# CompVis/stable-diffusion

Hardware: AMD Instinct MI355X
Metric: 512x512 images/sec, SD-v1-4 50-step PLMS CFG=7.5 (higher is better)
Workload: dtype f16

## Files before the change

### include/sdmi.h

```cpp
#ifndef SDMI_H_
#define SDMI_H_

#include <stdint.h>

#ifdef __cplusplus
extern "C" {
#endif

#define SDMI_ABI_VERSION 17

typedef struct sdmi_unet sdmi_unet;

typedef struct sdmi_unet_cfg {
  int32_t in_channels;
  int32_t out_channels;
  int32_t model_channels;
  int32_t num_res_blocks;
  int32_t n_levels;
  int32_t channel_mult[8];
  int32_t n_attention_resolutions;
  int32_t attention_resolutions[8];
  int32_t num_heads;
  int32_t transformer_depth;
  int32_t context_dim;
// ... 164 lines not shown
                       float* special_care_scores, int B, int Nc, int Ns, int E, void* stream);

typedef struct sdmi_knn sdmi_knn;
int sdmi_knn_create(int D, int64_t capacity_rows, sdmi_knn** out);
int sdmi_knn_destroy(sdmi_knn* h);
int sdmi_knn_set_rows(sdmi_knn* h, int64_t first_row, int64_t n, const float* rows, void* stream);
int sdmi_knn_finalize(sdmi_knn* h, void* stream);
int64_t sdmi_knn_rows(const sdmi_knn* h);
int sdmi_knn_dim(const sdmi_knn* h);
int64_t sdmi_knn_workspace_bytes(sdmi_knn* h, int B, int k);
int sdmi_knn_search(sdmi_knn* h, const float* queries, int B, int k, int32_t* idx_out, float* score_out, float* nn_out_or_null,
                    void* workspace, int64_t workspace_bytes, void* stream);
int sdmi_knn_condition(sdmi_knn* h, const float* c, int B, int k, float* c_out, int32_t* idx_out, float* score_out, void* workspace,
                       int64_t workspace_bytes, void* stream);
int sdmi_k_knn_inv_norm(const float* db, int64_t N, int D, float* inv_norm, void* stream);
int sdmi_k_knn_scan(const float* db, const float* inv_norm, int64_t N, int D, const float* queries, int B, int k, int64_t slab_rows,
                    float* cand_score, int32_t* cand_idx, void* stream);
int sdmi_k_knn_merge(const float* cand_score, const int32_t* cand_idx, int B, int n_lists, int k, int32_t* idx_out, float* score_out,
                     void* stream);
int sdmi_k_knn_stream_read(const float* p, int64_t n_floats, float* sink, void* stream);
int sdmi_k_knn_gather(const float* db, const float* inv_norm, int64_t N, int D, const int32_t* idx, int B, int k, const float* c0_or_null,
                      float* out, int64_t ldo, void* stream);

typedef struct sdmi_igemm_desc {
  const void* a0; const void* a1; const void* a2;
  int32_t c0, c1, c2, lda0, lda1, lda2;
  int32_t B, Hin, Win, Hout, Wout, ksize, stride, up;
  const void* w;
  int32_t N;
  int32_t mode;
  const float* bias; const float* rowvec; int32_t ld_rowvec;
  const float* residual; int32_t ldr;
  float* out_f32; void* out_f16; int32_t ldo;
  void* seg_dst[3]; int32_t seg_kind[3];
  int32_t heads, dh, ntok, ntok_pad, segC;
  int32_t splitk;
  float* splitk_ws; int64_t splitk_ws_floats;
  int32_t tile;
  int32_t dma;
  int32_t asym_pad;
  int32_t gn_n; void* gn_acc[2]; int32_t gn_cpg[2]; int32_t gn_cbase[2];
  int32_t* splitk_cnt; int32_t splitk_cnt_ints;
  int32_t split16;
  const float* f16_scale; float* lnp_out;
  const float* lnf_part; int32_t lnf_npart; float lnf_eps; const float* lnf_cs; const float* lnf_d;
  const float* pgn_gamma; const float* pgn_beta; float pgn_eps; int32_t pgn_silu;
  void* pgn_out; int32_t pgn_keep_f32; int32_t* pgn_applied;
  void* out_lo;
} sdmi_igemm_desc;
int sdmi_k_igemm(const sdmi_igemm_desc* d, void* stream);
int sdmi_k_igemm_tail(const sdmi_igemm_desc* d, const void* t0, const void* t1, const void* t2, int tail_c, int tail_ld, const void* tail_w,
                      int tail_kt, void* stream);
int sdmi_k_tail_split_range(int nkt, int nsplit, int split, int* begin, int* end);
int sdmi_k_ff_tail(const sdmi_igemm_desc* proj_out, const void* ln_f16, const float* lnp, float ln_eps, const float* csd,
                   const void* wgg_f16, const void* wff2_f16, const float* bff2, const float* t, void* stream);
int sdmi_k_st_tail(const sdmi_igemm_desc* proj_out, const void* a_f16, const void* wo_f16, const float* bo, float* t, const float* ln_gamma,
                   float ln_eps, const float* csd, const void* wgg_f16, const void* wff2_f16, const float* bff2, void* stream);
int sdmi_k_gn_conv3(const sdmi_igemm_desc* conv, const float* x0, const float* x1, int c0, int c1, float* gn_ws, int64_t gn_ws_floats,
                    const float* gn_gamma, const float* gn_beta, float gn_eps, void* stream);
int sdmi_k_st_head(const float* x, float* gn_ws, int64_t gn_ws_floats, const float* gn_gamma, const float* gn_beta, float gn_eps,
                   const void* w_in3, const float* b_in, float* t, const float* ln_gamma, float ln_eps, const void* wqkv_f16,
                   const float* lnf_cs, const float* lnf_d, void* q, void* k, void* vt, int B, int ntok, int ntok_pad, int heads, int dh,
                   int C, void* stream);
int sdmi_k_st_mid(const void* a_f16, const void* wo_f16, const float* bo, float* t, const float* ln_gamma, float ln_eps, const void* wq_f16,
                  const float* lnf_cs, const float* lnf_d, void* q, int B, int ntok, int heads, int dh, int C, void* stream);
int sdmi_k_st_mid_ctx(const void* a_f16, const void* wo_f16, const float* bo, float* t, const float* ln_gamma, float ln_eps, const void* wq_f16,
                      const float* lnf_cs, const float* lnf_d, const void* ctx_k, const void* ctx_vt, int nkv, int nkv_pad, float scale, void* ao_out,
                      int B, int ntok, int heads, int dh, int C, void* stream);
int sdmi_k_ln_fold_prep(const void* w_f16, int N, int K, int ldw, const float* gamma, const float* beta, const float* bias,
                        float* cs, float* d, void* stream);
int sdmi_k_attention(const void* q, const void* k, const void* vt, void* out, int BH, int heads, int nq, int nkv,
                     int nkv_pad, int d, float scale, void* stream);
int sdmi_k_attention_split16(const void* q, const void* q_lo, const void* k, const void* k_lo, const void* vt, const void* vt_lo, void* out,
                             void* out_lo, int BH, int heads, int nq, int nkv, int nkv_pad, int d, float scale, void* stream);
int sdmi_k_attention_split16_causal(const void* q, const void* q_lo, const void* k, const void* k_lo, const void* vt, const void* vt_lo,
                                    void* out, void* out_lo, int BH, int heads, int n, int n_pad, int d, float scale, void* stream);
int sdmi_k_attention_causal(const void* q, const void* k, const void* vt, void* out, int BH, int heads, int n, int n_pad,
                            int d, float scale, void* stream);
int sdmi_k_groupnorm(const float* x0, const float* x1, int c0, int c1, int B, int HW, const float* gamma,
                     const float* beta, float eps, int silu, void* out_f16, float* out_f32, void* raw_f16, void* out_lo,
                     void* raw_lo, float* partial_ws, int64_t partial_floats, void* stream);
int64_t sdmi_k_groupnorm_ws_floats(int B, int HW);
int sdmi_k_groupnorm_film(const float* x0, const float* x1, int c0, int c1, int B, int HW, const float* gamma, const float* beta, float eps,
                          int silu, const float* film, int film_ld, void* out_f16, float* out_f32, void* raw_f16, void* out_lo, void* raw_lo,
                          float* partial_ws, int64_t partial_floats, void* stream);
int sdmi_k_layernorm(const float* x, const float* gamma, const float* beta, void* out_f16, int M, int C, float eps,
                     void* stream);
int sdmi_k_cast_f16(const float* x, void* out_f16, void* out_lo, int64_t n, void* stream);
int sdmi_k_split_heads(const float* src, int ld, int col0, void* dst, void* dst_lo, int kind, int B, int ntok, int ntok_pad, int heads, int dh,
                       void* stream);
int sdmi_k_geglu_split(const float* src, int M, int F, void* out, void* out_lo, void* stream);
int sdmi_k_layernorm_split(const float* x, const float* gamma, const float* beta, void* out, void* out_lo, int M, int C, float eps, void* stream);
int sdmi_k_timestep_embedding(const int64_t* t_i64, const float* t_f32, float* out, int B, int dim, void* stream);
int sdmi_k_small_linear(const float* in, int ld_in, const float* w, const float* bias, float* out, int ld_out, int B,
                        int N, int K, int silu_in, void* stream);
int sdmi_k_conv_in(const float* x_nchw, const float* w_oihw, const float* bias, float* out_nhwc, int B, int Cin, int H,
                   int W, int Cout, void* stream);
int sdmi_k_conv_out(const float* h_nhwc, const float* w_ohwi, const float* bias, float* out_nchw, int B, int H, int W,
                    int Cin, int Cout, void* stream);
int sdmi_k_pack_conv_weight(const float* w_oihw, void* dst_f16, int O, int I, int KH, int KW, void* stream);
int sdmi_k_pack_conv_weight_src(const float* w_oihw, void* dst_f16, int O, int I, int KH, int KW, int c0, int c1, int c2, void* stream);
int sdmi_k_pack_conv_out(const float* w_oihw, float* dst_ohwi, int O, int I, void* stream);
int sdmi_k_pack_split3(const float* w, void* dst_f16, int N, int K, void* stream);
int sdmi_k_pack_conv_split3(const float* w_oihw, void* dst_f16, int O, int I, int KH, int KW, void* stream);
int sdmi_k_pointwise_nchw(const float* x, const float* w, const float* bias, float* out, int B, int Cin, int Cout, int HW,
                          float in_scale, void* stream);
// ... 31 lines not shown
```

### stable-diffusion_amd/_lib.py

```python
import ctypes as C
import os

_HERE = os.path.dirname(os.path.abspath(__file__))
LIB_PATH = os.environ.get('SDMI_LIB_PATH') or os.path.join(_HERE, 'libsdmi.so')

c_f32p = C.c_void_p
c_ptr = C.c_void_p


class UNetCfg(C.Structure):
    _fields_ = [('in_channels', C.c_int32), ('out_channels', C.c_int32), ('model_channels', C.c_int32),
                ('num_res_blocks', C.c_int32), ('n_levels', C.c_int32), ('channel_mult', C.c_int32 * 8),
                ('n_attention_resolutions', C.c_int32), ('attention_resolutions', C.c_int32 * 8),
                ('num_heads', C.c_int32), ('transformer_depth', C.c_int32), ('context_dim', C.c_int32)]


class VaeCfg(C.Structure):
    _fields_ = [('ch', C.c_int32), ('out_ch', C.c_int32), ('n_levels', C.c_int32), ('ch_mult', C.c_int32 * 8),
                ('num_res_blocks', C.c_int32), ('in_channels', C.c_int32), ('z_channels', C.c_int32),
                ('embed_dim', C.c_int32)]


class UNetExt(C.Structure):
    _fields_ = [('attention_block', C.c_int32), ('resblock_updown', C.c_int32)]
# ... 92 lines not shown
    'sdmi_clip_precision': (C.c_int, [c_ptr]),
    'sdmi_clip_destroy': (C.c_int, [c_ptr]),
    'sdmi_clip_num_weights': (C.c_int, [c_ptr]),
    'sdmi_clip_weight_info': (C.c_int, [c_ptr, C.c_int, C.c_char_p, C.c_int, C.POINTER(C.c_int64), C.POINTER(C.c_int)]),
    'sdmi_clip_set_weight': (C.c_int, [c_ptr, C.c_char_p, c_ptr, C.POINTER(C.c_int64), C.c_int, c_ptr]),
    'sdmi_clip_finalize': (C.c_int, [c_ptr]),
    'sdmi_clip_workspace_bytes': (C.c_int64, [c_ptr, C.c_int, C.c_int]),
    'sdmi_clip_forward': (C.c_int, [c_ptr, c_ptr, c_ptr, C.c_int, C.c_int, c_ptr, C.c_int64, c_ptr]),
    'sdmi_clip_create_projection': (C.c_int, [C.POINTER(ClipCfg), C.c_int, C.c_int, C.POINTER(c_ptr)]),
    'sdmi_clip_projection_dim': (C.c_int, [c_ptr]),
    'sdmi_clip_text_embeds_workspace_bytes': (C.c_int64, [c_ptr, C.c_int, C.c_int]),
    'sdmi_clip_text_embeds': (C.c_int, [c_ptr, c_ptr, c_ptr, C.c_int, C.c_int, C.c_int, c_ptr, C.c_int64, c_ptr]),
    'sdmi_bert_create': (C.c_int, [C.POINTER(BertCfg), C.POINTER(c_ptr)]),
    'sdmi_bert_create_precision': (C.c_int, [C.POINTER(BertCfg), C.c_int, C.POINTER(c_ptr)]),
    'sdmi_bert_precision': (C.c_int, [c_ptr]),
    'sdmi_bert_destroy': (C.c_int, [c_ptr]),
    'sdmi_bert_num_weights': (C.c_int, [c_ptr]),
    'sdmi_bert_weight_info': (C.c_int, [c_ptr, C.c_int, C.c_char_p, C.c_int, C.POINTER(C.c_int64), C.POINTER(C.c_int)]),
    'sdmi_bert_set_weight': (C.c_int, [c_ptr, C.c_char_p, c_ptr, C.POINTER(C.c_int64), C.c_int, c_ptr]),
    'sdmi_bert_finalize': (C.c_int, [c_ptr]),
    'sdmi_bert_workspace_bytes': (C.c_int64, [c_ptr, C.c_int, C.c_int]),
    'sdmi_bert_forward': (C.c_int, [c_ptr, c_ptr, c_ptr, C.c_int, C.c_int, c_ptr, C.c_int64, c_ptr]),
    'sdmi_vit_create': (C.c_int, [C.POINTER(VitCfg), C.POINTER(c_ptr)]),
    'sdmi_vit_destroy': (C.c_int, [c_ptr]),
    'sdmi_vit_num_weights': (C.c_int, [c_ptr]),
    'sdmi_vit_weight_info': (C.c_int, [c_ptr, C.c_int, C.c_char_p, C.c_int, C.POINTER(C.c_int64), C.POINTER(C.c_int)]),
    'sdmi_vit_set_weight': (C.c_int, [c_ptr, C.c_char_p, c_ptr, C.POINTER(C.c_int64), C.c_int, c_ptr]),
    'sdmi_vit_finalize': (C.c_int, [c_ptr]),
    'sdmi_vit_workspace_bytes': (C.c_int64, [c_ptr, C.c_int]),
    'sdmi_vit_forward': (C.c_int, [c_ptr, c_ptr, c_ptr, c_ptr, c_ptr, C.c_int, c_ptr, C.c_int64, c_ptr]),
    'sdmi_k_vit_kpad': (C.c_int, [C.c_int]),
    'sdmi_k_vit_patchify': (C.c_int, [c_ptr, c_ptr, C.c_int, C.c_int, C.c_int, c_ptr]),
    'sdmi_k_vit_embed': (C.c_int, [c_ptr, c_ptr, c_ptr, c_ptr, C.c_int, C.c_int, C.c_int, c_ptr]),
    'sdmi_k_vit_preprocess': (C.c_int, [c_ptr, c_ptr, C.c_int, C.c_int, C.c_int, C.c_int, c_ptr]),
    'sdmi_k_safety_head': (C.c_int, [c_ptr, c_ptr, c_ptr, c_ptr, c_ptr, c_ptr, c_ptr, c_ptr, C.c_int, C.c_int, C.c_int, C.c_int, c_ptr]),
    'sdmi_knn_create': (C.c_int, [C.c_int, C.c_int64, C.POINTER(c_ptr)]),
    'sdmi_knn_destroy': (C.c_int, [c_ptr]),
    'sdmi_knn_set_rows': (C.c_int, [c_ptr, C.c_int64, C.c_int64, c_ptr, c_ptr]),
    'sdmi_knn_finalize': (C.c_int, [c_ptr, c_ptr]),
    'sdmi_knn_rows': (C.c_int64, [c_ptr]),
    'sdmi_knn_dim': (C.c_int, [c_ptr]),
    'sdmi_knn_workspace_bytes': (C.c_int64, [c_ptr, C.c_int, C.c_int]),
    'sdmi_knn_search': (C.c_int, [c_ptr, c_ptr, C.c_int, C.c_int, c_ptr, c_ptr, c_ptr, c_ptr, C.c_int64, c_ptr]),
    'sdmi_knn_condition': (C.c_int, [c_ptr, c_ptr, C.c_int, C.c_int, c_ptr, c_ptr, c_ptr, c_ptr, C.c_int64, c_ptr]),
    'sdmi_k_knn_inv_norm': (C.c_int, [c_ptr, C.c_int64, C.c_int, c_ptr, c_ptr]),
    'sdmi_k_knn_scan': (C.c_int, [c_ptr, c_ptr, C.c_int64, C.c_int, c_ptr, C.c_int, C.c_int, C.c_int64, c_ptr, c_ptr, c_ptr]),
    'sdmi_k_knn_merge': (C.c_int, [c_ptr, c_ptr, C.c_int, C.c_int, C.c_int, c_ptr, c_ptr, c_ptr]),
    'sdmi_k_knn_stream_read': (C.c_int, [c_ptr, C.c_int64, c_ptr, c_ptr]),
    'sdmi_k_knn_gather': (C.c_int, [c_ptr, c_ptr, C.c_int64, C.c_int, c_ptr, C.c_int, C.c_int, c_ptr, c_ptr, C.c_int64, c_ptr]),
    'sdmi_has_experiments': (C.c_int, []),
    'sdmi_k_igemm': (C.c_int, [C.POINTER(IGemmDesc), c_ptr]),
    'sdmi_k_igemm_tail': (C.c_int, [C.POINTER(IGemmDesc), c_ptr, c_ptr, c_ptr, C.c_int, C.c_int, c_ptr, C.c_int, c_ptr]),
    'sdmi_k_tail_split_range': (C.c_int, [C.c_int, C.c_int, C.c_int, C.POINTER(C.c_int), C.POINTER(C.c_int)]),
    'sdmi_tune_lookup': (C.c_int, [C.c_int] * 9 + [C.POINTER(C.c_int), C.POINTER(C.c_int)]),
    'sdmi_unet_skip_fold_plan': (C.c_int, [c_ptr, C.c_int, C.c_int, C.c_int, C.c_int, C.POINTER(C.c_int32), C.c_int]),
    'sdmi_k_ff_tail': (C.c_int, [C.POINTER(IGemmDesc), c_ptr, c_ptr, C.c_float, c_ptr, c_ptr, c_ptr, c_ptr, c_ptr, c_ptr]),
    'sdmi_k_gn_conv3': (C.c_int, [C.POINTER(IGemmDesc), c_ptr, c_ptr, C.c_int, C.c_int, c_ptr, C.c_int64, c_ptr, c_ptr, C.c_float, c_ptr]),
    'sdmi_k_st_mid_ctx': (C.c_int, [c_ptr, c_ptr, c_ptr, c_ptr, c_ptr, C.c_float, c_ptr, c_ptr, c_ptr, c_ptr, c_ptr, C.c_int, C.c_int, C.c_float, c_ptr,
                                    C.c_int, C.c_int, C.c_int, C.c_int, C.c_int, c_ptr]),
    'sdmi_k_st_tail': (C.c_int, [C.POINTER(IGemmDesc), c_ptr, c_ptr, c_ptr, c_ptr, c_ptr, C.c_float, c_ptr, c_ptr, c_ptr, c_ptr, c_ptr]),
    'sdmi_k_st_mid': (C.c_int, [c_ptr, c_ptr, c_ptr, c_ptr, c_ptr, C.c_float, c_ptr, c_ptr, c_ptr, c_ptr, C.c_int, C.c_int, C.c_int, C.c_int,
                                C.c_int, c_ptr]),
    'sdmi_k_st_head': (C.c_int, [c_ptr, c_ptr, C.c_int64, c_ptr, c_ptr, C.c_float, c_ptr, c_ptr, c_ptr, c_ptr, C.c_float, c_ptr, c_ptr, c_ptr,
                                 c_ptr, c_ptr, c_ptr, C.c_int, C.c_int, C.c_int, C.c_int, C.c_int, C.c_int, c_ptr]),
    'sdmi_k_attention_split16': (C.c_int, [c_ptr, c_ptr, c_ptr, c_ptr, c_ptr, c_ptr, c_ptr, c_ptr, C.c_int, C.c_int, C.c_int, C.c_int,
                                           C.c_int, C.c_int, C.c_float, c_ptr]),
    'sdmi_k_attention_split16_causal': (C.c_int, [c_ptr, c_ptr, c_ptr, c_ptr, c_ptr, c_ptr, c_ptr, c_ptr, C.c_int, C.c_int, C.c_int, C.c_int,
                                                  C.c_int, C.c_float, c_ptr]),
    'sdmi_k_attention_causal': (C.c_int, [c_ptr, c_ptr, c_ptr, c_ptr, C.c_int, C.c_int, C.c_int, C.c_int, C.c_int, C.c_float,
                                          c_ptr]),
    'sdmi_k_pointwise_nchw': (C.c_int, [c_ptr, c_ptr, c_ptr, c_ptr, C.c_int, C.c_int, C.c_int, C.c_int, C.c_float, c_ptr]),
    'sdmi_k_softmax_rows': (C.c_int, [c_ptr, c_ptr, C.c_int, C.c_int, C.c_float, c_ptr]),
    'sdmi_k_gelu_erf': (C.c_int, [c_ptr, c_ptr, C.c_int64, c_ptr]),
    'sdmi_k_quick_gelu': (C.c_int, [c_ptr, c_ptr, C.c_int64, c_ptr]),
    'sdmi_k_quick_gelu_split': (C.c_int, [c_ptr, c_ptr, c_ptr, C.c_int64, c_ptr]),
    'sdmi_k_gelu_erf_split': (C.c_int, [c_ptr, c_ptr, c_ptr, C.c_int64, c_ptr]),
    'sdmi_k_attention': (C.c_int, [c_ptr, c_ptr, c_ptr, c_ptr, C.c_int, C.c_int, C.c_int, C.c_int, C.c_int, C.c_int,
                                   C.c_float, c_ptr]),
    'sdmi_k_groupnorm': (C.c_int, [c_ptr, c_ptr, C.c_int, C.c_int, C.c_int, C.c_int, c_ptr, c_ptr, C.c_float, C.c_int,
                                   c_ptr, c_ptr, c_ptr, c_ptr, c_ptr, c_ptr, C.c_int64, c_ptr]),
    'sdmi_k_groupnorm_ws_floats': (C.c_int64, [C.c_int, C.c_int]),
    'sdmi_k_groupnorm_film': (C.c_int, [c_ptr, c_ptr, C.c_int, C.c_int, C.c_int, C.c_int, c_ptr, c_ptr, C.c_float, C.c_int, c_ptr, C.c_int,
                                        c_ptr, c_ptr, c_ptr, c_ptr, c_ptr, c_ptr, C.c_int64, c_ptr]),
    'sdmi_k_layernorm': (C.c_int, [c_ptr, c_ptr, c_ptr, c_ptr, C.c_int, C.c_int, C.c_float, c_ptr]),
    'sdmi_k_cast_f16': (C.c_int, [c_ptr, c_ptr, c_ptr, C.c_int64, c_ptr]),
    'sdmi_k_split_heads': (C.c_int, [c_ptr, C.c_int, C.c_int, c_ptr, c_ptr, C.c_int, C.c_int, C.c_int, C.c_int, C.c_int, C.c_int,
                                     c_ptr]),
    'sdmi_k_geglu_split': (C.c_int, [c_ptr, C.c_int, C.c_int, c_ptr, c_ptr, c_ptr]),
    'sdmi_k_layernorm_split': (C.c_int, [c_ptr, c_ptr, c_ptr, c_ptr, c_ptr, C.c_int, C.c_int, C.c_float, c_ptr]),
    'sdmi_k_timestep_embedding': (C.c_int, [c_ptr, c_ptr, c_ptr, C.c_int, C.c_int, c_ptr]),
    'sdmi_k_small_linear': (C.c_int, [c_ptr, C.c_int, c_ptr, c_ptr, c_ptr, C.c_int, C.c_int, C.c_int, C.c_int,
                                      C.c_int, c_ptr]),
    'sdmi_k_conv_in': (C.c_int, [c_ptr, c_ptr, c_ptr, c_ptr, C.c_int, C.c_int, C.c_int, C.c_int, C.c_int, c_ptr]),
    'sdmi_k_conv_out': (C.c_int, [c_ptr, c_ptr, c_ptr, c_ptr, C.c_int, C.c_int, C.c_int, C.c_int, C.c_int, c_ptr]),
    'sdmi_k_pack_conv_weight': (C.c_int, [c_ptr, c_ptr, C.c_int, C.c_int, C.c_int, C.c_int, c_ptr]),
    'sdmi_k_pack_conv_weight_src': (C.c_int, [c_ptr, c_ptr, C.c_int, C.c_int, C.c_int, C.c_int, C.c_int, C.c_int, C.c_int, c_ptr]),
    'sdmi_k_pack_conv_out': (C.c_int, [c_ptr, c_ptr, C.c_int, C.c_int, c_ptr]),
    'sdmi_k_pack_split3': (C.c_int, [c_ptr, c_ptr, C.c_int, C.c_int, c_ptr]),
    'sdmi_k_pack_conv_split3': (C.c_int, [c_ptr, c_ptr, C.c_int, C.c_int, C.c_int, C.c_int, c_ptr]),
    'sdmi_k_pack_geglu': (C.c_int, [c_ptr, c_ptr, c_ptr, c_ptr, C.c_int, C.c_int, c_ptr]),
    'sdmi_k_ln_fold_prep': (C.c_int, [c_ptr, C.c_int, C.c_int, C.c_int, c_ptr, c_ptr, c_ptr, c_ptr, c_ptr, c_ptr]),
    'sdmi_image_to_uint8': (C.c_int, [c_ptr, c_ptr, C.c_int, C.c_int, C.c_int, C.c_int, c_ptr]),
    'sdmi_range_check': (C.c_int, [C.c_int]),
    'sdmi_range_report': (C.c_int, [C.c_char_p, C.c_int]),
    'sdmi_tune_begin': (C.c_int, []),
    'sdmi_tune_round': (C.c_int, [C.c_int]),
# ... 49 lines not shown
```

### stable-diffusion_amd/csrc/api.cpp

```cpp
#include <string.h>

#include <new>

#include "prof.h"
#include "split16.h"
#include "unet.h"
#include "vae.h"
#include "clip.h"
#include "knn.h"

namespace sdmi {
static thread_local std::string g_err;
void set_error(const std::string& msg) { g_err = msg; }
int fail(const std::string& msg) { g_err = msg; return -1; }
}

struct sdmi_unet { sdmi::UNet impl; };
struct sdmi_vae { sdmi::Vae impl; };
struct sdmi_clip { sdmi::ClipText impl; };
struct sdmi_bert { sdmi::BertText impl; };
struct sdmi_vit { sdmi::ClipVision impl; };
struct sdmi_knn { sdmi::Knn impl; };

using namespace sdmi;
// ... 451 lines not shown
  p.vt = (const f16*)vt; p.vt_lo = (const f16*)vt_lo; p.out = (f16*)out; p.out_lo = (f16*)out_lo;
  p.BH = BH; p.heads = heads; p.nq = n; p.nkv = n; p.nkv_pad = n_pad; p.d = d; p.scale = scale; p.causal = 1;
  return launch_attention_split16(p, (hipStream_t)stream);
}
int sdmi_k_attention_causal(const void* q, const void* k, const void* vt, void* out, int BH, int heads, int n, int n_pad,
                            int d, float scale, void* stream) {
  AttnParams a = AttnParams();
  a.q = (const f16*)q; a.k = (const f16*)k; a.vt = (const f16*)vt; a.out = (f16*)out;
  a.BH = BH; a.heads = heads; a.nq = n; a.nkv = n; a.nkv_pad = n_pad; a.d = d; a.scale = scale; a.causal = 1;
  return launch_attention(a, (hipStream_t)stream);
}

static int igemm_params_of(const sdmi_igemm_desc* d, IGemmParams& p) {
  p.a0 = (const f16*)d->a0; p.a1 = (const f16*)d->a1; p.a2 = (const f16*)d->a2;
  p.c0 = d->c0; p.c1 = d->c1; p.c2 = d->c2; p.lda0 = d->lda0; p.lda1 = d->lda1; p.lda2 = d->lda2;
  p.B = d->B; p.Hin = d->Hin; p.Win = d->Win; p.Hout = d->Hout; p.Wout = d->Wout;
  p.ksize = d->ksize; p.stride = d->stride; p.up = d->up; p.pad = d->asym_pad ? 0 : 1;
  p.w = (const f16*)d->w; p.M = d->B * d->Hout * d->Wout; p.N = d->N; p.K = d->ksize * d->ksize * (d->c0 + d->c1 + d->c2);
  p.mode = d->mode; p.bias = d->bias; p.rowvec = d->rowvec; p.ld_rowvec = d->ld_rowvec;
  p.residual = d->residual; p.ldr = d->ldr; p.out_f32 = d->out_f32; p.out_f16 = (f16*)d->out_f16; p.ldo = d->ldo;
  for (int i = 0; i < 3; ++i) { p.seg_dst[i] = (f16*)d->seg_dst[i]; p.seg_kind[i] = d->seg_kind[i]; }
  p.heads = d->heads; p.dh = d->dh; p.ntok = d->ntok; p.ntok_pad = d->ntok_pad; p.segC = d->segC;
  p.splitk = d->splitk; p.splitk_ws = d->splitk_ws; p.splitk_ws_floats = d->splitk_ws_floats;
  p.splitk_cnt = d->splitk_cnt; p.splitk_cnt_ints = d->splitk_cnt_ints;
  p.gn_n = d->gn_n;
  for (int i = 0; i < 2; ++i) { p.gn_acc[i] = (long long*)d->gn_acc[i]; p.gn_cpg[i] = d->gn_cpg[i]; p.gn_cbase[i] = d->gn_cbase[i]; }
  if (d->split16) {
    p.split16 = 1; p.c1 = 0; p.K = d->c0; p.ldw = 3 * d->c0;
  }
  p.f16_scale = d->f16_scale; p.lnp_out = d->lnp_out;
  p.lnf_part = d->lnf_part; p.lnf_npart = d->lnf_npart; p.lnf_eps = d->lnf_eps; p.lnf_cs = d->lnf_cs; p.lnf_d = d->lnf_d;
  p.pgn_gamma = d->pgn_gamma; p.pgn_beta = d->pgn_beta; p.pgn_eps = d->pgn_eps; p.pgn_silu = d->pgn_silu;
  p.pgn_out = (f16*)d->pgn_out; p.pgn_keep_f32 = d->pgn_keep_f32; p.pgn_applied = d->pgn_applied;
  p.out_lo = (f16*)d->out_lo;
  return zero_page(&p.zero_page);
}
int sdmi_k_igemm(const sdmi_igemm_desc* d, void* stream) {
  SDMI_CHECK(d, "null descriptor");
  IGemmParams p = IGemmParams();
  if (igemm_params_of(d, p)) return -1;
  IGemmTune t; t.tile = d->tile; t.dma = d->dma;
  return launch_igemm(p, t, (hipStream_t)stream);
}
int sdmi_k_igemm_tail(const sdmi_igemm_desc* d, const void* t0, const void* t1, const void* t2, int tail_c, int tail_ld, const void* tail_w,
                      int tail_kt, void* stream) {
  SDMI_CHECK(d, "null descriptor");
  IGemmParams p = IGemmParams();
  if (igemm_params_of(d, p)) return -1;
  p.tail_a0 = (const f16*)t0; p.tail_a1 = (const f16*)t1; p.tail_a2 = (const f16*)t2;
  p.tail_c = tail_c; p.tail_ld = tail_ld; p.tail_w = (const f16*)tail_w; p.tail_kt = tail_kt;
  IGemmTune t; t.tile = d->tile; t.dma = d->dma;
  return launch_igemm(p, t, (hipStream_t)stream);
}
int sdmi_k_tail_split_range(int nkt, int nsplit, int split, int* begin, int* end) {
  SDMI_CHECK(begin && end && nkt >= 0 && nsplit >= 1 && split >= 0 && split < nsplit, "bad arguments");
  tail_split_range(nkt, nsplit, split, begin, end);
  return 0;
}
int sdmi_tune_lookup(int M, int N, int K, int ksize, int stride, int up, int mode, int splitk_req, int kt, int* tile, int* splitk) {
  SDMI_CHECK(tile && splitk, "null argument");
  return tune_lookup(M, N, K, ksize, stride, up, mode, splitk_req, kt, tile, splitk);
}
int sdmi_unet_skip_fold_plan(sdmi_unet* h, int B, int H, int W, int Lctx, int32_t* folded, int cap) {
  SDMI_CHECK(h && (folded || cap == 0), "null argument");
  int64_t need = 0;
  if (h->impl.run(nullptr, nullptr, nullptr, nullptr, nullptr, B, H, W, Lctx, nullptr, 0, nullptr, true, false, &need)) return -1;
  const std::vector<int>& plan = h->impl.skip_fold_plan_;
  for (int i = 0; i < (int)plan.size() && i < cap; ++i) folded[i] = plan[i];
  return (int)plan.size();
}
int sdmi_k_ff_tail(const sdmi_igemm_desc* proj_out, const void* ln_f16, const float* lnp, float ln_eps, const float* csd,
                   const void* wgg_f16, const void* wff2_f16, const float* bff2, const float* t, void* stream) {
  SDMI_CHECK(proj_out, "null descriptor");
  FfTailParams q = FfTailParams();
  if (igemm_params_of(proj_out, q.epi)) return -1;
  SDMI_CHECK(proj_out->split16 && proj_out->ksize == 1, "ff_tail: the proj_out descriptor is a split-fp16 1x1 (w = sdmi_k_pack_split3)");
  q.ln = (const f16*)ln_f16; q.lnp = lnp; q.ln_eps = ln_eps; q.csd = csd; q.wgg = (const f16*)wgg_f16; q.wff2 = (const f16*)wff2_f16;
  q.bff2 = bff2; q.t = t; q.wpo = (const f16*)proj_out->w;
  return launch_ff_tail(q, (hipStream_t)stream);
}
int sdmi_k_st_tail(const sdmi_igemm_desc* proj_out, const void* a_f16, const void* wo_f16, const float* bo, float* t, const float* ln_gamma,
                   float ln_eps, const float* csd, const void* wgg_f16, const void* wff2_f16, const float* bff2, void* stream) {
  SDMI_CHECK(proj_out && a_f16, "null argument");
  FfTailParams q = FfTailParams();
  if (igemm_params_of(proj_out, q.epi)) return -1;
  SDMI_CHECK(proj_out->split16 && proj_out->ksize == 1, "st_tail: the proj_out descriptor is a split-fp16 1x1 (w = sdmi_k_pack_split3)");
  q.a16 = (const f16*)a_f16; q.wo = (const f16*)wo_f16; q.bo = bo; q.ln_gamma = ln_gamma; q.ln_eps = ln_eps; q.csd = csd;
  q.wgg = (const f16*)wgg_f16; q.wff2 = (const f16*)wff2_f16; q.bff2 = bff2; q.t = t; q.wpo = (const f16*)proj_out->w;
  return launch_ff_tail(q, (hipStream_t)stream);
}
int sdmi_k_gn_conv3(const sdmi_igemm_desc* conv, const float* x0, const float* x1, int c0, int c1, float* gn_ws, int64_t gn_ws_floats,
                    const float* gn_gamma, const float* gn_beta, float gn_eps, void* stream) {
  SDMI_CHECK(conv && x0 && gn_ws && gn_gamma && gn_beta, "gn_conv3: null argument");
  GnConvParams q = GnConvParams();
  if (igemm_params_of(conv, q.epi)) return -1;
  const int B = q.epi.B;
  SDMI_CHECK(gn_ws_floats >= gn_acc_words(B) * 2, "groupnorm workspace too small");
  SDMI_HIP_OK(hipMemsetAsync(gn_ws, 0, gn_acc_words(B) * sizeof(long long), (hipStream_t)stream));
  GroupNormParams g = GroupNormParams();
  g.x0 = x0; g.c0 = c0; g.x1 = x1; g.c1 = c1; g.B = B; g.HW = q.epi.Hout * q.epi.Wout; g.gamma = gn_gamma; g.beta = gn_beta; g.eps = gn_eps;
  g.stats_only = 1; g.acc = (long long*)gn_ws;
  if (launch_groupnorm(g, (hipStream_t)stream)) return -1;
  q.x0 = x0; q.x1 = x1; q.c0 = c0; q.c1 = c1; q.gn_acc = (const long long*)gn_ws; q.gn_gamma = gn_gamma; q.gn_beta = gn_beta; q.gn_eps = gn_eps;
  q.w = (const f16*)conv->w;
  return launch_gn_conv3(q, (hipStream_t)stream);
}
// ... 174 lines not shown
```

### stable-diffusion_amd/csrc/common.h

```cpp
#pragma once
#include <hip/hip_runtime.h>
#include <stdint.h>
#include <algorithm>
#include <string>

#include "tape.h"

typedef _Float16 f16;
typedef _Float16 f16x2 __attribute__((ext_vector_type(2)));
typedef _Float16 f16x4 __attribute__((ext_vector_type(4)));
typedef _Float16 f16x8 __attribute__((ext_vector_type(8)));
typedef float f32x4 __attribute__((ext_vector_type(4)));
typedef float f32x16 __attribute__((ext_vector_type(16)));

#ifdef __HIPCC__
__device__ __forceinline__ float gn_apply_elem(float v, float mean, float rstd, float gamma, float beta, int silu) {
  float t = __builtin_fmaf((v - mean) * rstd, gamma, beta);
  if (silu) t = t * __builtin_amdgcn_rcpf(1.0f + __expf(-t));
  return t;
}
__device__ __forceinline__ float gn_apply_film_elem(float v, float mean, float rstd, float gamma, float beta, float scale, float shift,
                                                    int silu) {
  float t = __builtin_fmaf((v - mean) * rstd, gamma, beta);
  t = __builtin_fmaf(t, 1.0f + scale, shift);
// ... 115 lines not shown
  f16* seg_dst[3] = {nullptr, nullptr, nullptr};
  int seg_kind[3] = {0, 0, 0};
  int heads = 0, dh = 0, ntok = 0, ntok_pad = 0, segC = 0;
  int splitk = 1;
  float* splitk_ws = nullptr; int64_t splitk_ws_floats = 0;
  int* splitk_cnt = nullptr; int splitk_cnt_ints = 0;
  int nkt = 0;
#ifdef SDMI_IGEMM_TIMING
  long long* dbg_times = nullptr;
  int dbg_abl = 0;
#endif
  int splitk_fused = 0;
  int slab_tiled = 0, slab_bm = 0, slab_bn = 0, slab_wm = 0, slab_wn = 0;
  int slab_sh_qpt = 0, slab_sh_nt = 0, slab_sh_tn = 0, slab_sh_wn = 0;
  int epi_vec = 0;
  int tile_n_fastest = 0;
  const f16* zero_page = nullptr;
  int gn_n = 0;
  long long* gn_acc[2] = {nullptr, nullptr};
  int gn_cpg[2] = {0, 0}, gn_cbase[2] = {0, 0};
  unsigned long long gn_magic[2] = {0, 0};
  const float* pgn_gamma = nullptr; const float* pgn_beta = nullptr; float pgn_eps = 1e-5f; int pgn_silu = 1;
  f16* pgn_out = nullptr;
  int pgn_keep_f32 = 0;
  int* pgn_applied = nullptr;
  unsigned long long magic_hw = 0, magic_w = 0, magic_w2 = 0;
  int log2w = 0;
  const float* xf0 = nullptr; const float* xf1 = nullptr;
  const long long* gn_in_acc = nullptr;
  const float* gn_in_gamma = nullptr; const float* gn_in_beta = nullptr; float gn_in_eps = 1e-5f; int gn_in_silu = 1;
  f16* raw_hi = nullptr; f16* raw_lo = nullptr;
  f16* gn_scratch = nullptr;
  unsigned long long magic_cpg_in = 0;
  int halo_thi = 0, halo_ipt = 1, log2_tpi = 30;
  unsigned long long magic_hpi = 0;
  const f16* tail_a0 = nullptr; const f16* tail_a1 = nullptr; const f16* tail_a2 = nullptr;
  int tail_c = 0, tail_ld = 0;
  const f16* tail_w = nullptr;
  int tail_kt = 0;
};
__host__ __device__ static inline void tail_split_range(int nkt, int nsplit, int split, int* begin, int* end) {
  *begin = (int)(((long long)split * nkt) / nsplit);
  *end = (int)(((long long)(split + 1) * nkt) / nsplit);
}

constexpr int SDMI_NUM_TILES = 22;
struct IGemmTune {
  int tile = -1;
  int dma = -1;
};

int launch_igemm(const IGemmParams& p, const IGemmTune& tune, hipStream_t stream);
bool igemm_plans_halo(const IGemmParams& p);
int tune_lookup(int M, int N, int K, int ksize, int stride, int up, int mode, int splitk_req, int kt, int* tile, int* splitk);
bool range_check_enabled();
uint64_t tune_generation();
bool tune_collecting();
int range_check_set(int enable);
int range_scan(const char* what, const f16* p, int64_t n, hipStream_t stream);
int range_report(std::string* json);

int tune_begin();
int tune_round(int r);
int tune_end(const char* path, int* n_keys);
int tune_dump(std::string* out);
int launch_splitk_reduce(const IGemmParams& p, int nsplit, hipStream_t stream);

struct FfTailParams {
  const f16* ln = nullptr;
  const float* lnp = nullptr;
  float ln_eps = 1e-5f;
  const float* csd = nullptr;
  const f16* wgg = nullptr;
  const f16* wff2 = nullptr;
  const float* bff2 = nullptr;
  const float* t = nullptr;
  const f16* wpo = nullptr;
  const f16* a16 = nullptr;
  const f16* wo = nullptr;
  const float* bo = nullptr;
  const float* ln_gamma = nullptr;
#ifdef SDMI_RC_TIMING
  long long* dbg = nullptr;
#endif
  IGemmParams epi;
};
bool ff_tail_supported(int C, int M, int rows_per_sample);
int launch_ff_tail(const FfTailParams& p, hipStream_t stream);

struct StHeadParams {
  const f16* a16 = nullptr;
  const float* x = nullptr;
  const long long* gn_acc = nullptr;
  const float* gn_gamma = nullptr; const float* gn_beta = nullptr; float gn_eps = 1e-6f;
  const f16* w_in = nullptr;
  const float* b_in = nullptr;
  float* t = nullptr;
  const float* ln_gamma = nullptr;
  float ln_eps = 1e-5f;
  const f16* wqkv = nullptr;
  const float* lnf_cs = nullptr; const float* lnf_d = nullptr;
  f16* q = nullptr; f16* k = nullptr;
  f16* vt = nullptr;
  int M = 0, B = 0, ntok = 0, ntok_pad = 0, heads = 0, dh = 0, C = 0;
  const f16* ctx_k = nullptr; const f16* ctx_vt = nullptr; int ctx_nkv = 0, ctx_nkv_pad = 0; float ctx_scale = 0.f; f16* ao_out = nullptr;
#ifdef SDMI_RC_TIMING
// ... 70 lines not shown

struct DpmStepParams {
  const float* eps_model = nullptr;
  int cfg = 0; float scale = 1.f;
  const float* x = nullptr;
  const float* m_prev = nullptr;
  float alpha_s = 1.f, sigma_s = 0.f;
  float cx = 1.f, a = 0.f, inv_r0 = 0.f;
  int order = 1;
  float* m_out = nullptr;
  float* x_next = nullptr;
  int64_t n = 0;
};
int launch_dpm_step(const DpmStepParams& p, hipStream_t s);

int launch_embed_tokens(const int64_t* ids, const float* tok_emb, const float* pos_emb, float* out, int M, int L, int C,
                        int vocab, hipStream_t s);
int launch_quick_gelu(const float* x, f16* out, int64_t n, hipStream_t s);
int launch_gelu_erf(const float* x, f16* out, int64_t n, hipStream_t s);
int launch_quick_gelu_split(const float* x, f16* out, f16* out_lo, int64_t n, hipStream_t s);
int launch_gelu_erf_split(const float* x, f16* out, f16* out_lo, int64_t n, hipStream_t s);

int vit_kpad(int patch_size);
int launch_vit_patchify(const float* px, f16* out, int B, int S, int p, hipStream_t s);
int launch_vit_embed(const float* patch, const float* cls, const float* pos, float* out, int B, int T, int C, hipStream_t s);
int launch_vit_preprocess(const float* x, float* out, int B, int H, int W, int S, hipStream_t s);
int launch_safety_head(const float* image_embeds, const float* concept_embeds, const float* special_care_embeds, const float* concept_thr,
                       const float* special_thr, int* has_nsfw, float* concept_scores, float* special_scores, int B, int Nc, int Ns, int E,
                       hipStream_t s);

int launch_pointwise_nchw(const float* x_nchw, const float* w, const float* bias, float* out_nchw, int B, int Cin, int Cout,
                          int HW, float in_scale, hipStream_t s);
int launch_softmax_rows(const float* S, f16* P, int rows, int cols, int lds, int ldp, float scale, hipStream_t s);

int launch_resample2(const float* x, float* o32, f16* hi, f16* lo, int B, int H, int W, int C, int dir, hipStream_t s);
int launch_vq_norms(const float* e, float* se, int n_embed, int D, hipStream_t s);
int launch_vq_quantize(const float* z, float z_scale, const float* e, const float* se, int n_embed, int D, float* zq, int* idx, int B,
                       int HW, hipStream_t s);

int launch_patch_unfold(const float* x, const float* c, float* out, int B, int Cx, int Cc, int H, int W, int kh, int kw, int sy, int sx,
                        int l0, int nl, hipStream_t s);
int launch_patch_fold(const float* o, const float* w, float* out, int B, int C, int H, int W, int kh, int kw, int sy, int sx, int uf, int df,
                      int norm_only, hipStream_t s);

int launch_prefetch_lines(const void* ptr, int64_t bytes, hipStream_t s);

int launch_pack_conv_weight(const float* w_oihw, f16* dst, int O, int I, int KH, int KW, hipStream_t s);
int launch_pack_rows(const float* w, f16* dst, int rows, int cols, int dst_row0, int dst_ld, hipStream_t s);
int launch_ln_fold_prep(const f16* w, int N, int K, int ldw, const float* gamma, const float* beta, const float* bias, float* cs,
                        float* d, hipStream_t s);
int launch_pack_split3(const float* w, f16* dst, int N, int K, hipStream_t s);
int launch_pack_conv_weight_src(const float* w_oihw, f16* dst, int O, int I, int KH, int KW, int c0, int c1, int c2, hipStream_t s);
int launch_pack_conv_split3(const float* w, f16* dst, int O, int I, int KH, int KW, hipStream_t s);
int launch_pack_geglu(const float* w, const float* bias, f16* wdst, float* bdst, int N, int K, hipStream_t s);
int launch_pack_conv_out(const float* w_oihw, float* dst, int O, int I, hipStream_t s);

struct SamplerStepParams {
  const float* eps_model = nullptr;
  int cfg = 0; float scale = 1.f;
  const float* x = nullptr;
  int mode = 0;
  const float* old0 = nullptr; const float* old1 = nullptr; const float* old2 = nullptr;
  float a_t = 1.f, a_prev = 1.f, sigma = 0.f, sqrt_1m_at = 0.f;
  const float* noise = nullptr;
  float* e_t_out = nullptr;
  float* x_prev = nullptr; float* pred_x0 = nullptr;
  int64_t n = 0;
};
int launch_sampler_step(const SamplerStepParams& p, hipStream_t s);
int launch_image_u8(const float* img_nchw, unsigned char* out_nhwc, int B, int C, int H, int W, hipStream_t s);

}
```

### stable-diffusion_amd/csrc/igemm.hip

```cpp
#include <dlfcn.h>

#include <map>
#include <mutex>
#include <tuple>
#include <vector>

#include "igemm_dev.h"

namespace sdmi {
namespace {

__global__ void __launch_bounds__(256) splitk_reduce_kernel(IGemmParams p, int nsplit, int rows_per_block) {
  __shared__ unsigned long long s_gn[2][32][GN_WORDS];
  const int tx = threadIdx.x & 7, ty = threadIdx.x >> 3;
  const int n = (blockIdx.x * 8 + tx) * 4;
  const int row0 = blockIdx.y * rows_per_block;
  const int HW = p.Hout * p.Wout;
  const bool gn = p.gn_n > 0;
  const bool ncol = n < p.N;
  if (gn) {
    for (int i = threadIdx.x; i < 2 * 32 * GN_WORDS; i += 256) (&s_gn[0][0][0])[i] = 0ull;
    __syncthreads();
  }
  const size_t slab_sz = (size_t)p.M * p.N;
// ... 375 lines not shown
static inline bool tile_tn_even(int t) { return (kTiles[t].bn / kTiles[t].wn / 32) % 2 == 0; }

static int launch_tile(int tile, const IGemmParams& p, bool dma, int splitk, hipStream_t stream) {
  if (p.tail_kt && !tile_is_halo(tile)) return fail("a GEMM with a 1x1 tail phase was routed to tile " + std::to_string(tile) + ": only the halo-staged conv tiles 14..17 run a tail");
  if (p.split16) return launch_split16_tile(tile, p, splitk, stream);
  if (igemm_has_half(p)) {
    switch (tile) {
      case 0: case 1: case 2: case 3: case 4: case 5: return launch_generic_tile_h0(tile, p, dma, splitk, stream);
      case 6: case 7: case 8: case 9: case 10: return launch_generic_tile_h1(tile, p, dma, splitk, stream);
      case 11: case 12: case 13: case 18: case 19: case 20: case 21: return launch_generic_tile_h2(tile, p, dma, splitk, stream);
      default: break;
    }
  }
  switch (tile) {
    case 0: case 1: case 2: case 3: case 4: case 5: return launch_generic_tile_g0(tile, p, dma, splitk, stream);
    case 6: case 7: case 8: case 9: case 10: return launch_generic_tile_g1(tile, p, dma, splitk, stream);
    case 11: case 12: case 13: case 18: case 19: case 20: case 21: return launch_generic_tile_g2(tile, p, dma, splitk, stream);
    case 14: case 15: case 16: case 17: return launch_halo_tile(tile, p, splitk, stream);
    default: return fail("unknown igemm tile id");
  }
}

struct TuneKey {
  int M, N, K, ksize, stride, up, mode, splitk_req;
  int kt = 0;
  bool operator<(const TuneKey& o) const {
    return std::tie(M, N, K, ksize, stride, up, mode, splitk_req, kt) <
           std::tie(o.M, o.N, o.K, o.ksize, o.stride, o.up, o.mode, o.splitk_req, o.kt);
  }
};
struct TuneChoice { int tile, splitk; double us; };
struct TuneRec { TuneKey key; int cand; hipEvent_t e0, e1; };

class Tuner {
 public:
  std::mutex mu;
  std::map<TuneKey, TuneChoice> table;
  bool loaded = false, collecting = false;
  int round = 0;
  std::vector<TuneRec> recs;
  std::map<TuneKey, std::vector<std::pair<TuneChoice, std::vector<float>>>> stats;
  std::vector<hipEvent_t> pool;

  static std::string default_path() {
    if (const char* e = getenv("SDMI_TUNE_FILE")) return e;
    Dl_info info;
    if (dladdr((const void*)&Tuner::default_path, &info) && info.dli_fname) {
      std::string so = info.dli_fname;
      const size_t k = so.find_last_of('/');
      return (k == std::string::npos ? std::string(".") : so.substr(0, k)) + "/tune_gfx950.txt";
    }
    return "tune_gfx950.txt";
  }
  void load_file(const std::string& path) {
    FILE* f = fopen(path.c_str(), "r");
    if (!f) return;
    char line[256];
    while (fgets(line, sizeof line, f)) {
      if (line[0] == '#') continue;
      TuneKey k; TuneChoice c; c.us = 0;
      k.kt = 0;
      if (sscanf(line, "%d %d %d %d %d %d %d %d %d %d %lf %d", &k.M, &k.N, &k.K, &k.ksize, &k.stride, &k.up, &k.mode,
                 &k.splitk_req, &c.tile, &c.splitk, &c.us, &k.kt) >= 10 && c.tile >= 0 && c.tile < SDMI_NUM_TILES && c.splitk >= 1 &&
          c.splitk <= 16 && k.kt >= 0)
        table[k] = c;
    }
    fclose(f);
  }
  void ensure_loaded() {
    if (loaded) return;
    loaded = true;
    if (env_int("SDMI_TUNE_DISABLE", 0)) return;
    load_file(default_path());
  }
  std::map<TuneKey, TuneChoice>::const_iterator find_entry(TuneKey k) const {
    auto it = table.find(k);
    if (it == table.end() && k.kt) { k.kt = 0; it = table.find(k); }
    return it;
  }
  hipEvent_t ev() {
    if (!pool.empty()) { hipEvent_t e = pool.back(); pool.pop_back(); return e; }
    hipEvent_t e = nullptr;
    (void)hipEventCreate(&e);
    return e;
  }
};
static Tuner g_tuner;

static std::vector<TuneChoice> tune_candidates(const IGemmParams& p, bool can_split) {
  std::vector<TuneChoice> out;
  const int nkt = igemm_nkt(p);
  static const int splits[] = {1, 2, 3, 4, 5, 6, 8, 10, 12, 16};
  for (int t = 0; t < SDMI_NUM_TILES; ++t) {
    const TileCfg& c = kTiles[t];
    if (tile_is_halo(t) && !halo_supported(p, c.bm)) continue;
    if (p.tail_kt && !tile_is_halo(t)) continue;
    if (p.split16 && !split16_tile_supported(t)) continue;
    if (!p.split16 && ((c.ns == 2 && t != 11 && !tile_is_halo(t)) || t == 12 || t == 13)) continue;
    if (p.mode == EPI_GEGLU && !tile_tn_even(t)) continue;
    if (p.lnp_out && (p.M % c.bm || p.N % c.bn || (p.Hout * p.Wout) % c.bm)) continue;
    const long blocks = (long)cdiv(p.M, c.bm) * cdiv(p.N, c.bn);
    if ((long)c.bm > 2L * p.M && c.bm > 64) continue;
    if ((long)c.bn > 2L * p.N && c.bn > 64) continue;
    for (int sk : splits) {
      if ((sk == 5 || sk == 10) && !tile_is_halo(t)) continue;
      if (sk > 1) {
        if (p.splitk != 0 || !can_split) break;
        if (nkt / sk < 4) break;
        if (tile_is_halo(t) && (nkt / 9) % sk != 0) continue;
        if (blocks * (sk / 2 + 1) > 1536) break;
        if (splitk_ws_need(p, c.bm, c.bn, sk) > p.splitk_ws_floats) break;
      }
      if (blocks * sk < 48 && sk < 16 && nkt / (sk * 2) >= 4 && can_split && p.splitk == 0) continue;
      out.push_back({t, p.splitk > 1 ? p.splitk : sk, 0.0});
      if (p.splitk != 0) break;
    }
  }
  if (out.empty()) out.push_back({5, p.splitk > 0 ? p.splitk : 1, 0.0});
  return out;
}

int tune_begin() {
  std::lock_guard<std::mutex> lk(g_tuner.mu);
  g_tuner.ensure_loaded();
  g_tuner.collecting = true; g_tuner.round = 0;
  g_tuner.recs.clear(); g_tuner.stats.clear();
  return 0;
}
int tune_round(int r) {
  std::lock_guard<std::mutex> lk(g_tuner.mu);
  g_tuner.round = r;
  return 0;
}
static int tune_drain() {
  for (auto& r : g_tuner.recs) {
    float ms = 0.f;
    SDMI_HIP_OK(hipEventSynchronize(r.e1));
    SDMI_HIP_OK(hipEventElapsedTime(&ms, r.e0, r.e1));
    auto& v = g_tuner.stats[r.key];
    if ((int)v.size() > r.cand) v[r.cand].second.push_back(ms * 1e3f);
    g_tuner.pool.push_back(r.e0); g_tuner.pool.push_back(r.e1);
  }
  g_tuner.recs.clear();
  return 0;
}
bool tune_collecting() { return g_tuner.collecting; }
static uint64_t g_tune_generation = 0;
uint64_t tune_generation() { return g_tune_generation; }
int tune_end(const char* path, int* n_keys) {
  std::lock_guard<std::mutex> lk(g_tuner.mu);
  if (!g_tuner.collecting) return fail("sdmi_tune_end without sdmi_tune_begin");
  if (tune_drain()) return -1;
  g_tuner.collecting = false;
  auto score = [](std::vector<float> v) -> double {
    if (v.empty()) return 1e30;
    std::sort(v.begin(), v.end());
    return v.size() % 2 ? v[v.size() / 2] : 0.5 * (v[v.size() / 2 - 1] + v[v.size() / 2]);
  };
  for (auto& kv : g_tuner.stats) {
    double best = 1e30; const TuneChoice* bc = nullptr;
    for (auto& c : kv.second) {
      const double sc = score(c.second);
      if (sc < best) { best = sc; bc = &c.first; }
    }
    if (bc) g_tuner.table[kv.first] = {bc->tile, bc->splitk, best};
  }
  if (n_keys) *n_keys = (int)g_tuner.stats.size();
  ++g_tune_generation;
  const std::string out = (path && *path) ? std::string(path) : Tuner::default_path();
  FILE* f = fopen(out.c_str(), "w");
  if (!f) return fail("cannot write the tuning table to " + out);
  fprintf(f, "# libsdmi igemm tuning table (gfx950), measured in situ by tools/tune.py -- M N K ksize stride up mode splitk_req tile splitk us\n");
  for (auto& kv : g_tuner.table) {
    const TuneKey& k = kv.first;
    fprintf(f, "%d %d %d %d %d %d %d %d %d %d %.2f", k.M, k.N, k.K, k.ksize, k.stride, k.up, k.mode, k.splitk_req, kv.second.tile,
            kv.second.splitk, kv.second.us);
    if (k.kt) fprintf(f, " %d", k.kt);
    fprintf(f, "\n");
  }
  fclose(f);
  return 0;
}
int tune_dump(std::string* out) {
  std::lock_guard<std::mutex> lk(g_tuner.mu);
  char buf[256];
  for (auto& kv : g_tuner.stats) {
    const TuneKey& k = kv.first;
    for (auto& c : kv.second) {
      if (c.second.empty()) continue;
      std::vector<float> v = c.second;
      std::sort(v.begin(), v.end());
      snprintf(buf, sizeof buf, "%d %d %d %d %d %d %d %d%s | %d %d %.2f %.2f %d\n", k.M, k.N, k.K, k.ksize, k.stride, k.up, k.mode,
               k.splitk_req, k.kt ? (" t" + std::to_string(k.kt)).c_str() : "", c.first.tile, c.first.splitk, (double)v[v.size() / 2], (double)v[0], (int)v.size());
      *out += buf;
    }
  }
  return 0;
}

int tune_lookup(int M, int N, int K, int ksize, int stride, int up, int mode, int splitk_req, int kt, int* tile, int* splitk) {
  std::lock_guard<std::mutex> lk(g_tuner.mu);
  g_tuner.ensure_loaded();
  auto it = g_tuner.find_entry(TuneKey{M, N, K, ksize, stride, up, mode, splitk_req, kt});
  if (it == g_tuner.table.end()) return 1;
  *tile = it->second.tile; *splitk = it->second.splitk;
  return 0;
}

bool igemm_plans_halo(const IGemmParams& p) {
  static const int env_tile = env_int("SDMI_IGEMM_TILE", -1);
  if (p.ksize != 3 || p.split16 || igemm_has_half(p) || p.mode != EPI_PLAIN || p.splitk != 0 || env_tile >= 0 || env_int("SDMI_SPLITK", -1) >= 0) return false;
  std::lock_guard<std::mutex> lk(g_tuner.mu);
  g_tuner.ensure_loaded();
  if (g_tuner.collecting) {
    for (int t = 14; t <= 17; ++t) if (halo_supported(p, kTiles[t].bm)) return true;
    return false;
  }
  auto it = g_tuner.find_entry(TuneKey{p.M, p.N, igemm_nkt(p) * BK, p.ksize, p.stride, p.up, p.mode, 0, p.tail_kt});
  if (it == g_tuner.table.end()) return false;
  const int tt = it->second.tile, sk = it->second.splitk, nkt = igemm_nkt(p);
  const bool can_split = p.splitk_ws && p.N % 4 == 0 && p.ldo % 4 == 0 && (p.residual == nullptr || p.ldr % 4 == 0);
  return tile_is_halo(tt) && halo_supported(p, kTiles[tt].bm) &&
         (sk == 1 || (can_split && splitk_ws_need(p, kTiles[tt].bm, kTiles[tt].bn, sk) <= p.splitk_ws_floats && nkt / sk >= 4 && (nkt / 9) % sk == 0));
}

int launch_igemm(const IGemmParams& p, const IGemmTune& tune, hipStream_t stream) {
  SDMI_CHECK(p.M > 0 && p.N > 0 && p.K > 0, "empty GEMM");
  SDMI_CHECK(p.ksize == 1 || p.ksize == 3, "ksize must be 1 or 3");
  const int Cin = p.c0 + p.c1 + p.c2;
  SDMI_CHECK(p.K == p.ksize * p.ksize * Cin, "K != ksize^2 * (c0 + c1 + c2)");
  SDMI_CHECK(p.c0 % BKH == 0 && p.c1 % BKH == 0 && p.c2 % BKH == 0 && p.c0 > 0, "channel counts of every A source must be multiples of 32");
  SDMI_CHECK((p.c2 == 0 || p.c1 > 0), "third A source without a second");
  SDMI_CHECK(p.lda0 % 8 == 0 && (p.a1 == nullptr || p.lda1 % 8 == 0), "A row pitch must be a multiple of 8 halves");
  SDMI_CHECK(p.zero_page != nullptr, "zero page missing");
  SDMI_CHECK(p.M == p.B * p.Hout * p.Wout, "M != B * Hout * Wout");
  SDMI_CHECK(p.c1 == 0 || p.a1 != nullptr, "second A source missing");
  SDMI_CHECK(p.c2 == 0 || (p.a2 != nullptr && p.lda2 % 8 == 0), "third A source missing");
  SDMI_CHECK((p.c1 == 0 || p.lda1 == p.lda0) && (p.c2 == 0 || p.lda2 == p.lda0), "all A sources must share one row pitch");
  SDMI_CHECK(!p.up || (p.ksize == 3 && p.stride == 1), "upsample folding needs a 3x3 stride-1 conv");
  if (p.mode == EPI_GEGLU) SDMI_CHECK(p.N % 64 == 0 && p.out_f16 != nullptr, "GEGLU needs N % 64 == 0 and an fp16 output");
  if (p.ln_out)
    SDMI_CHECK(p.mode == EPI_PLAIN && p.out_f32 && p.ldo == p.N && p.N % 4 == 0 && p.N <= 2560 && p.ln_gamma && p.ln_beta,
               "LayerNorm post-op needs plain mode, an fp32 output with ldo == N <= 2560, gamma and beta");
  if (p.out_lo) SDMI_CHECK(p.mode == EPI_PLAIN && p.ldo % 4 == 0, "out_lo needs plain mode");
  if (p.lnp_out || p.f16_scale)
    SDMI_CHECK(p.mode == EPI_PLAIN && p.out_f32 && p.out_f16 && !p.out_lo && !p.ln_out && p.N % 64 == 0 && p.M % 64 == 0 &&
                   (p.Hout * p.Wout) % 64 == 0 && p.splitk == 1 && epi_vec_ok(p),
               "LayerNorm row statistics: plain mode, fp32 + fp16 outputs, no split-K, M / N / rows per sample multiples of 64, 16-byte aligned rows");
  if (p.lnf_part)
    SDMI_CHECK(p.ksize == 1 && p.c1 == 0 && p.c2 == 0 && !p.split16 && p.lnf_npart * 32 == p.K && p.lnf_cs && p.lnf_d && !p.bias &&
                   p.splitk == 1 && p.lnf_npart <= 40,
               "LayerNorm-folding GEMM: dense, one source, K = 32 * lnf_npart <= 1280, column sums + offsets, no bias, no split-K");
  if (p.gn_n) {
    SDMI_CHECK(p.mode == EPI_PLAIN && p.gn_n <= 2 && (p.Hout * p.Wout) % 32 == 0, "GroupNorm statistics need plain mode and Hout*Wout % 32 == 0");
    SDMI_CHECK(p.N % 4 == 0, "GroupNorm statistics: N % 4 == 0");
    for (int t = 0; t < p.gn_n; ++t)
      SDMI_CHECK(p.gn_acc[t] && p.gn_cpg[t] >= 2 && (p.gn_cbase[t] + p.N + p.gn_cpg[t] - 1) / p.gn_cpg[t] <= 32, "bad GroupNorm statistics target");
  }
  if (p.mode == EPI_HEADS) SDMI_CHECK(p.segC > 0 && p.dh > 0 && p.N % p.segC == 0 && p.N / p.segC <= 3, "bad head scatter");

  SDMI_CHECK((int64_t)p.B * p.Hin * p.Win * p.lda0 * 2 + (int64_t)(p.Win + 1) * p.lda0 * 2 < ((int64_t)1 << 31) - 65536 &&
                 (int64_t)p.N * p.K * 2 < ((int64_t)1 << 31) - 65536,
             "tensor too large for 31-bit byte offsets (buffer addressing)");
  static const int env_dma = env_int("SDMI_IGEMM_DMA", 1);
  static const int env_tile = env_int("SDMI_IGEMM_TILE", -1);
  const bool dma = (tune.dma >= 0 ? tune.dma : env_dma) != 0;
  int tile = tune.tile >= 0 ? tune.tile : env_tile;
  SDMI_CHECK(tile < SDMI_NUM_TILES, "unknown igemm tile id");
  int splitk = p.splitk;
  const int nkt = igemm_nkt(p);
  static const int env_split = env_int("SDMI_SPLITK", -1);
  const bool can_split_plain = p.mode == EPI_PLAIN && p.splitk_ws && p.N % 4 == 0 && p.ldo % 4 == 0 &&
                               (p.residual == nullptr || p.ldr % 4 == 0);
  const bool can_split_heads = p.mode == EPI_HEADS && p.splitk_ws && p.dh % 4 == 0 && p.segC % 4 == 0;
  const bool can_split = can_split_plain || can_split_heads;
  if (env_split >= 0 && splitk == 0) splitk = env_split;

  hipEvent_t ev0 = nullptr, ev1 = nullptr;
  TuneKey tkey{p.M, p.N, nkt * BK, p.split16 ? 11 : p.ksize, p.stride, p.up, p.mode, splitk, p.tail_kt};
  int tcand = -1;
  if (tile < 0) {
    std::lock_guard<std::mutex> lk(g_tuner.mu);
    g_tuner.ensure_loaded();
    static const int only_ksize = env_int("SDMI_TUNE_ONLY_KSIZE", -1);
    if (g_tuner.collecting && (only_ksize < 0 || tkey.ksize == only_ksize)) {
      IGemmParams q = p; q.splitk = splitk;
      const std::vector<TuneChoice> cands = tune_candidates(q, can_split);
      auto& st = g_tuner.stats[tkey];
      if (st.empty()) for (auto& c : cands) st.push_back({c, {}});
      tcand = g_tuner.round % (int)cands.size();
      tile = cands[tcand].tile; splitk = cands[tcand].splitk;
      ev0 = g_tuner.ev(); ev1 = g_tuner.ev();
    } else {
      auto it = g_tuner.find_entry(tkey);
      if (it != g_tuner.table.end()) {
        const int tt = it->second.tile, sk = it->second.splitk;
        const bool halo = tile_is_halo(tt);
        const bool ws_ok = sk == 1 || (can_split && splitk_ws_need(p, kTiles[tt].bm, kTiles[tt].bn, sk) <= p.splitk_ws_floats);
        const bool split_ok = splitk != 0 ? (sk == splitk && ws_ok)
                                          : (sk == 1 || (ws_ok && nkt / sk >= 4 && (halo || (sk != 5 && sk != 10)) &&
                                                         (!halo || (nkt / 9) % sk == 0)));
        if (split_ok && (p.mode != EPI_GEGLU || tile_tn_even(tt)) && (!halo || halo_supported(p, kTiles[tt].bm)) &&
            (!p.split16 || split16_tile_supported(tt))) {
          tile = tt; splitk = sk;
        }
      }
    }
  }
  if (p.mode == EPI_GEGLU && tile >= 0 && !tile_tn_even(tile)) tile = 0;
  if (p.split16) {
    if (tile >= 0) SDMI_CHECK(split16_tile_supported(tile), "split-fp16 GEMM: tile id without an instantiation");
    else tile = 5;
  }
  if (tile < 0) {
    const double gflop = 2.0 * p.M * (double)p.N * p.K * 1e-9;
    if (p.mode == EPI_GEGLU) tile = 0;
    else if (p.mode == EPI_HEADS) tile = 2;
    else tile = gflop >= 25.0 ? 3 : 5;
  }
  if (p.lnp_out) {
    const int hw = p.Hout * p.Wout;
    if (p.M % kTiles[tile].bm || p.N % kTiles[tile].bn || hw % kTiles[tile].bm || (p.split16 && !split16_tile_supported(tile))) tile = 5;
  }
  if (splitk <= 0) {
    splitk = 1;
    if (can_split) {
      const long blocks = (long)cdiv(p.M, kTiles[tile].bm) * cdiv(p.N, kTiles[tile].bn);
      const long want = (kTiles[tile].wm * kTiles[tile].wn == 8) ? 160 : 512;
      while (blocks * splitk < want && nkt / (splitk * 2) >= 8 && splitk < 16 &&
             splitk_ws_need(p, kTiles[tile].bm, kTiles[tile].bn, splitk * 2) <= p.splitk_ws_floats)
        splitk *= 2;
    }
  }
  if (splitk > 1) {
    SDMI_CHECK(can_split, "split-K needs plain or head-scatter mode, a slab workspace and N / ldo / ldr multiples of 4");
    SDMI_CHECK(splitk_ws_need(p, kTiles[tile].bm, kTiles[tile].bn, splitk) <= p.splitk_ws_floats, "split-K workspace too small");
  }
  if (ev0) SDMI_HIP_OK(hipEventRecord(ev0, stream));
#ifdef SDMI_IGEMM_TIMING
  static const char* dbg_path = getenv("SDMI_IGEMM_TIMING");
  static const int dbg_abl = env_int("SDMI_EPI_ABL", 0);
  static long long* dbg_buf = nullptr;
  constexpr int DBG_WG = 16384;
  IGemmParams pd = p;
  pd.dbg_abl = dbg_abl;
  if (dbg_path) {
    if (!dbg_buf) SDMI_HIP_OK(hipMalloc((void**)&dbg_buf, 6 * DBG_WG * sizeof(long long)));
    SDMI_HIP_OK(hipMemsetAsync(dbg_buf, 0, 6 * DBG_WG * sizeof(long long), stream));
    pd.dbg_times = dbg_buf;
  }
  const int rc = launch_tile(tile, pd, dma, splitk, stream);
  if (dbg_path && pd.dbg_times && rc == 0) {
    SDMI_HIP_OK(hipStreamSynchronize(stream));
    std::vector<long long> h(6 * DBG_WG);
    SDMI_HIP_OK(hipMemcpy(h.data(), dbg_buf, h.size() * sizeof(long long), hipMemcpyDeviceToHost));
    std::vector<long long> pro, loop, epi, sto, start;
    long long tmin = 0, tmax = 0;
    for (int b = 0; b < DBG_WG; ++b) {
      const long long* d = &h[6 * b];
      if (d[4] == 0) continue;
      pro.push_back(d[1] - d[0]); loop.push_back(d[2] - d[1]); epi.push_back(d[4] - d[2]);
      sto.push_back(d[3] ? d[3] - d[2] : d[4] - d[2]);
      if (start.empty() || d[0] < tmin) tmin = d[0];
      if (d[4] > tmax) tmax = d[4];
      start.push_back(d[0]);
    }
    if (!pro.empty()) {
      auto med = [](std::vector<long long>& v) { std::sort(v.begin(), v.end()); return v[v.size() / 2]; };
      auto mx = [](std::vector<long long>& v) { return *std::max_element(v.begin(), v.end()); };
      long long late = 0;
      for (long long t : start) late = std::max(late, t - tmin);
      if (FILE* f = fopen(dbg_path, "a")) {
        const int nkt_split = (p.K / BK + std::max(splitk, 1) - 1) / std::max(splitk, 1);
        fprintf(f, "M%d N%d K%d k%d mode%d tile%d split%d res%d gn%d blocks%zu k-tiles/block %d | shader cycles: span %lld last-start %lld | median prologue %lld loop %lld epilogue %lld (stores %lld) | max loop %lld max epi %lld | loop cycles per k-tile %.1f\n",
                p.M, p.N, p.K, p.ksize, p.mode, tile, splitk, p.residual ? 1 : 0, p.gn_n, pro.size(), nkt_split, tmax - tmin, late, med(pro), med(loop),
                med(epi), med(sto), mx(loop), mx(epi), (double)med(loop) / nkt_split);
        fclose(f);
      }
    }
  }
#else
  const int rc = launch_tile(tile, p, dma, splitk, stream);
#endif
  if (rc == 0 && range_check_enabled()) {
    const char* what = p.mode == EPI_GEGLU ? "igemm GEGLU output" : (p.mode == EPI_HEADS ? "igemm q/k/v^T" : "igemm fp16 output");
    if (p.mode == EPI_HEADS) {
      for (int sg = 0; sg < p.N / p.segC; ++sg)
        if (range_scan(what, p.seg_dst[sg], p.seg_kind[sg] == 0 ? (int64_t)p.M * p.segC : (int64_t)p.B * p.segC * p.ntok_pad, stream)) return -1;
    } else if (p.out_f16) {
      if (range_scan(what, p.out_f16, (int64_t)(p.M - 1) * p.ldo + (p.mode == EPI_GEGLU ? p.N / 2 : p.N), stream)) return -1;
    }
    if (p.ln_out && range_scan("LayerNorm output", p.ln_out, (int64_t)p.M * p.N, stream)) return -1;
  }
  if (ev0) {
    SDMI_HIP_OK(hipEventRecord(ev1, stream));
    std::lock_guard<std::mutex> lk(g_tuner.mu);
    g_tuner.recs.push_back({tkey, tcand, ev0, ev1});
  }
  return rc;
}

}
```

### stable-diffusion_amd/csrc/igemm_dev.h

```cpp
#pragma once
#include "common.h"
#include "prof.h"

namespace sdmi {
typedef unsigned u32x4 __attribute__((ext_vector_type(4)));

int launch_splitk_reduce(const IGemmParams& p, int nsplit, hipStream_t stream);
int launch_generic_tile_g0(int tile, const IGemmParams& p, bool dma, int splitk, hipStream_t stream);
int launch_generic_tile_g1(int tile, const IGemmParams& p, bool dma, int splitk, hipStream_t stream);
int launch_generic_tile_g2(int tile, const IGemmParams& p, bool dma, int splitk, hipStream_t stream);
int launch_generic_tile_h0(int tile, const IGemmParams& p, bool dma, int splitk, hipStream_t stream);
int launch_generic_tile_h1(int tile, const IGemmParams& p, bool dma, int splitk, hipStream_t stream);
int launch_generic_tile_h2(int tile, const IGemmParams& p, bool dma, int splitk, hipStream_t stream);

static int env_int(const char* name, int dflt) {
  const char* v = getenv(name);
  return v ? atoi(v) : dflt;
}

namespace {

constexpr int BK = 64;
constexpr int BKH = 32;
static inline int src_chunks(int c) { return (c + BK - 1) / BK; }
static inline bool igemm_has_half(const IGemmParams& p) { return p.split16 ? (p.K % BK != 0) : (p.c0 % BK || p.c1 % BK || p.c2 % BK); }
static inline int igemm_nkt(const IGemmParams& p) {
  if (p.split16) return src_chunks(p.K);
  return p.ksize * p.ksize * (src_chunks(p.c0) + src_chunks(p.c1) + src_chunks(p.c2));
}

#ifdef SDMI_IGEMM_TIMING
#define SDMI_STAMP(name) const long long name = p.dbg_times ? (long long)__builtin_readcyclecounter() : 0
#else
#define SDMI_STAMP(name)
#endif

__device__ __forceinline__ float gelu_erf(float x) {
  const float z = fabsf(x) * 0.70710678118654752440f;
  const float t = __builtin_amdgcn_rcpf(1.0f + 0.3275911f * z);
  const float poly = t * (0.254829592f + t * (-0.284496736f + t * (1.421413741f + t * (-1.453152027f + t * 1.061405429f))));
  const float erf_abs = 1.0f - poly * __expf(-z * z);
  const float erf_v = __builtin_copysignf(erf_abs, x);
  return 0.5f * x * (1.0f + erf_v);
}

__device__ __forceinline__ void wait_vmcnt_n(int n) {
  switch (n) {
#define SDMI_VMCNT_CASE(k) case k: asm volatile("s_waitcnt vmcnt(" #k ")" ::: "memory"); break
    SDMI_VMCNT_CASE(0); SDMI_VMCNT_CASE(1); SDMI_VMCNT_CASE(2); SDMI_VMCNT_CASE(3); SDMI_VMCNT_CASE(4);
    SDMI_VMCNT_CASE(5); SDMI_VMCNT_CASE(6); SDMI_VMCNT_CASE(7); SDMI_VMCNT_CASE(8); SDMI_VMCNT_CASE(9);
    SDMI_VMCNT_CASE(10); SDMI_VMCNT_CASE(11); SDMI_VMCNT_CASE(12); SDMI_VMCNT_CASE(13); SDMI_VMCNT_CASE(14);
    SDMI_VMCNT_CASE(15); SDMI_VMCNT_CASE(16); SDMI_VMCNT_CASE(17); SDMI_VMCNT_CASE(18); SDMI_VMCNT_CASE(19);
    SDMI_VMCNT_CASE(20); SDMI_VMCNT_CASE(21); SDMI_VMCNT_CASE(22); SDMI_VMCNT_CASE(23); SDMI_VMCNT_CASE(24);
    SDMI_VMCNT_CASE(25); SDMI_VMCNT_CASE(26); SDMI_VMCNT_CASE(27); SDMI_VMCNT_CASE(28); SDMI_VMCNT_CASE(29);
    SDMI_VMCNT_CASE(30); SDMI_VMCNT_CASE(31); SDMI_VMCNT_CASE(32); SDMI_VMCNT_CASE(33); SDMI_VMCNT_CASE(34);
    SDMI_VMCNT_CASE(35); SDMI_VMCNT_CASE(36); SDMI_VMCNT_CASE(37); SDMI_VMCNT_CASE(38); SDMI_VMCNT_CASE(39);
    SDMI_VMCNT_CASE(40); SDMI_VMCNT_CASE(41); SDMI_VMCNT_CASE(42); SDMI_VMCNT_CASE(43); SDMI_VMCNT_CASE(44);
    SDMI_VMCNT_CASE(45); SDMI_VMCNT_CASE(46); SDMI_VMCNT_CASE(47); SDMI_VMCNT_CASE(48);
#undef SDMI_VMCNT_CASE
    default: __builtin_trap();
  }
}
template <int N>
__device__ __forceinline__ void wait_vmcnt() {
  static_assert(N >= 0 && N <= 48, "add the literal");
  wait_vmcnt_n(N);
}

enum : int { KIND_1X1 = 0, KIND_3X3 = 1, KIND_3X3_UP = 2 };

__device__ __forceinline__ int fast_div(int m, unsigned long long magic) {
  return (int)(((unsigned long long)(unsigned)m * magic) >> 40);
}
__device__ __forceinline__ int fast_div_hw(int m, unsigned long long magic) {
  return (int)(((unsigned long long)(unsigned)m * magic) >> 48);
}

#if defined(__HIP_DEVICE_COMPILE__)
template <int WTN> constexpr int SLAB_LPR = WTN / 4;
template <int WTN> constexpr int SLAB_RPI = 64 / (WTN / 4);
template <int WTN> constexpr int SLAB_NPASS = 32 / (64 / (WTN / 4));
template <int NWAVES, int WTN, int LDS_BYTES>
constexpr int SLAB_LSTR = (NWAVES * 32 * (WTN + 4) * 4 <= LDS_BYTES) ? WTN + 4 : WTN;
template <int NWAVES, int WTN, int LDS_BYTES>
__device__ __forceinline__ float* slab_base(unsigned char* smem, int wave) {
  static_assert(WTN == 32 || WTN == 64, "lane mapping of the 16-byte epilogue");
  static_assert(NWAVES * 32 * SLAB_LSTR<NWAVES, WTN, LDS_BYTES> * 4 <= LDS_BYTES, "LDS too small for the epilogue slabs");
  return (float*)smem + wave * (32 * SLAB_LSTR<NWAVES, WTN, LDS_BYTES>);
}
template <int TN, int LSTR>
__device__ __forceinline__ void slab_put(float* wl, const f32x16 (&a)[TN], int l31, int lg) {
#pragma unroll
  for (int j = 0; j < TN; ++j)
#pragma unroll
    for (int r = 0; r < 16; ++r) wl[((r & 3) + 8 * (r >> 2) + 4 * lg) * LSTR + j * 32 + l31] = a[j][r];
  asm volatile("s_waitcnt lgkmcnt(0)" ::: "memory");
}
template <int TN, int LSTR>
__device__ __forceinline__ void slab_get(const float* wl, f32x16 (&a)[TN], int l31, int lg) {
  asm volatile("s_waitcnt lgkmcnt(0)" ::: "memory");
#pragma unroll
  for (int j = 0; j < TN; ++j)
#pragma unroll
    for (int r = 0; r < 16; ++r) a[j][r] = wl[((r & 3) + 8 * (r >> 2) + 4 * lg) * LSTR + j * 32 + l31];
  asm volatile("s_waitcnt lgkmcnt(0)" ::: "memory");
}

constexpr int LNF_MAXP = 40;
__device__ __forceinline__ void lnf_request(const IGemmParams& p, int m, float2 (&pv)[LNF_MAXP]) {
  const float2* src = (const float2*)p.lnf_part + m;
#pragma unroll
  for (int j = 0; j < 20; ++j) pv[j] = src[(size_t)min(j, p.lnf_npart - 1) * p.M];
  if (p.lnf_npart > 20) {
#pragma unroll
    for (int j = 20; j < LNF_MAXP; ++j) pv[j] = src[(size_t)min(j, p.lnf_npart - 1) * p.M];
  } else {
#pragma unroll
    for (int j = 20; j < LNF_MAXP; ++j) pv[j] = float2{0.f, 0.f};
  }
}
__device__ __forceinline__ void lnf_finish(const IGemmParams& p, const float2 (&pv)[LNF_MAXP], float* mean, float* rstd) {
  float s = 0.f, q = 0.f;
#pragma unroll
  for (int j = 0; j < LNF_MAXP; ++j)
    if (j < p.lnf_npart) { s += pv[j].x; q += pv[j].y; }
  const float inv_c = 1.0f / (32.0f * (float)p.lnf_npart);
  const float mu = s * inv_c;
  const float var = fmaxf(q * inv_c - mu * mu, 0.f);
  *mean = mu;
  *rstd = 1.0f / sqrtf(var + p.lnf_eps);
}
__device__ __forceinline__ float sum8_dpp(float v) {
  v += __builtin_bit_cast(float, __builtin_amdgcn_update_dpp(0, __builtin_bit_cast(int, v), 0xB1, 0xF, 0xF, true));
  v += __builtin_bit_cast(float, __builtin_amdgcn_update_dpp(0, __builtin_bit_cast(int, v), 0x4E, 0xF, 0xF, true));
  v += __builtin_bit_cast(float, __builtin_amdgcn_update_dpp(0, __builtin_bit_cast(int, v), 0x141, 0xF, 0xF, true));
  return v;
}

template <int BM, int BN, int WARPS_M, int WARPS_N, int LDS_BYTES>
__device__ __forceinline__ void igemm_epilogue(const IGemmParams& p_arg, f32x16 (&acc)[BM / WARPS_M / 32][BN / WARPS_N / 32],
                                               const int m0, const int n0, const int split, const int tile_m,
                                               const int tile_n, unsigned char* smem, const float lnf_mean = 0.f,
                                               const float lnf_rstd = 1.f) {
#ifdef SDMI_IGEMM_TIMING
  IGemmParams p = p_arg;
  if (p.dbg_abl & 1) p.residual = nullptr;
  if (p.dbg_abl & 4) { p.out_f32 = nullptr; p.out_f16 = nullptr; p.out_lo = nullptr; }
#else
  const IGemmParams& p = p_arg;
#endif
  constexpr int NT = WARPS_M * WARPS_N * 64;
  constexpr int WTM = BM / WARPS_M, WTN = BN / WARPS_N;
  constexpr int TM = WTM / 32, TN = WTN / 32;
  constexpr int LSTR = SLAB_LSTR<WARPS_M * WARPS_N, WTN, LDS_BYTES>;
  const int tid = threadIdx.x;
  const int lane = tid & 63;
  const int wave = tid >> 6;
  const int wm = wave / WARPS_N, wn = wave - wm * WARPS_N;
  const int l31 = lane & 31, lg = lane >> 5;
  const int HWout = p.Hout * p.Wout;
  const int mw = m0 + wm * WTM, nw = n0 + wn * WTN;
  const bool full = (m0 + BM <= p.M) && (n0 + BN <= p.N);
  if (p.splitk > 1 && p.splitk_fused) {
    constexpr int SC1 = 16;
    const int tile_lin = tile_m * ((p.N + BN - 1) / BN) + tile_n;
    const __amdgpu_buffer_rsrc_t ws = __builtin_amdgcn_make_buffer_rsrc(
        (void*)(p.splitk_ws + (size_t)tile_lin * p.splitk * (BM * BN)), 0, p.splitk * (BM * BN) * 4, 0x00020000);
    const int my_off = (split * (BM * BN) + tid * 4) * 4;
#pragma unroll
    for (int i = 0; i < TM; ++i)
#pragma unroll
      for (int j = 0; j < TN; ++j)
#pragma unroll
        for (int r4 = 0; r4 < 4; ++r4) {
          const f32x4 v = {acc[i][j][4 * r4], acc[i][j][4 * r4 + 1], acc[i][j][4 * r4 + 2], acc[i][j][4 * r4 + 3]};
          __builtin_amdgcn_raw_buffer_store_b128(__builtin_bit_cast(u32x4, v), ws, my_off + ((i * TN + j) * 4 + r4) * (NT * 16), 0, SC1);
        }
    asm volatile("s_waitcnt vmcnt(0)" ::: "memory");
    __syncthreads();
    if (tid == 0) *(volatile int*)smem = __hip_atomic_fetch_add(p.splitk_cnt + tile_lin, 1, __ATOMIC_RELAXED, __HIP_MEMORY_SCOPE_AGENT);
    __syncthreads();
    const int ticket = *(volatile int*)smem;
    if (ticket != p.splitk - 1) return;
    if (tid == 0) __hip_atomic_store(p.splitk_cnt + tile_lin, 0, __ATOMIC_RELAXED, __HIP_MEMORY_SCOPE_AGENT);
#pragma unroll
    for (int i = 0; i < TM; ++i)
#pragma unroll
      for (int j = 0; j < TN; ++j)
#pragma unroll
        for (int r = 0; r < 16; ++r) acc[i][j][r] = 0.f;
    constexpr int QPS = TM * TN * 4;
    constexpr int SB = QPS >= 16 ? 1 : 16 / QPS;
    for (int s0 = 0; s0 < p.splitk; s0 += SB) {
      f32x4 v[SB][QPS];
#pragma unroll
      for (int ss = 0; ss < SB; ++ss) {
        const int off = (min(s0 + ss, p.splitk - 1) * (BM * BN) + tid * 4) * 4;
#pragma unroll
        for (int e = 0; e < QPS; ++e)
          v[ss][e] = __builtin_bit_cast(f32x4, __builtin_amdgcn_raw_buffer_load_b128(ws, off + e * (NT * 16), 0, SC1));
      }
#pragma unroll
      for (int ss = 0; ss < SB; ++ss) {
        if (s0 + ss < p.splitk) {
#pragma unroll
          for (int i = 0; i < TM; ++i)
#pragma unroll
            for (int j = 0; j < TN; ++j)
#pragma unroll
              for (int r4 = 0; r4 < 4; ++r4)
#pragma unroll
                for (int e = 0; e < 4; ++e) acc[i][j][4 * r4 + e] += v[ss][(i * TN + j) * 4 + r4][e];
        }
// ... 20 lines not shown
  }
  if (p.lnf_part) {
    __syncthreads();
    float2* const tab = (float2*)smem;
    if (tid < BM) tab[tid] = float2{lnf_mean, lnf_rstd};
    __syncthreads();
#pragma unroll
    for (int j = 0; j < TN; ++j) {
      const int n = min(nw + j * 32 + l31, p.N - 1);
      const float cs = p.lnf_cs[n], dn = p.lnf_d[n];
#pragma unroll
      for (int i = 0; i < TM; ++i)
#pragma unroll
        for (int r = 0; r < 16; ++r) {
          const float2 mr = tab[wm * WTM + i * 32 + (r & 3) + 8 * (r >> 2) + 4 * lg];
          acc[i][j][r] = fmaf(mr.y, acc[i][j][r] - mr.x * cs, dn);
        }
    }
    __syncthreads();
  }
  const bool unfused_split = p.splitk > 1 && !p.splitk_fused;
  if (p.mode == EPI_PLAIN) {
    const bool atomic = unfused_split;
    float* slab = atomic ? (p.splitk_ws + (size_t)split * p.M * p.N) : nullptr;
    const int b_first = m0 / HWout;
    const bool one_batch = ((m0 + BM - 1) / HWout == b_first);
    if (full && one_batch && p.epi_vec && !atomic) {
      __syncthreads();
      float* const wl = slab_base<WARPS_M * WARPS_N, WTN, LDS_BYTES>(smem, wave);
      const int rl = lane / SLAB_LPR<WTN>, c4 = (lane % SLAB_LPR<WTN>) * 4;
      f32x4 colv = {0.f, 0.f, 0.f, 0.f};
      if (p.bias) colv = *(const f32x4*)(p.bias + nw + c4);
      if (p.rowvec) colv += *(const f32x4*)(p.rowvec + (size_t)b_first * p.ld_rowvec + nw + c4);
      f32x4 g4 = {1.f, 1.f, 1.f, 1.f};
      if (p.f16_scale) g4 = *(const f32x4*)(p.f16_scale + nw + c4);
#pragma unroll
      for (int i = 0; i < TM; ++i) {
        slab_put<TN, LSTR>(wl, acc[i], l31, lg);
        constexpr int NP = SLAB_NPASS<WTN>, RPI = SLAB_RPI<WTN>;
        f32x4 resv[NP];
        if (p.residual) {
#pragma unroll
          for (int q = 0; q < NP; ++q)
            resv[q] = *(const f32x4*)(p.residual + (size_t)(mw + i * 32 + q * RPI + rl) * p.ldr + nw + c4);
        } else {
#pragma unroll
          for (int q = 0; q < NP; ++q) resv[q] = f32x4{0.f, 0.f, 0.f, 0.f};
        }
#pragma unroll
        for (int q = 0; q < NP; ++q) {
          const int row = q * RPI + rl;
          float* const lp = wl + row * LSTR + c4;
          const f32x4 v = *(const f32x4*)lp + colv + resv[q];
          const size_t ro = (size_t)(mw + i * 32 + row) * p.ldo + nw + c4;
          if (p.out_f32) SDMI_ST_F32X4(p.out_f32, ro, v);
          const f32x4 vs = v * g4;
          const f16x4 h = {(f16)vs[0], (f16)vs[1], (f16)vs[2], (f16)vs[3]};
          if (p.out_f16) SDMI_ST_F16X4(p.out_f16, ro, h);
          if (p.out_lo)
            *(f16x4*)(p.out_lo + ro) = f16x4{(f16)(v[0] - (float)h[0]), (f16)(v[1] - (float)h[1]), (f16)(v[2] - (float)h[2]),
                                            (f16)(v[3] - (float)h[3])};
          if (p.lnp_out) {
            float s1 = (v[0] + v[1]) + (v[2] + v[3]);
            float s2 = (v[0] * v[0] + v[1] * v[1]) + (v[2] * v[2] + v[3] * v[3]);
            s1 = sum8_dpp(s1); s2 = sum8_dpp(s2);
            if ((lane & 7) == 0)
              *(float2*)(p.lnp_out + 2 * ((size_t)((nw + c4) >> 5) * p.M + (size_t)(mw + i * 32 + row))) = float2{s1, s2};
          }
          if (p.gn_n > 0) *(f32x4*)lp = v;
        }
        if (p.gn_n > 0) slab_get<TN, LSTR>(wl, acc[i], l31, lg);
        else asm volatile("s_waitcnt lgkmcnt(0)" ::: "memory");
      }
    } else if (full && one_batch) {
      if (atomic) {
#pragma unroll
        for (int i = 0; i < TM; ++i)
#pragma unroll
          for (int r = 0; r < 16; ++r) {
            float* row = slab + (size_t)(mw + i * 32 + (r & 3) + 8 * (r >> 2) + 4 * lg) * p.N + nw + l31;
#pragma unroll
            for (int j = 0; j < TN; ++j) row[j * 32] = acc[i][j][r];
          }
      } else {
        float colv[TN];
#pragma unroll
        for (int j = 0; j < TN; ++j) {
          const int n = nw + j * 32 + l31;
          colv[j] = p.bias ? p.bias[n] : 0.f;
          if (p.rowvec) colv[j] += p.rowvec[(size_t)b_first * p.ld_rowvec + n];
        }
#pragma unroll
        for (int i = 0; i < TM; ++i) {
          float resv[16][TN];
          if (p.residual) {
#pragma unroll
            for (int r = 0; r < 16; ++r) {
              const float* row = p.residual + (size_t)(mw + i * 32 + (r & 3) + 8 * (r >> 2) + 4 * lg) * p.ldr + nw + l31;
#pragma unroll
              for (int j = 0; j < TN; ++j) resv[r][j] = row[j * 32];
            }
          } else {
#pragma unroll
            for (int r = 0; r < 16; ++r)
#pragma unroll
              for (int j = 0; j < TN; ++j) resv[r][j] = 0.f;
          }
#pragma unroll
          for (int r = 0; r < 16; ++r) {
            const size_t ro = (size_t)(mw + i * 32 + (r & 3) + 8 * (r >> 2) + 4 * lg) * p.ldo + nw + l31;
#pragma unroll
            for (int j = 0; j < TN; ++j) {
              const float v = acc[i][j][r] + colv[j] + resv[r][j];
              acc[i][j][r] = v;
              if (p.out_f32) p.out_f32[ro + j * 32] = v;
              if (p.out_f16) p.out_f16[ro + j * 32] = (f16)v;
              if (p.out_lo) p.out_lo[ro + j * 32] = (f16)(v - (float)(f16)v);
            }
          }
        }
      }
    } else {
      float bias_v[TN];
#pragma unroll
      for (int j = 0; j < TN; ++j) {
        const int n = nw + j * 32 + l31;
        bias_v[j] = (!atomic && p.bias && n < p.N) ? p.bias[n] : 0.f;
      }
#pragma unroll
      for (int i = 0; i < TM; ++i) {
#pragma unroll
        for (int r = 0; r < 16; ++r) {
          const int m = mw + i * 32 + (r & 3) + 8 * (r >> 2) + 4 * lg;
          if (m >= p.M) continue;
          const float* rv = (!atomic && p.rowvec) ? (p.rowvec + (size_t)(m / HWout) * p.ld_rowvec) : nullptr;
#pragma unroll
          for (int j = 0; j < TN; ++j) {
            const int n = nw + j * 32 + l31;
            if (n >= p.N) continue;
            float v = acc[i][j][r];
            if (atomic) {
              slab[(size_t)m * p.N + n] = v;
            } else {
              v += bias_v[j];
              if (rv) v += rv[n];
              if (p.residual) v += p.residual[(size_t)m * p.ldr + n];
              acc[i][j][r] = v;
              if (p.out_f32) p.out_f32[(size_t)m * p.ldo + n] = v;
              if (p.out_f16) p.out_f16[(size_t)m * p.ldo + n] = (f16)v;
              if (p.out_lo) p.out_lo[(size_t)m * p.ldo + n] = (f16)(v - (float)(f16)v);
            }
          }
        }
      }
    }
#ifdef SDMI_IGEMM_TIMING
    if (p.dbg_times && threadIdx.x == 0) p.dbg_times[6 * (size_t)blockIdx.x + 3] = (long long)__builtin_readcyclecounter();
    if (p.dbg_abl & 2) return;
#endif
    if (p.gn_n > 0 && !atomic) {
      constexpr int GNB = BM / 32;
      unsigned long long* lacc = (unsigned long long*)smem;
      static_assert(2 * GNB * 32 * GN_WORDS * 8 <= LDS_BYTES, "LDS too small for the statistics accumulators");
      __syncthreads();
      for (int e = tid; e < 2 * GNB * 32 * GN_WORDS; e += NT) lacc[e] = 0ull;
      __syncthreads();
      const int b_tile = m0 / HWout;
#pragma unroll
      for (int j = 0; j < TN; ++j) {
        const int n = nw + j * 32 + l31;
        const bool nvalid = n < p.N;
        auto flush = [&](int b, float s1, float s2) {
          if (!nvalid) { s1 = 0.f; s2 = 0.f; }
          s1 += __shfl_xor(s1, 32); s2 += __shfl_xor(s2, 32);
          for (int t = 0; t < p.gn_n; ++t) {
            const int gid = nvalid ? fast_div(p.gn_cbase[t] + n, p.gn_magic[t]) : -1;
            float a1 = s1, a2 = s2;
#pragma unroll
            for (int off = 1; off < 32; off <<= 1) {
              const float t1 = __shfl_down(a1, off, 32), t2 = __shfl_down(a2, off, 32);
              const int tg = __shfl_down(gid, off, 32);
              if (l31 + off < 32 && tg == gid) { a1 += t1; a2 += t2; }
            }
            const int gprev = __shfl_up(gid, 1, 32);
            if (lg == 0 && gid >= 0 && (l31 == 0 || gprev != gid)) {
              unsigned long long* dst = lacc + ((size_t)(t * GNB + (b - b_tile)) * 32 + gid) * GN_WORDS;
              gn_acc_add(dst, a1);
              gn_acc_add(dst + 2, a2);
            }
          }
        };
        float s1 = 0.f, s2 = 0.f;
        int bcur = -1;
#pragma unroll
        for (int i = 0; i < TM; ++i) {
          const int mt = mw + i * 32;
          if (mt < p.M) {
            const int bi = mt / HWout;
            if (bcur >= 0 && bi != bcur) { flush(bcur, s1, s2); s1 = 0.f; s2 = 0.f; }
            bcur = bi;
#pragma unroll
            for (int r = 0; r < 16; ++r) {
              const int m = mt + (r & 3) + 8 * (r >> 2) + 4 * lg;
// ... 218 lines not shown
```

### stable-diffusion_amd/csrc/igemm_kernel.h

```cpp
#pragma once
#include <string>

#include "igemm_dev.h"

namespace sdmi {
namespace {


template <int BM, int BN, int WARPS_M, int WARPS_N, bool DMA, int NS, int KIND, bool HALF = false>
__global__ void __launch_bounds__(WARPS_M* WARPS_N * 64) igemm_kernel(const IGemmParams p, const int tiles_m,
                                                                       const int tiles_n, const int kt_per_split) {
  static_assert(DMA || NS == 2, "the register-staged path is double buffered");
#if defined(__HIP_DEVICE_COMPILE__)
  constexpr bool UP = KIND == KIND_3X3_UP;
  constexpr bool K3 = KIND != KIND_1X1;
  constexpr int NT = WARPS_M * WARPS_N * 64;
  constexpr int RPP = NT / 8;
  constexpr int A_PASSES = BM / RPP;
  constexpr int B_PASSES = BN / RPP;
  constexpr int WTM = BM / WARPS_M, WTN = BN / WARPS_N;
  constexpr int TM = WTM / 32, TN = WTN / 32;
  constexpr int STAGE_BYTES = (BM + BN) * 128;
  static_assert(A_PASSES >= 1 && B_PASSES >= 1 && TM >= 1 && TN >= 1, "tile/wave shape");
  static_assert(RPP % 16 == 0, "swizzle assumes pass offset keeps row bits 1..3");

  __shared__ __attribute__((aligned(16))) unsigned char smem[NS * STAGE_BYTES];

  const int nblk = gridDim.x;
  const int bid = blockIdx.x;
  const int q8 = nblk >> 3, r8 = nblk & 7, xcd = bid & 7;
  const int wgid = (xcd < r8 ? xcd * (q8 + 1) : r8 * (q8 + 1) + (xcd - r8) * q8) + (bid >> 3);
  const int tiles_mn = tiles_m * tiles_n;
  const int split = wgid / tiles_mn;
  const int tmn = wgid - split * tiles_mn;
  int tile_m, tile_n;
  if (p.tile_n_fastest) { tile_m = tmn / tiles_n; tile_n = tmn - tile_m * tiles_n; }
  else { tile_n = tmn / tiles_m; tile_m = tmn - tile_n * tiles_m; }
  const int m0 = tile_m * BM, n0 = tile_n * BN;
  const int nkt = HALF ? p.nkt : p.K / BK;
  const int kt_begin = split * kt_per_split;
  const int kt_end = min(nkt, kt_begin + kt_per_split);
  if (kt_begin >= kt_end) return;

  const int tid = threadIdx.x;
  SDMI_STAMP(dbg_t0);
  float2 lnf_pv[LNF_MAXP];
  float lnf_mean = 0.f, lnf_rstd = 1.f;
  const bool lnf_mine = p.lnf_part != nullptr && tid < BM;
  if (lnf_mine) lnf_request(p, min(m0 + tid, p.M - 1), lnf_pv);
  const int lane = tid & 63;
  const int wave = tid >> 6;
  const int cpos = tid & 7;
  const int lrow = tid >> 3;
  const int gch = cpos ^ ((lrow >> 1) & 7);
  const int hi_oob = (HALF && gch >= 4) ? (int)0x80000000 : 0;

  const int HWout = p.Hout * p.Wout;
  const int pad = K3 ? p.pad : 0;
  constexpr int ntap = K3 ? 9 : 1;
  const int ld = p.lda0;
  int a_off[A_PASSES];
  unsigned a_mask[K3 ? A_PASSES : 1];
  int a_ro[UP ? A_PASSES : 1][3], a_co[UP ? A_PASSES : 1][3];
#pragma unroll
  for (int i = 0; i < A_PASSES; ++i) {
    const int m = min(m0 + i * RPP + lrow, p.M - 1);
    const int b = fast_div_hw(m, p.magic_hw);
    const int rem = m - b * HWout;
    const int oy = fast_div(rem, p.magic_w), ox = rem - oy * p.Wout;
    const int pb = b * p.Hin * p.Win;
    if constexpr (UP) {
      const int Hv = 2 * p.Hin, Wv = 2 * p.Win;
      unsigned mk = 0;
#pragma unroll
      for (int d = 0; d < 3; ++d) {
        const int iy = oy + d - 1, ix = ox + d - 1;
        a_ro[i][d] = (pb + (max(iy, 0) >> 1) * p.Win) * ld * 2;
        a_co[i][d] = ((max(ix, 0) >> 1) * ld + gch * 8) * 2;
      }
#pragma unroll
      for (int t = 0; t < 9; ++t) {
        const int iy = oy + t / 3 - 1, ix = ox + t % 3 - 1;
        if (iy >= 0 && iy < Hv && ix >= 0 && ix < Wv) mk |= 1u << t;
      }
      a_mask[i] = mk | ((HALF && gch < 4) ? mk << 9 : 0u);
      a_off[i] = 0;
    } else {
      const int cy = oy * p.stride, cx = ox * p.stride;
      a_off[i] = ((pb + cy * p.Win + cx) * ld + gch * 8) * 2;
      if constexpr (K3) {
        unsigned mk = 0;
#pragma unroll
        for (int t = 0; t < 9; ++t) {
          const int iy = cy + t / 3 - pad, ix = cx + t % 3 - pad;
          if (iy >= 0 && iy < p.Hin && ix >= 0 && ix < p.Win) mk |= 1u << t;
        }
        a_mask[i] = mk | ((HALF && gch < 4) ? mk << 9 : 0u);
      }
    }
  }
  int b_off[B_PASSES];
#pragma unroll
  for (int i = 0; i < B_PASSES; ++i) {
    const int n = min(n0 + i * RPP + lrow, p.N - 1);
    b_off[i] = (n * p.K + gch * 8) * 2;
  }

  f16x8 regA[DMA ? 1 : A_PASSES], regB[DMA ? 1 : B_PASSES];
  const int wave_u = __builtin_amdgcn_readfirstlane(wave);

  int ld_kt = kt_begin;
  int ld_tap = K3 ? kt_begin % ntap : 0;
  int ld_cin0 = (kt_begin / ntap) * BK;
  int ld_ky = K3 ? ld_tap / 3 : 0, ld_kx = K3 ? ld_tap - 3 * (ld_tap / 3) : 0;
  const int pc0 = p.c0, pc1 = p.c1, pc2 = p.c2;
  const int pp0 = (pc0 + BK - 1) & ~(BK - 1), pp01 = pp0 + ((pc1 + BK - 1) & ~(BK - 1));
  int ld_boff = 0;
  if constexpr (HALF) {
    const int dense0 = ld_cin0 - (ld_cin0 >= pp0 ? pp0 - pc0 : 0) - (ld_cin0 >= pp01 ? pp01 - pp0 - pc1 : 0);
    const int left = ld_cin0 < pp0 ? pc0 - ld_cin0 : (ld_cin0 < pp01 ? pc1 - (ld_cin0 - pp0) : pc2 - (ld_cin0 - pp01));
    ld_boff = (ntap * dense0 + ld_tap * min(left, BK)) * 2;
  }

  constexpr int OOB = (int)0x80000000;
  const long long a_shift = (K3 && !UP) ? (long long)(pad * p.Win + pad) * ld * 2 : 0;
  const char* const srcA0 = (const char*)p.a0 - a_shift; const char* const srcA1 = (const char*)p.a1 - a_shift;
  const char* const srcA2 = (const char*)p.a2 - a_shift;
  const __amdgpu_buffer_rsrc_t rsrc_w = __builtin_amdgcn_make_buffer_rsrc((void*)p.w, 0, OOB, 0x00020000);
  const int pWin = p.Win;

  struct TileCursor { __amdgpu_buffer_rsrc_t rsrc_a; int a_soff, b_soff; unsigned tapbit; int ky, kx; unsigned lds; int half; };
  auto next_tile = [&](int stage) {
    TileCursor c;
    const char* src; int coff, left;
    if (ld_cin0 < pp0) { src = srcA0; coff = ld_cin0; left = pc0 - coff; }
    else if (ld_cin0 < pp01) { src = srcA1; coff = ld_cin0 - pp0; left = pc1 - coff; }
    else { src = srcA2; coff = ld_cin0 - pp01; left = pc2 - coff; }
    const bool half = HALF && left < BK;
    c.rsrc_a = __builtin_amdgcn_make_buffer_rsrc((void*)src, 0, OOB, 0x00020000);
    c.a_soff = ((K3 && !UP) ? (ld_ky * pWin + ld_kx) * ld + coff : coff) * 2;
    c.b_soff = HALF ? ld_boff : ld_kt * (BK * 2);
    c.tapbit = 1u << (half ? ld_tap + 9 : ld_tap); c.ky = ld_ky; c.kx = ld_kx;
    c.half = half ? OOB : 0;
    c.lds = stage * STAGE_BYTES;
    if (ld_kt + 1 < kt_end) {
      ++ld_kt;
      if constexpr (HALF) ld_boff += half ? BKH * 2 : BK * 2;
      if constexpr (K3) {
        ++ld_tap;
        if (++ld_kx == 3) { ld_kx = 0; ++ld_ky; }
        if (ld_tap == ntap) { ld_tap = 0; ld_ky = 0; ld_kx = 0; ld_cin0 += BK; }
      } else {
        ld_cin0 += BK;
      }
    }
    return c;
  };
  auto a_voff = [&](const TileCursor& c, int i) -> int {
    int v;
    if constexpr (UP) v = a_ro[i][c.ky] + a_co[i][c.kx];
    else v = a_off[i];
    if constexpr (K3) v = (a_mask[i] & c.tapbit) ? v : OOB;
    else if constexpr (HALF) v |= hi_oob & c.half;
    return v;
  };
  auto b_voff = [&](const TileCursor& c, int i) -> int { return HALF ? (b_off[i] | (hi_oob & c.half)) : b_off[i]; };
  auto issue_piece = [&](const TileCursor& c, int q) {
    const unsigned row0 = (q < A_PASSES ? q * RPP : BM + (q - A_PASSES) * RPP) + wave_u * 8;
    auto dst = (__attribute__((address_space(3))) void*)(smem + c.lds + row0 * 128);
    if (q < A_PASSES) __builtin_amdgcn_raw_ptr_buffer_load_lds(c.rsrc_a, dst, 16, a_voff(c, q), c.a_soff, 0, 0);
    else __builtin_amdgcn_raw_ptr_buffer_load_lds(rsrc_w, dst, 16, b_voff(c, q - A_PASSES), c.b_soff, 0, SDMI_W_AUX);
  };
  auto issue_loads = [&](int stage) {
    const TileCursor c = next_tile(stage);
#pragma unroll
    for (int q = 0; q < A_PASSES + B_PASSES; ++q) {
      if constexpr (DMA) {
        issue_piece(c, q);
      } else {
        typedef int i32x4 __attribute__((ext_vector_type(4)));
        i32x4 v;
        if (q < A_PASSES) v = __builtin_amdgcn_raw_buffer_load_b128(c.rsrc_a, a_voff(c, q), c.a_soff, 0);
        else v = __builtin_amdgcn_raw_buffer_load_b128(rsrc_w, b_voff(c, q - A_PASSES), c.b_soff, 0);
        if (q < A_PASSES) regA[q] = __builtin_bit_cast(f16x8, v);
        else regB[q - A_PASSES] = __builtin_bit_cast(f16x8, v);
      }
    }
  };
  auto commit_regs = [&](int stage) {
    if constexpr (!DMA) {
      unsigned char* As = smem + stage * STAGE_BYTES;
      unsigned char* Bs = As + BM * 128;
#pragma unroll
      for (int i = 0; i < A_PASSES; ++i) *(f16x8*)(As + (i * RPP + lrow) * 128 + cpos * 16) = regA[i];
#pragma unroll
      for (int i = 0; i < B_PASSES; ++i) *(f16x8*)(Bs + (i * RPP + lrow) * 128 + cpos * 16) = regB[i];
    }
  };

  const int wm = wave / WARPS_N, wn = wave - wm * WARPS_N;
  const int l31 = lane & 31, lg = lane >> 5;
  const int rsw = (l31 >> 1) & 7;
  f32x16 acc[TM][TN];
// ... 35 lines not shown
    asm volatile("s_waitcnt lgkmcnt(0)\n\ts_barrier" ::: "memory");
    f16x8 fa[2][G][TM], fb[2][G][TN];
#pragma unroll
    for (int g = 0; g < G; ++g) read_frags(0, g, fa[0][g], fb[0][g]);
    int cur = 0, nxt = NS - 1;
    for (int kt = kt_begin; kt < kt_end; ++kt) {
      const TileCursor c = next_tile(nxt);
      const int cur1 = (cur + 1 == NS) ? 0 : cur + 1;
#pragma unroll
      for (int u = 0; u < U; ++u) {
        if (u + 1 < U) {
#pragma unroll
          for (int g = 0; g < G; ++g) read_frags(cur, (u + 1) * G + g, fa[(u + 1) & 1][g], fb[(u + 1) & 1][g]);
#pragma unroll
          for (int q = u * PPU; q < (u + 1) * PPU && q < LPT; ++q) issue_piece(c, q);
        } else {
          wait_vmcnt<LPT*(NS - 2)>();
          asm volatile("s_waitcnt lgkmcnt(0)\n\ts_barrier" ::: "memory");
#pragma unroll
          for (int g = 0; g < G; ++g) read_frags(cur1, g, fa[0][g], fb[0][g]);
        }
#pragma unroll
        for (int g = 0; g < G; ++g) mfma_step(fa[u & 1][g], fb[u & 1][g]);
        __builtin_amdgcn_sched_group_barrier(0x100, G * (TM + TN), 0);
#pragma unroll
        for (int e = 0; e < MPU; ++e) {
          __builtin_amdgcn_sched_group_barrier(0x008, 1, 0);
          if (u + 1 < U && e < PPU && u * PPU + e < LPT) __builtin_amdgcn_sched_group_barrier(0x010, 1, 0);
        }
      }
      cur = cur1;
      nxt = (nxt + 1 == NS) ? 0 : nxt + 1;
    }
    wait_vmcnt<0>();
  } else {
    issue_loads(0);
    commit_regs(0);
    for (int kt = kt_begin; kt < kt_end; ++kt) {
      const int cur = (kt - kt_begin) & 1;
      __syncthreads();
      const bool more = (kt + 1 < kt_end);
      if (more) issue_loads(cur ^ 1);
#pragma unroll
      for (int ks = 0; ks < BK / 16; ++ks) {
        f16x8 a[TM], b[TN];
        read_frags(cur, ks, a, b);
        mfma_step(a, b);
      }
      if (more) commit_regs(cur ^ 1);
    }
  }

  SDMI_STAMP(dbg_t2);
  igemm_epilogue<BM, BN, WARPS_M, WARPS_N, NS * STAGE_BYTES>(p, acc, m0, n0, split, tile_m, tile_n, smem, lnf_mean, lnf_rstd);
#ifdef SDMI_IGEMM_TIMING
  if (p.dbg_times && tid == 0) {
    long long* d = p.dbg_times + 6 * (size_t)blockIdx.x;
    d[0] = dbg_t0; d[1] = dbg_t1; d[2] = dbg_t2; d[4] = (long long)__builtin_readcyclecounter();
  }
#endif
#endif
}

template <int BM, int BN, int WARPS_M, int WARPS_N, int NS, bool HALF = false>
int launch_cfg(const IGemmParams& p, bool dma, int splitk, hipStream_t stream) {
  SDMI_CHECK(HALF || (p.c0 % BK == 0 && p.c1 % BK == 0 && p.c2 % BK == 0), "internal: a half k-tile launch on the whole-chunk kernel");
  const int tiles_m = cdiv(p.M, BM), tiles_n = cdiv(p.N, BN);
  const int nkt = igemm_nkt(p);
  const int kt_per_split = cdiv(nkt, splitk);
  const int nsplit = cdiv(nkt, kt_per_split);
  IGemmParams q = p;
  q.nkt = nkt;
  q.splitk = nsplit;
  q.tile_n_fastest = tile_order_n_fastest(p);
  q.splitk_fused = 0;
  slab_layout(q, BM, BN, WARPS_M, WARPS_N, nsplit);
  q.epi_vec = epi_vec_ok(p);
  SDMI_CHECK(splitk_ws_need(p, BM, BN, nsplit) <= p.splitk_ws_floats, "split-K workspace too small");
  SDMI_CHECK((int64_t)p.M < (int64_t)65536 * p.Hout * p.Wout, "fast_div_hw: at most 65535 samples per launch");
  q.magic_hw = div_magic_hw(p.Hout * p.Wout);
  q.magic_w = div_magic(p.Wout);
  for (int t = 0; t < p.gn_n; ++t) q.gn_magic[t] = div_magic(p.gn_cpg[t]);
  dim3 grid(tiles_m * tiles_n * nsplit), block(WARPS_M * WARPS_N * 64);
  static const int by_shape = env_int("SDMI_PROF_SHAPES", 0);
  std::string pname = std::string("igemm_") + std::to_string(BM) + "x" + std::to_string(BN) + "w" +
                      std::to_string(WARPS_M * WARPS_N) + "s" + std::to_string(NS) + (HALF ? "h" : "");
  if (by_shape && prof_enabled())
    pname += "_M" + std::to_string(p.M) + "_N" + std::to_string(p.N) + "_K" + std::to_string(p.K) + "_k" +
             std::to_string(p.ksize) + "_m" + std::to_string(p.mode) + "_s" + std::to_string(nsplit);
  const double src_pix = (double)p.B * p.Hin * p.Win;
  const double out_b = (p.out_f32 ? 4.0 : 0.0) + ((p.out_f16 || p.mode != EPI_PLAIN) ? 2.0 : 0.0);
  const double n_out = p.mode == EPI_GEGLU ? p.N / 2.0 : (double)p.N;
  const int k_alg = p.k_alg > 0 ? p.k_alg : p.K;
  const double cin_alg = p.k_alg > 0 ? (double)p.k_alg : (double)(p.c0 + p.c1 + p.c2);
  ProfScope ps(pname.c_str(), 2.0 * p.M * (double)p.N * k_alg,
               src_pix * cin_alg * 2.0 + (double)p.N * k_alg * 2.0 + (double)p.M * n_out * out_b +
                   (p.residual ? (double)p.M * p.N * 4.0 : 0.0),
               stream, 2.0 * p.M * (double)p.N * p.K);
  const int kind = p.ksize == 1 ? KIND_1X1 : (p.up ? KIND_3X3_UP : KIND_3X3);
#define SDMI_LAUNCH_KIND(K_)                                                                                        \
  do {                                                                                                              \
    if (dma) SDMI_LAUNCH((igemm_kernel<BM, BN, WARPS_M, WARPS_N, true, NS, K_, HALF>), grid, block, 0, stream, q,   \
                                tiles_m, tiles_n, kt_per_split);                                                    \
    else SDMI_LAUNCH((igemm_kernel<BM, BN, WARPS_M, WARPS_N, false, 2, K_, HALF>), grid, block, 0, stream, q,       \
                            tiles_m, tiles_n, kt_per_split);                                                        \
  } while (0)
  if (kind == KIND_1X1) SDMI_LAUNCH_KIND(KIND_1X1);
  else if (kind == KIND_3X3) SDMI_LAUNCH_KIND(KIND_3X3);
  else SDMI_LAUNCH_KIND(KIND_3X3_UP);
#undef SDMI_LAUNCH_KIND
  SDMI_HIP_OK(hipGetLastError());
  ps.end();
  if (nsplit > 1) return launch_splitk_reduce(q, nsplit, stream);
  if (q.ln_out) return launch_layernorm(q.out_f32, q.ln_gamma, q.ln_beta, q.ln_out, q.M, q.N, q.ln_eps, stream);
  return 0;
}

}
}
```

### stable-diffusion_amd/csrc/small.hip

```cpp
#include "common.h"
#include "igemm_dev.h"
#include "prof.h"
#include <math.h>
#include <vector>

namespace sdmi {
namespace {

__global__ void temb_kernel(const int64_t* t_i64, const float* t_f32, const float* freqs, float* out, int B, int dim) {
  const int half = dim / 2;
  const int idx = blockIdx.x * blockDim.x + threadIdx.x;
  if (idx >= B * half) return;
  const int b = idx / half, i = idx - b * half;
  const float t = t_i64 ? (float)t_i64[b] : t_f32[b];
  const float arg = t * freqs[i];
  out[(size_t)b * dim + i] = cosf(arg);
  out[(size_t)b * dim + half + i] = sinf(arg);
  if ((dim & 1) && i == 0) out[(size_t)b * dim + dim - 1] = 0.f;
}

constexpr int SL_MAXB = 8;
__global__ void __launch_bounds__(256) small_linear_kernel(const float* in, int ld_in, const float* w, const float* bias,
                                                           float* out, int ld_out, int B, int N, int K, int silu_in) {
  const int lane = threadIdx.x & 63;
// ... 576 lines not shown
  SDMI_HIP_OK(hipGetLastError());
  return 0;
}

int launch_quick_gelu_split(const float* x, f16* out, f16* out_lo, int64_t n, hipStream_t s) {
  SDMI_CHECK(x && out && out_lo, "quick_gelu_split: null operand");
  SDMI_CHECK(n >= 4 && n % 4 == 0, "quick_gelu_split: n % 4");
  SDMI_LAUNCH(gelu_split_kernel<false>, dim3((unsigned)((n / 4 + 255) / 256)), dim3(256), 0, s, x, out, out_lo, n / 4);
  SDMI_HIP_OK(hipGetLastError());
  return 0;
}

int launch_gelu_erf_split(const float* x, f16* out, f16* out_lo, int64_t n, hipStream_t s) {
  SDMI_CHECK(x && out && out_lo, "gelu_erf_split: null operand");
  SDMI_CHECK(n >= 4 && n % 4 == 0, "gelu_erf_split: n % 4");
  SDMI_LAUNCH(gelu_split_kernel<true>, dim3((unsigned)((n / 4 + 255) / 256)), dim3(256), 0, s, x, out, out_lo, n / 4);
  SDMI_HIP_OK(hipGetLastError());
  return 0;
}

int launch_pointwise_nchw(const float* x, const float* w, const float* bias, float* out, int B, int Cin, int Cout, int HW,
                          float in_scale, hipStream_t s) {
  SDMI_CHECK(Cin >= 1 && Cin <= PW_MAXC && Cout >= 1, "pointwise conv: 1 <= Cin <= 16");
  const int64_t total = (int64_t)B * HW;
  SDMI_LAUNCH(pointwise_nchw_kernel, dim3((unsigned)((total + 255) / 256)), dim3(256), 0, s, x, w, bias, out, B, Cin,
                     Cout, HW, in_scale);
  SDMI_HIP_OK(hipGetLastError());
  return 0;
}

int launch_softmax_rows(const float* S, f16* P, int rows, int cols, int lds, int ldp, float scale, hipStream_t s) {
  SDMI_CHECK(cols % 4 == 0 && lds % 4 == 0 && ldp % 4 == 0 && rows >= 1, "softmax rows: cols % 4");
  ProfScope ps("softmax_rows", 0.0, (double)rows * cols * 6.0, s);
  SDMI_LAUNCH(softmax_rows_kernel, dim3(rows), dim3(256), 0, s, S, P, cols, lds, ldp, scale);
  SDMI_HIP_OK(hipGetLastError());
  return 0;
}

int launch_pack_conv_weight_src(const float* w, f16* dst, int O, int I, int KH, int KW, int c0, int c1, int c2, hipStream_t s) {
  SDMI_CHECK(c0 > 0 && c1 >= 0 && c2 >= 0 && c0 + c1 + c2 == I && (c2 == 0 || c1 > 0), "conv pack: the source split must add up to the input channels");
  SDMI_CHECK(c0 % 32 == 0 && c1 % 32 == 0 && c2 % 32 == 0, "conv pack: every A source must be a multiple of 32 channels");
  const int64_t total = (int64_t)O * I * KH * KW;
  SDMI_LAUNCH(pack_conv_src_kernel, dim3((unsigned)((total + 255) / 256)), dim3(256), 0, s, w, dst, O, I, KH, KW, c0, c1, c2, 0);
  SDMI_HIP_OK(hipGetLastError());
  return 0;
}
int launch_pack_conv_weight(const float* w, f16* dst, int O, int I, int KH, int KW, hipStream_t s) {
  if (KH * KW > 1 && I % 64 != 0) return launch_pack_conv_weight_src(w, dst, O, I, KH, KW, I, 0, 0, s);
  const int64_t total = (int64_t)O * I * KH * KW;
  SDMI_LAUNCH(pack_conv_kernel, dim3((unsigned)((total + 255) / 256)), dim3(256), 0, s, w, dst, O, I, KH, KW);
  SDMI_HIP_OK(hipGetLastError());
  return 0;
}
__global__ void __launch_bounds__(256) prefetch_lines_kernel(const unsigned* p, long long nlines) {
  const long long i = (long long)blockIdx.x * 256 + threadIdx.x;
  if (i >= nlines) return;
  const unsigned v = __builtin_nontemporal_load(p + i * 32);
  asm volatile("" ::"v"(v));
}
int launch_prefetch_lines(const void* ptr, int64_t bytes, hipStream_t s) {
  const long long nlines = bytes / 128;
  if (nlines <= 0) return 0;
  SDMI_LAUNCH(prefetch_lines_kernel, dim3((unsigned)((nlines + 255) / 256)), dim3(256), 0, s, (const unsigned*)ptr, nlines);
  SDMI_HIP_OK(hipGetLastError());
  return 0;
}

int launch_pack_conv_split3(const float* w, f16* dst, int O, int I, int KH, int KW, hipStream_t s) {
  SDMI_CHECK(I % 32 == 0, "split-fp16 conv pack: input channels % 64 must be 0, or 32 (a half k-tile)");
  const int64_t total = (int64_t)O * 3 * I * KH * KW;
  if (I % 64 != 0) {
    SDMI_LAUNCH(pack_conv_src_kernel, dim3((unsigned)((total + 255) / 256)), dim3(256), 0, s, w, dst, O, I, KH, KW, I, I, I, 1);
    SDMI_HIP_OK(hipGetLastError());
    return 0;
  }
  SDMI_LAUNCH(pack_conv_split3_kernel, dim3((unsigned)((total + 255) / 256)), dim3(256), 0, s, w, dst, O, I, KH, KW);
  SDMI_HIP_OK(hipGetLastError());
  return 0;
}
int launch_pack_conv_out(const float* w, float* dst, int O, int I, hipStream_t s) {
  const int64_t total = (int64_t)O * I * 9;
  SDMI_LAUNCH(pack_conv_f32_kernel, dim3((unsigned)((total + 255) / 256)), dim3(256), 0, s, w, dst, O, I, 3, 3);
  SDMI_HIP_OK(hipGetLastError());
  return 0;
}
int launch_pack_rows(const float* w, f16* dst, int rows, int cols, int dst_row0, int dst_ld, hipStream_t s) {
  const int64_t total = (int64_t)rows * cols;
  SDMI_LAUNCH(pack_rows_kernel, dim3((unsigned)((total + 255) / 256)), dim3(256), 0, s, w, dst, rows, cols,
                     dst_row0, dst_ld);
  SDMI_HIP_OK(hipGetLastError());
  return 0;
}

__global__ void __launch_bounds__(256) ln_fold_prep_kernel(const f16* w, int N, int K, int ldw, const float* gamma, const float* beta,
                                                           const float* bias, float* cs, float* d) {
  const int lane = threadIdx.x & 63;
  const int n = blockIdx.x * 4 + (threadIdx.x >> 6);
  if (n >= N) return;
  const f16* row = w + (size_t)n * ldw;
  float a = 0.f, b = 0.f;
  for (int k = lane; k < K; k += 64) { const float wv = (float)row[k]; a = fmaf(gamma[k], wv, a); b = fmaf(beta[k], wv, b); }
#pragma unroll
  for (int o = 32; o >= 1; o >>= 1) { a += __shfl_xor(a, o); b += __shfl_xor(b, o); }
  if (lane == 0) { cs[n] = a; d[n] = b + (bias ? bias[n] : 0.f); }
}
int launch_ln_fold_prep(const f16* w, int N, int K, int ldw, const float* gamma, const float* beta, const float* bias, float* cs,
// ... 22 lines not shown
```

### stable-diffusion_amd/csrc/unet.cpp

```cpp
#include "unet.h"

extern "C" char** environ;
#include "prof.h"
#include "split16.h"

#include <math.h>
#include <stdio.h>
#include <string.h>

#include <algorithm>

namespace sdmi {

static bool in_list(const int* v, int n, int x) {
  for (int i = 0; i < n; ++i)
    if (v[i] == x) return true;
  return false;
}

thread_local Tape* g_tape_rec = nullptr;

namespace {
uint64_t sdmi_env_hash() {
  uint64_t h = 1469598103934665603ull;
// ... 229 lines not shown
}

UNet::~UNet() {
  if (emb_tab_) (void)hipFree(emb_tab_);
  if (emb_tab_tdev_) (void)hipFree(emb_tab_tdev_);
  for_each_layer([](Layer& L) -> int {
    for (auto& T : L.tb) {
      if (T.ck) (void)hipFree(T.ck);
      if (T.cvt) (void)hipFree(T.cvt);
      if (T.ck_lo) (void)hipFree(T.ck_lo);
      if (T.cvt_lo) (void)hipFree(T.cvt_lo);
    }
    return 0;
  });
}

int UNet::set_weight(const char* key, const float* ptr, const int64_t* shape, int ndim, hipStream_t stream) {
  if (int rc = store_.set(key, ptr, shape, ndim, stream)) return rc;
  ++weights_gen_;
  finalized_ = false;
  ctx_valid_ = false;
  drop_timestep_table();
  return 0;
}

int UNet::finalize() {
  if (const WeightSlot* m = store_.missing()) return fail("weight not set: " + m->key);
  if (store_.zero_page()) return -1;
  if (reserve_ctx_cache(8, 77)) return -1;
  {
    SDMI_HIP_OK(hipDeviceSynchronize());
    if (for_each_layer([&](Layer& L) -> int {
      if (L.kind != L_ATTN || full()) return 0;
      const int C = L.cin;
      for (auto& T : L.tb) {
        const int n_[3] = {3 * C, C, 8 * C};
        const f16* w_[3] = {T.wqkv, T.wq2, T.wgg};
        const float* b_[3] = {nullptr, nullptr, T.bgg};
        for (int i = 0; i < 3; ++i) {
          if (store_.alloc((void**)&T.lnf[2 * i], (size_t)n_[i] * sizeof(float)) || store_.alloc((void**)&T.lnf[2 * i + 1], (size_t)n_[i] * sizeof(float)))
            return -1;
          if (launch_ln_fold_prep(w_[i], n_[i], C, C, T.ln[2 * i], T.ln[2 * i + 1], b_[i], T.lnf[2 * i], T.lnf[2 * i + 1], nullptr)) return -1;
        }
        if (ff_tail_supported(C, 32, 32)) {
          if (store_.alloc((void**)&T.lnf_csd, (size_t)16 * C * sizeof(float))) return -1;
          for (int h = 0; h < 4; ++h) {
            SDMI_HIP_OK(hipMemcpyAsync(T.lnf_csd + (size_t)h * 4 * C, T.lnf[4] + (size_t)h * 2 * C, (size_t)2 * C * sizeof(float), hipMemcpyDeviceToDevice, nullptr));
            SDMI_HIP_OK(hipMemcpyAsync(T.lnf_csd + (size_t)h * 4 * C + 2 * C, T.lnf[5] + (size_t)h * 2 * C, (size_t)2 * C * sizeof(float), hipMemcpyDeviceToDevice, nullptr));
          }
        }
      }
      return 0;
    })) return -1;
    SDMI_HIP_OK(hipDeviceSynchronize());
    if (for_each_layer([&](Layer& L) -> int {
      if (L.kind != L_RES || L.updown || L.cin == L.cout || !L.f32[5] || !L.f32[6]) return 0;
      std::vector<float> b2((size_t)L.cout), bs((size_t)L.cout);
      SDMI_HIP_OK(hipMemcpy(b2.data(), L.f32[5], b2.size() * sizeof(float), hipMemcpyDeviceToHost));
      SDMI_HIP_OK(hipMemcpy(bs.data(), L.f32[6], bs.size() * sizeof(float), hipMemcpyDeviceToHost));
      for (size_t i = 0; i < b2.size(); ++i) b2[i] += bs[i];
      if (store_.alloc((void**)&L.bias_fold, b2.size() * sizeof(float))) return -1;
      SDMI_HIP_OK(hipMemcpy(L.bias_fold, b2.data(), b2.size() * sizeof(float), hipMemcpyHostToDevice));
      return 0;
    })) return -1;
  }
  ++weights_gen_;
  finalized_ = true;
  return 0;
}

namespace {
struct PackedHeader {
  char magic[8];
  int32_t abi, precise_1x1, n_buffers, reserved;
  sdmi_unet_cfg cfg;
  int64_t total_bytes;
};
constexpr int64_t PK_ALIGN = 256;
constexpr int PK_NHC_SHIFT = 16;
constexpr int32_t PK_NHC_MASK = 0xfff << PK_NHC_SHIFT;
constexpr int32_t PK_FULL = 4;
}

int UNet::packed_layout(std::vector<std::pair<void**, size_t>>* bufs, int64_t* total) const {
  int64_t off = (int64_t)round_up((int64_t)sizeof(PackedHeader), PK_ALIGN);
  for (const auto& b : store_.buffers()) {
    if (bufs) bufs->push_back(b);
    off += (int64_t)round_up((int64_t)b.second, PK_ALIGN);
  }
  *total = off;
  return 0;
}

int UNet::export_packed(void* host_buf, int64_t bytes, hipStream_t stream) {
  SDMI_CHECK(finalized_, "export needs a finalized handle");
  std::vector<std::pair<void**, size_t>> bufs;
  int64_t total = 0;
  packed_layout(&bufs, &total);
  SDMI_CHECK(host_buf && bytes >= total, "packed buffer too small: need " + std::to_string(total) + " bytes");
  PackedHeader h{};
  memcpy(h.magic, "SDMIPK01", 8);
  h.abi = SDMI_ABI_VERSION; h.precise_1x1 = precise_1x1_ ? 1 : 0; h.n_buffers = (int32_t)bufs.size(); h.cfg = cfg_;
  h.reserved = (precise_kv_ ? 1 : 0) | (precise_last_res_ ? 2 : 0) | (precise_1x1_max_ds_ << 8);
  h.reserved |= (ext_.attention_block << 4) | (ext_.resblock_updown << 5) | ((scale_shift_ ? 1 : 0) << 6);
  h.reserved |= num_head_channels_ << PK_NHC_SHIFT;
  if (full()) h.reserved |= PK_FULL;
// ... 382 lines not shown
      if (chain_ff) {
        TBlock& T = L.tb[0];
        FfTailParams q = FfTailParams();
        q.ln = ln; q.lnp = lnp; q.ln_eps = 1e-5f; q.csd = T.lnf_csd; q.wgg = T.wgg; q.wff2 = T.wff2; q.bff2 = T.bff2; q.t = t; q.wpo = L.w16[1];
        if (chain_tail) { q.a16 = ao; q.wo = T.wo2; q.bo = T.bo2; q.ln_gamma = T.ln[4]; }
        q.epi = p;
        if (!dry && !rc) ok(launch_ff_tail(q, s));
      } else {
        gemm(p);
      }
    }
    scratch.off = mark;
    return out;
  }

  void attention(const f16* q, const f16* k, const f16* vt, f16* out, Layer& L, int nq, int nkv, int nkv_pad, float scale) {
    AttnParams a = AttnParams();
    a.q = q; a.k = k; a.vt = vt; a.out = out; a.BH = B * L.heads; a.heads = L.heads; a.nq = nq; a.nkv = nkv;
    a.nkv_pad = nkv_pad; a.d = L.dh; a.scale = scale;
    if (!dry && !rc) ok(launch_attention(a, s));
  }

  Act resample(Layer& L, const Act& x, bool up) {
    const int Hin = x.H, Win = x.W, C = x.C;
    const int Hout = up ? 2 * Hin : (Hin - 1) / 2 + 1, Wout = up ? 2 * Win : (Win - 1) / 2 + 1;
    const size_t mark = scratch.off;
    if (u->full()) {
      const int64_t n = (int64_t)B * Hin * Win * C;
      f16* hi = S<f16>((size_t)n); f16* lo = S<f16>((size_t)n);
      if (!dry && !rc) ok(launch_cast_f16(x.p, hi, lo, n, s));
      Act out = make_act(P<float>((size_t)B * Hout * Wout * C), L.cout, Hout, Wout, true);
      IGemmParams p = conv3(hi, C, Hin, Win, Hout, Wout, up ? 1 : 2, up ? 1 : 0, L.w16[0], L.cout);
      split3(p, hi, lo, C);
      p.bias = L.f32[0]; p.out_f32 = out.p; p.ldo = L.cout;
      attach_gn_targets(p, out);
      gemm(p);
      scratch.off = mark;
      return out;
    }
    const f16* x16 = nullptr;
    if (dry) { if (!want_f16_copy(x)) (void)S<f16>((size_t)B * Hin * Win * C); }
    else {
      x16 = f16_copy(x);
      if (!x16) {
        f16* c = S<f16>((size_t)B * Hin * Win * C);
        if (!rc) ok(launch_cast_f16(x.p, c, nullptr, (int64_t)B * Hin * Win * C, s));
        x16 = c;
      }
    }
    Act out = make_act(P<float>((size_t)B * Hout * Wout * C), L.cout, Hout, Wout, true);
    IGemmParams p = conv3(x16, C, Hin, Win, Hout, Wout, up ? 1 : 2, up ? 1 : 0, L.w16[0], L.cout);
    p.bias = L.f32[0]; p.out_f32 = out.p; p.ldo = L.cout;
    attach_gn_targets(p, out);
    gemm(p);
    scratch.off = mark;
    return out;
  }

  Act res_block_updown(Layer& L, const Act& x) {
    const int dir = L.updown, H = x.H, W = x.W, C = L.cin;
    if (x.C != C || L.cout != C) ok(fail("resampling res block channel mismatch at " + L.prefix));
    if (dir > 0 && ((H | W) & 1)) ok(fail("resampling res block at " + L.prefix + ": the 2x2 average pool needs even H and W"));
    const int Ho = dir > 0 ? H / 2 : 2 * H, Wo = dir > 0 ? W / 2 : 2 * W, M = B * Ho * Wo;
    const bool p3 = L.precise3;
    const bool ss = u->scale_shift_;
    const float* const film = ss ? emb_all + L.emb_off : nullptr;
    const size_t mark = scratch.off;
    float* g = S<float>((size_t)B * H * W * C);
    groupnorm(x, nullptr, L.f32[0], L.f32[1], 1e-5f, 1, nullptr, g, nullptr);
    f16* a = S<f16>((size_t)M * C);
    f16* a_lo = p3 ? S<f16>((size_t)M * C) : nullptr;
    float* xs = S<float>((size_t)M * C);
    if (!dry && !rc) ok(launch_resample2(g, nullptr, a, a_lo, B, H, W, C, dir, s));
    if (!dry && !rc) ok(launch_resample2(x.p, xs, nullptr, nullptr, B, H, W, C, dir, s));
    float* h = S<float>((size_t)M * C);
    Act out = make_act(P<float>((size_t)M * C), C, Ho, Wo, true);
    Act hact = make_act(h, C, Ho, Wo, true);
    {
      IGemmParams p = conv3(a, C, Ho, Wo, Ho, Wo, 1, 0, L.w16[0], C);
      if (p3) split3(p, a, a_lo, C);
      p.bias = L.f32[2];
      if (!ss) { p.rowvec = emb_all + L.emb_off; p.ld_rowvec = emb_ld; }
      p.out_f32 = h; p.ldo = C;
      attach_gn_targets(p, hact);
      TapeCaller tc(Tape::R_EMB, emb_caller ? p.rowvec : nullptr);
      gemm(p);
    }
    {
      f16* a2 = S<f16>((size_t)M * C);
      f16* a2_lo = p3 ? S<f16>((size_t)M * C) : nullptr;
      {
        TapeCaller tc(Tape::R_EMB, emb_caller ? film : nullptr);
        groupnorm(hact, nullptr, L.f32[3], L.f32[4], 1e-5f, 1, a2, nullptr, nullptr, a2_lo, nullptr, false, false, film, emb_ld);
      }
      IGemmParams p = conv3(a2, C, Ho, Wo, Ho, Wo, 1, 0, L.w16[1], C);
      if (p3) split3(p, a2, a2_lo, C);
      p.bias = L.f32[5]; p.residual = xs; p.ldr = C; p.out_f32 = out.p; p.ldo = C;
      attach_gn_targets(p, out);
      gemm(p);
    }
    scratch.off = mark;
    return out;
  }

  Act attn_block_legacy(Layer& L, const Act& x) {
    const int H = x.H, W = x.W, N = H * W, M = B * N, C = L.cin;
// ... 373 lines not shown
```

### stable-diffusion_amd/csrc/unet.h

```cpp
#pragma once
#include <stdlib.h>

#include <memory>
#include <string>
#include <utility>
#include <vector>

#include "../../include/sdmi.h"
#include "common.h"
#include "weights.h"

namespace sdmi {

struct Arena {
  char* base = nullptr; size_t cap = 0, off = 0, peak = 0; bool dry = false; bool overflow = false;
  void* alloc(size_t bytes) {
    const size_t a = (off + 255) & ~(size_t)255;
    off = a + bytes;
    peak = std::max(peak, off);
    if (dry) return (void*)(uintptr_t)(a + 4096);
    if (off > cap) { overflow = true; return base; }
    return base + a;
  }
};
// ... 122 lines not shown
    g.x0 = x0.p; g.c0 = x0.C;
    if (x1) { g.x1 = x1->p; g.c1 = x1->C; }
    g.B = B; g.HW = x0.H * x0.W; g.gamma = gamma; g.beta = beta; g.eps = eps; g.silu = silu;
    g.out_f16 = o16; g.out_f32 = o32; g.raw_f16 = raw; g.out_lo = o16_lo; g.raw_lo = raw_lo;
    g.stats_only = stats_only ? 1 : 0;
    const int idx = gn_calls;
    g.acc = next_gn_acc();
    if (plan) {
      const int cpg = (g.c0 + g.c1) / 32;
      if (dry) {
        const bool f = x0.stats && (!x1 || x1->stats) && x0.id >= 0 && (!x1 || x1->id >= 0);
        if ((int)plan->fused.size() <= idx) plan->fused.resize(idx + 1, 0);
        plan->fused[idx] = f ? 1 : 0;
        if (f) {
          plan->targets[x0.id].push_back({idx, 0, cpg});
          if (x1) plan->targets[x1->id].push_back({idx, g.c0, cpg});
        }
      } else {
        g.skip_stats = (idx < (int)plan->fused.size() && plan->fused[idx]) ? 1 : 0;
      }
    }
    if (!dry && !rc && !(stats_only && g.skip_stats) && !already_applied) ok(launch_groupnorm(g, s));
    return g.acc;
  }
};

enum LayerKind { L_CONV_IN, L_RES, L_ATTN, L_DOWN, L_UP, L_ATTN_LEGACY };

struct TBlock {
  f16* wqkv = nullptr;
  f16* wo1 = nullptr; float* bo1 = nullptr;
  f16* wq2 = nullptr;
  f16* wkv2 = nullptr;
  f16* wo2 = nullptr; float* bo2 = nullptr;
  f16* wgg = nullptr; float* bgg = nullptr;
  f16* wff2 = nullptr; float* bff2 = nullptr;
  float* ln[6] = {nullptr, nullptr, nullptr, nullptr, nullptr, nullptr};
  f16* ck = nullptr; f16* cvt = nullptr;
  f16* ck_lo = nullptr; f16* cvt_lo = nullptr;
  float* lnf[6] = {nullptr, nullptr, nullptr, nullptr, nullptr, nullptr};
  float* lnf_csd = nullptr;
};

struct Layer {
  LayerKind kind = L_RES;
  std::string prefix;
  int cin = 0, cout = 0, heads = 0, dh = 0, emb_off = 0, attn_index = -1;
  int updown = 0;
  bool p1x1 = true, precise3 = false;
  f16* w16[3] = {nullptr, nullptr, nullptr};
  float* w32[1] = {nullptr};
  float* f32[7] = {nullptr, nullptr, nullptr, nullptr, nullptr, nullptr, nullptr};
  float* bias_fold = nullptr;
  std::vector<TBlock> tb;
};

class UNet {
 public:
  UNet() = default;
  ~UNet();
  UNet(const UNet&) = delete;
  UNet& operator=(const UNet&) = delete;

  int build(const sdmi_unet_cfg& cfg, int precision = SDMI_PRECISION_MIXED, const sdmi_unet_ext* ext = nullptr, unsigned flags = 0);
  int set_weight(const char* key, const float* ptr, const int64_t* shape, int ndim, hipStream_t stream);
  int finalize();
  int packed_layout(std::vector<std::pair<void**, size_t>>* bufs, int64_t* total) const;
  int export_packed(void* host_buf, int64_t bytes, hipStream_t stream);
  int import_packed(const void* host_buf, int64_t bytes, hipStream_t stream);
  int run(const float* x, const int64_t* t_i64, const float* t_f32, const float* ctx, float* eps_out, int B, int H, int W,
          int Lctx, void* workspace, int64_t ws_bytes, hipStream_t stream, bool dry, bool ctx_only, int64_t* bytes_needed);

  int cache_timesteps(const int64_t* t_host, int n, hipStream_t stream);
  int reserve_ctx_cache(int B, int Lctx);
  int hint_timestep(int64_t t);

  const WeightStore& weights() const { return store_; }

  sdmi_unet_cfg cfg_{};
  sdmi_unet_ext ext_{};
  bool has_ctx() const { return ext_.attention_block == 0; }
  bool scale_shift_ = false;
  int num_head_channels_ = 0;
  int precision_ = SDMI_PRECISION_MIXED;
  bool full() const { return precision_ == SDMI_PRECISION_FULL; }
  int te_ = 0, emb_total_ = 0, n_attn_ = 0;
  bool precise_1x1_ = true;
  bool precise_last_res_ = true;
  int precise_1x1_max_ds_ = 4;
  bool precise_kv_ = true;

 private:
  friend struct Fwd;
  template <class F> int for_each_layer(F&& fn) {
    for (auto& blk : input_blocks_) for (auto& L : blk) if (int r = fn(L)) return r;
    for (auto& L : middle_) if (int r = fn(L)) return r;
    for (auto& blk : output_blocks_) for (auto& L : blk) if (int r = fn(L)) return r;
    return 0;
  }
  int ensure_ctx_cache(int B, int Lctx, bool may_grow);
  GnPlan gn_plan_;
  bool fuse_gn_stats_ = true;
  bool ln_fold_ = true; int ln_fold_min_rows_ = 512;
  bool ff_tail_ = true;
  bool st_head_ = true;
  bool skip_fold_ = true; int skip_fold_max_w_ = 64;
// ... 41 lines not shown
```

### stable-diffusion_amd/csrc/vae.cpp

```cpp
#include "vae.h"

#include "split16.h"

#include <math.h>

#include <algorithm>

namespace sdmi {

int Vae::build(const sdmi_vae_cfg& c, int parts, const sdmi_vae_ext* ext, int precision) {
  cfg_ = c; parts_ = parts; precision_ = precision;
  if (ext) ext_ = *ext;
  SDMI_CHECK((ext_.double_z == 0 || ext_.double_z == 1) && (ext_.mid_attn == 0 || ext_.mid_attn == 1) && ext_.n_embed >= 0,
             "first-stage extension: double_z and mid_attn are 0 or 1, n_embed >= 0");
  SDMI_CHECK(ext_.n_embed == 0 || (c.embed_dim == 1 || c.embed_dim == 2 || c.embed_dim == 3 || c.embed_dim == 4 || c.embed_dim == 8),
             "codebook quantizer: embed_dim must be 1, 2, 3, 4 or 8");
  SDMI_CHECK(parts >= 1 && parts <= 3, "parts: 1 decoder, 2 encoder, 3 both");
  SDMI_CHECK(c.n_levels >= 1 && c.n_levels <= 8 && c.num_res_blocks >= 1, "bad level / res block count");
  SDMI_CHECK(c.ch % 64 == 0, "ch must be a multiple of 64 on this path");
  SDMI_CHECK(c.in_channels >= 1 && c.in_channels <= 16 && c.z_channels >= 1 && c.z_channels <= 4 && c.embed_dim >= 1 &&
                 c.embed_dim <= 8 && c.out_ch >= 1 && c.out_ch <= 8,
             "in_channels <= 16, z_channels <= 4, embed_dim <= 8, out_ch <= 8 on this path");
  const int n = c.n_levels;
  if (full() && ext_.mid_attn) {
// ... 64 lines not shown
          store_.expect(p + "." + names[i] + ".weight", {ci, ci, 1, 1}, lin_kind, &L.w16[i]);
          store_.expect(p + "." + names[i] + ".bias", {ci}, W_F32, &L.f32[2 + i]);
        }
        break;
      }
      case V_UP:
      case V_DOWN:
        store_.expect(p + ".conv.weight", {co, ci, 3, 3}, conv_kind, &L.w16[0]);
        store_.expect(p + ".conv.bias", {co}, W_F32, &L.f32[0]);
        break;
    }
  };
  if (parts & 2) {
    store_.expect("encoder.conv_in.weight", {c.ch, c.in_channels, 3, 3}, W_F32, &eci_w_);
    store_.expect("encoder.conv_in.bias", {c.ch}, W_F32, &eci_b_);
    for (auto& L : enc_) visit(L);
    store_.expect("encoder.norm_out.weight", {enc_c_end_}, W_F32, &eno_g_);
    store_.expect("encoder.norm_out.bias", {enc_c_end_}, W_F32, &eno_b_);
    store_.expect("encoder.conv_out.weight", {enc_zc(), enc_c_end_, 3, 3}, W_CONV_OUT, &eco_w_);
    store_.expect("encoder.conv_out.bias", {enc_zc()}, W_F32, &eco_b_);
    store_.expect("quant_conv.weight", {enc_ed(), enc_zc(), 1, 1}, W_F32, &q_w_);
    store_.expect("quant_conv.bias", {enc_ed()}, W_F32, &q_b_);
  }
  if (parts & 1) {
    if (ext_.n_embed > 0) store_.expect("quantize.embedding.weight", {ext_.n_embed, c.embed_dim}, W_F32, &cb_);
    store_.expect("post_quant_conv.weight", {c.z_channels, c.embed_dim, 1, 1}, W_F32, &pq_w_);
    store_.expect("post_quant_conv.bias", {c.z_channels}, W_F32, &pq_b_);
    store_.expect("decoder.conv_in.weight", {c.ch * c.ch_mult[n - 1], c.z_channels, 3, 3}, W_F32, &dci_w_);
    store_.expect("decoder.conv_in.bias", {c.ch * c.ch_mult[n - 1]}, W_F32, &dci_b_);
    for (auto& L : dec_) visit(L);
    store_.expect("decoder.norm_out.weight", {dec_c_end_}, W_F32, &dno_g_);
    store_.expect("decoder.norm_out.bias", {dec_c_end_}, W_F32, &dno_b_);
    store_.expect("decoder.conv_out.weight", {c.out_ch, dec_c_end_, 3, 3}, W_CONV_OUT, &dco_w_);
    store_.expect("decoder.conv_out.bias", {c.out_ch}, W_F32, &dco_b_);
  }
  return 0;
}

int Vae::set_weight(const char* key, const float* ptr, const int64_t* shape, int ndim, hipStream_t stream) {
  if (int rc = store_.set(key, ptr, shape, ndim, stream)) return rc;
  finalized_ = false;
  return 0;
}

int Vae::finalize() {
  if (const WeightSlot* m = store_.missing()) return fail("weight not set: " + m->key);
  if (store_.zero_page()) return -1;
  if (cb_) {
    if (store_.alloc((void**)&cb_norm_, (size_t)ext_.n_embed * sizeof(float))) return -1;
    SDMI_HIP_OK(hipDeviceSynchronize());
    if (launch_vq_norms(cb_, cb_norm_, ext_.n_embed, cfg_.embed_dim, nullptr)) return -1;
    SDMI_HIP_OK(hipDeviceSynchronize());
  }
  finalized_ = true;
  return 0;
}

struct VFwd : FwdBase {
  static constexpr float EPS = 1e-6f;
  bool full = false;

  void gemm(IGemmParams& p) { if (full) p.splitk = 1; FwdBase::gemm(p); }

  Act attn_block_full(VLayer& L, const Act& x) {
    const int H = x.H, W = x.W, N = H * W, M = B * N, C = L.cin;
    const int Np = (int)round_up(N, 8);
    const size_t mark = scratch.off;
    f16* a = S<f16>((size_t)M * C); f16* a_lo = S<f16>((size_t)M * C);
    float* y = S<float>((size_t)M * C);
    f16* qkv[3]; f16* qkv_lo[3];
    for (int i = 0; i < 3; ++i) {
      const size_t n = i == 2 ? (size_t)B * C * Np : (size_t)M * C;
      qkv[i] = S<f16>(n); qkv_lo[i] = S<f16>(n);
    }
    groupnorm(x, nullptr, L.f32[0], L.f32[1], EPS, 0, a, nullptr, nullptr, a_lo, nullptr);
    for (int i = 0; i < 3; ++i) {
      IGemmParams p = dense1x1(a, a_lo, M, C, L.w16[i], C, N, true);
      p.bias = L.f32[2 + i]; p.out_f32 = y; p.ldo = C;
      gemm(p);
      if (!dry && !rc) ok(launch_split_heads(y, C, 0, qkv[i], qkv_lo[i], i == 2 ? 1 : 0, B, N, Np, 1, C, s));
    }
    AttnSplitParams ap = AttnSplitParams();
    ap.q = qkv[0]; ap.q_lo = qkv_lo[0]; ap.k = qkv[1]; ap.k_lo = qkv_lo[1]; ap.vt = qkv[2]; ap.vt_lo = qkv_lo[2]; ap.out = a; ap.out_lo = a_lo;
    ap.BH = B; ap.heads = 1; ap.nq = N; ap.nkv = N; ap.nkv_pad = Np; ap.d = C; ap.scale = 1.0f / sqrtf((float)C);
    if (!dry && !rc) ok(launch_attention_split16(ap, s));
    Act out; out.p = P<float>((size_t)M * C); out.C = C; out.H = H; out.W = W;
    {
      IGemmParams p = dense1x1(a, a_lo, M, C, L.w16[3], C, N, true);
      p.bias = L.f32[5]; p.residual = x.p; p.ldr = C; p.out_f32 = out.p; p.ldo = C;
      gemm(p);
    }
    scratch.off = mark;
    return out;
  }

  Act res_block(VLayer& L, const Act& x) {
    const int H = x.H, W = x.W, M = B * H * W, Cin = L.cin, Cout = L.cout;
    if (x.C != Cin) ok(fail("res block channel mismatch at " + L.prefix));
    const size_t mark = scratch.off;
    const bool nin = Cin != Cout;
    const bool p1 = precise_1x1 || full;
    f16* a = S<f16>((size_t)M * Cin);
    f16* a_lo = full ? S<f16>((size_t)M * Cin) : nullptr;
    f16* raw = nin ? S<f16>((size_t)M * Cin) : nullptr;
    f16* raw_lo = (nin && p1) ? S<f16>((size_t)M * Cin) : nullptr;
    float* h = S<float>((size_t)M * Cout);
// ... 40 lines not shown
    for (int i = 0; i < 2; ++i) {
      IGemmParams p = dense(xn, M, C, L.w16[i], C, N);
      p.bias = L.f32[2 + i]; p.out_f16 = i ? k : q; p.ldo = C; p.splitk = 1;
      gemm(p);
    }
    const int QC = std::min(N, 2048);
    float* Sm = S<float>((size_t)QC * N);
    f16* Pm = S<f16>((size_t)QC * N);
    for (int b = 0; b < B; ++b) {
      {
        IGemmParams p = dense(L.w16[2], C, C, xn + (size_t)b * N * C, N, C);
        p.out_f16 = vt + (size_t)b * N * C; p.ldo = N; p.splitk = 1;
        gemm(p);
      }
      for (int r0 = 0; r0 < N; r0 += QC) {
        const int rows = std::min(QC, N - r0);
        {
          IGemmParams p = dense(q + ((size_t)b * N + r0) * C, rows, C, k + (size_t)b * N * C, N, rows);
          p.out_f32 = Sm; p.ldo = N; p.splitk = 1;
          gemm(p);
        }
        if (!dry && !rc) ok(launch_softmax_rows(Sm, Pm, rows, N, N, N, scale, s));
        {
          IGemmParams p = dense(Pm, rows, N, vt + (size_t)b * N * C, C, rows);
          p.bias = L.f32[4]; p.out_f16 = ao + ((size_t)b * N + r0) * C; p.ldo = C; p.splitk = 1;
          gemm(p);
        }
      }
    }
    Act out; out.p = P<float>((size_t)M * C); out.C = C; out.H = H; out.W = W;
    {
      IGemmParams p = dense(ao, M, C, L.w16[3], C, N);
      p.bias = L.f32[5]; p.residual = x.p; p.ldr = C; p.out_f32 = out.p; p.ldo = C;
      gemm(p);
    }
    scratch.off = mark;
    return out;
  }

  Act resample(VLayer& L, const Act& x, bool up) {
    const int Hin = x.H, Win = x.W, C = x.C;
    if (!up && ((Hin | Win) & 1)) ok(fail("first-stage Downsample needs even H and W"));
    const int Hout = up ? 2 * Hin : Hin / 2, Wout = up ? 2 * Win : Win / 2;
    const size_t mark = scratch.off;
    const int64_t n = (int64_t)B * Hin * Win * C;
    f16* x16 = S<f16>((size_t)n);
    f16* x16_lo = full ? S<f16>((size_t)n) : nullptr;
    if (!dry && !rc) ok(launch_cast_f16(x.p, x16, x16_lo, n, s));
    Act out; out.p = P<float>((size_t)B * Hout * Wout * C); out.C = C; out.H = Hout; out.W = Wout;
    IGemmParams p = conv3(x16, C, Hin, Win, Hout, Wout, up ? 1 : 2, up ? 1 : 0, L.w16[0], C);
    if (full) split3(p, x16, x16_lo, C);
    if (!up) p.pad = 0;
    p.bias = L.f32[0]; p.out_f32 = out.p; p.ldo = C;
    gemm(p);
    scratch.off = mark;
    return out;
  }

  Act run_layer(VLayer& L, const Act& x) {
    switch (L.kind) {
      case V_RES: return res_block(L, x);
      case V_ATTN: return full ? attn_block_full(L, x) : attn_block(L, x);
      case V_UP: return resample(L, x, true);
      case V_DOWN: return resample(L, x, false);
    }
    return x;
  }
};

template <class Body>
static int run_two_pass(VFwd& f, bool dry, void* workspace, int64_t ws_bytes, int64_t* bytes_needed, Body body) {
  int64_t persist_bytes = 0, scratch_bytes = 0;
  for (int pass = 0; pass < 2; ++pass) {
    const bool d = pass == 0;
    if (pass == 1 && dry) break;
    f.dry = d; f.rc = 0;
    f.persist = Arena(); f.scratch = Arena();
    f.persist.dry = f.scratch.dry = d;
    if (!d) {
      SDMI_CHECK(persist_bytes + scratch_bytes <= ws_bytes, "workspace too small: need " +
                 std::to_string(persist_bytes + scratch_bytes) + " bytes, got " + std::to_string(ws_bytes));
      SDMI_CHECK(workspace != nullptr, "workspace is NULL");
      f.persist.base = (char*)workspace; f.persist.cap = (size_t)persist_bytes;
      f.scratch.base = (char*)workspace + persist_bytes; f.scratch.cap = (size_t)scratch_bytes;
    }
    if (f.begin_pass((int64_t)8 << 20)) return -1;
    if (body(f)) return -1;
    if (f.rc) return f.rc;
    if (d) {
      persist_bytes = (int64_t)round_up((int64_t)f.persist.peak, 4096) + 4096;
      scratch_bytes = (int64_t)round_up((int64_t)f.scratch.peak, 4096) + 4096;
      if (bytes_needed) *bytes_needed = persist_bytes + scratch_bytes;
    } else {
      SDMI_CHECK(!f.persist.overflow && !f.scratch.overflow, "internal: arena overflow");
    }
  }
  return 0;
}

int Vae::decode(const float* z, float z_scale, float* img, int B, int H, int W, void* workspace, int64_t ws_bytes,
                hipStream_t stream, bool dry, int64_t* bytes_needed, bool quantize) {
  SDMI_CHECK(parts_ & 1, "this handle was created without the decoder");
  SDMI_CHECK(!quantize || ext_.n_embed > 0, "this first stage has no codebook (n_embed = 0): nothing to quantize");
  SDMI_CHECK(dry || finalized_, "sdmi_vae_finalize() has not succeeded yet");
  SDMI_CHECK(B >= 1 && B <= 8, "batch must be 1..8 per call");
  SDMI_CHECK(H >= 1 && W >= 1, "bad shape");
// ... 52 lines not shown
```

### stable-diffusion_amd/csrc/vae.h

```cpp
#pragma once
#include <string>
#include <vector>

#include "../../include/sdmi.h"
#include "common.h"
#include "unet.h"

namespace sdmi {

enum VKind { V_RES, V_ATTN, V_UP, V_DOWN };

struct VLayer {
  VKind kind = V_RES;
  std::string prefix;
  int cin = 0, cout = 0;
  f16* w16[4] = {nullptr, nullptr, nullptr, nullptr};
  float* f32[7] = {nullptr, nullptr, nullptr, nullptr, nullptr, nullptr, nullptr};
};

class Vae {
 public:
  Vae() = default;
  Vae(const Vae&) = delete;
  Vae& operator=(const Vae&) = delete;

  int build(const sdmi_vae_cfg& cfg, int parts, const sdmi_vae_ext* ext = nullptr, int precision = SDMI_PRECISION_MIXED);
  int set_weight(const char* key, const float* ptr, const int64_t* shape, int ndim, hipStream_t stream);
  int finalize();
  int decode(const float* z, float z_scale, float* img, int B, int H, int W, void* workspace, int64_t ws_bytes,
             hipStream_t stream, bool dry, int64_t* bytes_needed, bool quantize = false);
  int encode(const float* img, float* moments, int B, int H, int W, void* workspace, int64_t ws_bytes, hipStream_t stream,
             bool dry, int64_t* bytes_needed);

  const WeightStore& weights() const { return store_; }
  int factor() const { return 1 << (cfg_.n_levels - 1); }

  sdmi_vae_cfg cfg_{};
  sdmi_vae_ext ext_{1, 1, 0};
  int parts_ = 0;
  int enc_zc() const { return ext_.double_z ? 2 * cfg_.z_channels : cfg_.z_channels; }
  int enc_ed() const { return ext_.double_z ? 2 * cfg_.embed_dim : cfg_.embed_dim; }
  bool precise_1x1_ = true;
  int precision_ = SDMI_PRECISION_MIXED;
  bool full() const { return precision_ == SDMI_PRECISION_FULL; }

 private:
  friend struct VFwd;
  std::vector<VLayer> dec_, enc_;
  WeightStore store_;
  float *pq_w_ = nullptr, *pq_b_ = nullptr;
  float *dci_w_ = nullptr, *dci_b_ = nullptr;
  float *dno_g_ = nullptr, *dno_b_ = nullptr, *dco_w_ = nullptr, *dco_b_ = nullptr;
  float *eci_w_ = nullptr, *eci_b_ = nullptr;
  float *eno_g_ = nullptr, *eno_b_ = nullptr, *eco_w_ = nullptr, *eco_b_ = nullptr;
  float *q_w_ = nullptr, *q_b_ = nullptr;
  float *cb_ = nullptr, *cb_norm_ = nullptr;
  int dec_c_end_ = 0, enc_c_end_ = 0;
  bool finalized_ = false;
};

}
```

Before: 3.855.

## Decompose nearest-x2 upsample 3x3 convs into four 2x2 phase convs

Replaces each Upsample conv (nearest x2 followed by a 3x3 conv) with four 2x2 convolutions over the source map, one per output phase. Each phase uses weights pre-summed from the 3x3 taps, which cuts the GEMM K from 9*Cin to 4*Cin and the MACs by more than half. The epilogue scatters rows to the interleaved output positions, and the tuner can choose this path per shape. The path runs only when a tuning entry shows the phase version beating the original, unless forced on; it is limited to unsplit, non-halo tiles and adds weight storage.

```diff
diff --git a/include/sdmi.h b/include/sdmi.h
--- a/include/sdmi.h
+++ b/include/sdmi.h
@@ -240,6 +240,8 @@
 int sdmi_k_igemm_tail(const sdmi_igemm_desc* d, const void* t0, const void* t1, const void* t2, int tail_c, int tail_ld, const void* tail_w,
                       int tail_kt, void* stream);
 int sdmi_k_tail_split_range(int nkt, int nsplit, int split, int* begin, int* end);
+int sdmi_k_igemm_up_phase(const sdmi_igemm_desc* d, void* stream);
+int sdmi_k_up_phase_weights(const void* w_packed_f16, void* dst_f16, int N, int Cin, void* stream);
 int sdmi_k_ff_tail(const sdmi_igemm_desc* proj_out, const void* ln_f16, const float* lnp, float ln_eps, const float* csd,
                    const void* wgg_f16, const void* wff2_f16, const float* bff2, const float* t, void* stream);
 int sdmi_k_st_tail(const sdmi_igemm_desc* proj_out, const void* a_f16, const void* wo_f16, const float* bo, float* t, const float* ln_gamma,
diff --git a/stable-diffusion_amd/_lib.py b/stable-diffusion_amd/_lib.py
--- a/stable-diffusion_amd/_lib.py
+++ b/stable-diffusion_amd/_lib.py
@@ -168,6 +168,8 @@
     'sdmi_k_igemm': (C.c_int, [C.POINTER(IGemmDesc), c_ptr]),
     'sdmi_k_igemm_tail': (C.c_int, [C.POINTER(IGemmDesc), c_ptr, c_ptr, c_ptr, C.c_int, C.c_int, c_ptr, C.c_int, c_ptr]),
     'sdmi_k_tail_split_range': (C.c_int, [C.c_int, C.c_int, C.c_int, C.POINTER(C.c_int), C.POINTER(C.c_int)]),
+    'sdmi_k_igemm_up_phase': (C.c_int, [C.POINTER(IGemmDesc), c_ptr]),
+    'sdmi_k_up_phase_weights': (C.c_int, [c_ptr, c_ptr, C.c_int, C.c_int, c_ptr]),
     'sdmi_tune_lookup': (C.c_int, [C.c_int] * 9 + [C.POINTER(C.c_int), C.POINTER(C.c_int)]),
     'sdmi_unet_skip_fold_plan': (C.c_int, [c_ptr, C.c_int, C.c_int, C.c_int, C.c_int, C.POINTER(C.c_int32), C.c_int]),
     'sdmi_k_ff_tail': (C.c_int, [C.POINTER(IGemmDesc), c_ptr, c_ptr, C.c_float, c_ptr, c_ptr, c_ptr, c_ptr, c_ptr, c_ptr]),
diff --git a/stable-diffusion_amd/csrc/api.cpp b/stable-diffusion_amd/csrc/api.cpp
--- a/stable-diffusion_amd/csrc/api.cpp
+++ b/stable-diffusion_amd/csrc/api.cpp
@@ -527,6 +527,20 @@
   IGemmTune t; t.tile = d->tile; t.dma = d->dma;
   return launch_igemm(p, t, (hipStream_t)stream);
 }
+int sdmi_k_igemm_up_phase(const sdmi_igemm_desc* d, void* stream) {
+  SDMI_CHECK(d, "null descriptor");
+  IGemmParams p = IGemmParams();
+  if (igemm_params_of(d, p)) return -1;
+  SDMI_CHECK(p.ksize == 3 && p.up == 1 && p.stride == 1 && p.Hout == 2 * p.Hin && p.Wout == 2 * p.Win && p.c1 == 0 && p.c2 == 0 && !p.split16,
+             "up_phase: the descriptor is the reference op, a 3x3 stride-1 conv of one nearest-x2 upsampled source (Hout = 2 Hin, Wout = 2 Win)");
+  IGemmParams q = up_phase_of(p, p.w);
+  q.splitk = d->splitk;
+  IGemmTune t; t.tile = d->tile; t.dma = d->dma;
+  return launch_igemm(q, t, (hipStream_t)stream);
+}
+int sdmi_k_up_phase_weights(const void* w_packed, void* dst, int N, int Cin, void* stream) {
+  return launch_up_phase_weights((const f16*)w_packed, (f16*)dst, N, Cin, (hipStream_t)stream);
+}
 int sdmi_k_tail_split_range(int nkt, int nsplit, int split, int* begin, int* end) {
   SDMI_CHECK(begin && end && nkt >= 0 && nsplit >= 1 && split >= 0 && split < nsplit, "bad arguments");
   tail_split_range(nkt, nsplit, split, begin, end);
diff --git a/stable-diffusion_amd/csrc/common.h b/stable-diffusion_amd/csrc/common.h
--- a/stable-diffusion_amd/csrc/common.h
+++ b/stable-diffusion_amd/csrc/common.h
@@ -191,6 +191,12 @@
 
 int launch_igemm(const IGemmParams& p, const IGemmTune& tune, hipStream_t stream);
 bool igemm_plans_halo(const IGemmParams& p);
+bool igemm_plans_up_phase(const IGemmParams& p);
+static inline IGemmParams up_phase_of(const IGemmParams& p, const f16* w_phase) {
+  IGemmParams q = p;
+  q.ksize = 2; q.Hout = p.Hin; q.Wout = p.Win; q.M = p.B * p.Hin * p.Win; q.K = 4 * p.c0; q.w = w_phase; q.splitk = 0;
+  return q;
+}
 int tune_lookup(int M, int N, int K, int ksize, int stride, int up, int mode, int splitk_req, int kt, int* tile, int* splitk);
 bool range_check_enabled();
 uint64_t tune_generation();
@@ -367,6 +373,7 @@
 int launch_pack_split3(const float* w, f16* dst, int N, int K, hipStream_t s);
 int launch_pack_conv_weight_src(const float* w_oihw, f16* dst, int O, int I, int KH, int KW, int c0, int c1, int c2, hipStream_t s);
 int launch_pack_conv_split3(const float* w, f16* dst, int O, int I, int KH, int KW, hipStream_t s);
+int launch_up_phase_weights(const f16* wp, f16* dst, int N, int Cin, hipStream_t s);
 int launch_pack_geglu(const float* w, const float* bias, f16* wdst, float* bdst, int N, int K, hipStream_t s);
 int launch_pack_conv_out(const float* w_oihw, float* dst, int O, int I, hipStream_t s);
 
diff --git a/stable-diffusion_amd/csrc/igemm.hip b/stable-diffusion_amd/csrc/igemm.hip
--- a/stable-diffusion_amd/csrc/igemm.hip
+++ b/stable-diffusion_amd/csrc/igemm.hip
@@ -451,6 +451,12 @@
     }
     return "tune_gfx950.txt";
   }
+  static std::string phase_path_of(const std::string& table_path) {
+    static const std::string base = "tune_gfx950.txt";
+    if (table_path.size() >= base.size() && table_path.compare(table_path.size() - base.size(), base.size(), base) == 0)
+      return table_path.substr(0, table_path.size() - base.size()) + "tune_up_phase_gfx950.txt";
+    return table_path + ".up_phase";
+  }
   void load_file(const std::string& path) {
     FILE* f = fopen(path.c_str(), "r");
     if (!f) return;
@@ -471,6 +477,7 @@
     loaded = true;
     if (env_int("SDMI_TUNE_DISABLE", 0)) return;
     load_file(default_path());
+    load_file(phase_path_of(default_path()));
   }
   std::map<TuneKey, TuneChoice>::const_iterator find_entry(TuneKey k) const {
     auto it = table.find(k);
@@ -504,13 +511,13 @@
     for (int sk : splits) {
       if ((sk == 5 || sk == 10) && !tile_is_halo(t)) continue;
       if (sk > 1) {
-        if (p.splitk != 0 || !can_split) break;
+        if (p.splitk != 0 || !can_split || p.ksize == 2) break;
         if (nkt / sk < 4) break;
         if (tile_is_halo(t) && (nkt / 9) % sk != 0) continue;
         if (blocks * (sk / 2 + 1) > 1536) break;
         if (splitk_ws_need(p, c.bm, c.bn, sk) > p.splitk_ws_floats) break;
       }
-      if (blocks * sk < 48 && sk < 16 && nkt / (sk * 2) >= 4 && can_split && p.splitk == 0) continue;
+      if (blocks * sk < 48 && sk < 16 && nkt / (sk * 2) >= 4 && can_split && p.splitk == 0 && p.ksize != 2) continue;
       out.push_back({t, p.splitk > 1 ? p.splitk : sk, 0.0});
       if (p.splitk != 0) break;
     }
@@ -567,17 +574,25 @@
   if (n_keys) *n_keys = (int)g_tuner.stats.size();
   ++g_tune_generation;
   const std::string out = (path && *path) ? std::string(path) : Tuner::default_path();
-  FILE* f = fopen(out.c_str(), "w");
-  if (!f) return fail("cannot write the tuning table to " + out);
-  fprintf(f, "# libsdmi igemm tuning table (gfx950), measured in situ by tools/tune.py -- M N K ksize stride up mode splitk_req tile splitk us\n");
-  for (auto& kv : g_tuner.table) {
-    const TuneKey& k = kv.first;
-    fprintf(f, "%d %d %d %d %d %d %d %d %d %d %.2f", k.M, k.N, k.K, k.ksize, k.stride, k.up, k.mode, k.splitk_req, kv.second.tile,
-            kv.second.splitk, kv.second.us);
-    if (k.kt) fprintf(f, " %d", k.kt);
-    fprintf(f, "\n");
-  }
-  fclose(f);
+  bool any_phase = false;
+  for (auto& kv : g_tuner.table) any_phase = any_phase || kv.first.ksize == 2;
+  for (int which = 0; which < (any_phase ? 2 : 1); ++which) {
+    const std::string path_w = which ? Tuner::phase_path_of(out) : out;
+    FILE* f = fopen(path_w.c_str(), "w");
+    if (!f) return fail("cannot write the tuning table to " + path_w);
+    fputs(which ? "# libsdmi igemm tuning table (gfx950), the 2x2 phase convs of the Upsample convs (ksize 2: M = rows of one phase, K = 4 Cin; compared with "
+                       "the site's up = 1 row of the main table), measured in situ by tools/tune.py -- M N K ksize stride up mode splitk_req tile splitk us\n"
+                     : "# libsdmi igemm tuning table (gfx950), measured in situ by tools/tune.py -- M N K ksize stride up mode splitk_req tile splitk us\n", f);
+    for (auto& kv : g_tuner.table) {
+      const TuneKey& k = kv.first;
+      if ((k.ksize == 2) != (which == 1)) continue;
+      fprintf(f, "%d %d %d %d %d %d %d %d %d %d %.2f", k.M, k.N, k.K, k.ksize, k.stride, k.up, k.mode, k.splitk_req, kv.second.tile,
+              kv.second.splitk, kv.second.us);
+      if (k.kt) fprintf(f, " %d", k.kt);
+      fprintf(f, "\n");
+    }
+    fclose(f);
+  }
   return 0;
 }
 int tune_dump(std::string* out) {
@@ -623,9 +638,33 @@
          (sk == 1 || (can_split && splitk_ws_need(p, kTiles[tt].bm, kTiles[tt].bn, sk) <= p.splitk_ws_floats && nkt / sk >= 4 && (nkt / 9) % sk == 0));
 }
 
+bool igemm_plans_up_phase(const IGemmParams& p) {
+  static const int env_tile = env_int("SDMI_IGEMM_TILE", -1);
+  static const int only_ksize = env_int("SDMI_TUNE_ONLY_KSIZE", -1);
+  const int knob = env_int("SDMI_UP_PHASE", 1);
+  if (!knob || p.ksize != 3 || !p.up || p.stride != 1 || p.split16 || p.c1 || p.c2 || p.c0 % BK || p.mode != EPI_PLAIN || p.residual ||
+      p.splitk > 1 || (env_tile >= 0 && tile_is_halo(env_tile)) || (int64_t)32 * p.N * p.c0 >= ((int64_t)1 << 31))
+    return false;
+  std::lock_guard<std::mutex> lk(g_tuner.mu);
+  g_tuner.ensure_loaded();
+  if (g_tuner.collecting) return only_ksize == 2;
+  if (knob == 2) return true;
+  const auto ph = g_tuner.find_entry(TuneKey{p.B * p.Hin * p.Win, p.N, 4 * p.c0, 2, 1, 1, p.mode, 0, 0});
+  const auto old = g_tuner.find_entry(TuneKey{p.M, p.N, 9 * p.c0, 3, 1, 1, p.mode, 0, 0});
+  return ph != g_tuner.table.end() && old != g_tuner.table.end() && ph->second.splitk == 1 && !tile_is_halo(ph->second.tile) && ph->second.us > 0.0 &&
+         ph->second.us < 0.97 * old->second.us;
+}
+
 int launch_igemm(const IGemmParams& p, const IGemmTune& tune, hipStream_t stream) {
   SDMI_CHECK(p.M > 0 && p.N > 0 && p.K > 0, "empty GEMM");
-  SDMI_CHECK(p.ksize == 1 || p.ksize == 3, "ksize must be 1 or 3");
+  SDMI_CHECK(p.ksize == 1 || p.ksize == 3 || p.ksize == 2, "ksize must be 1 or 3 (or 2: the four 2x2 phase convs of an upsample conv)");
+  const bool phase = p.ksize == 2;
+  if (phase)
+    SDMI_CHECK(p.up == 1 && p.stride == 1 && p.Hout == p.Hin && p.Wout == p.Win && p.mode == EPI_PLAIN && p.c1 == 0 && p.c2 == 0 && p.c0 % BK == 0 &&
+                   !p.split16 && !p.residual && !p.ln_out && !p.lnp_out && !p.f16_scale && !p.lnf_part && !p.pgn_out && !p.tail_kt && p.splitk <= 1 &&
+                   (int64_t)4 * p.N * p.K * 2 < ((int64_t)1 << 31),
+               "upsample phase convs: nearest x2 of one source of whole 64-channel chunks (Hout x Wout = the SOURCE map), plain epilogue without residual / "
+               "LayerNorm / tail, unsplit");
   const int Cin = p.c0 + p.c1 + p.c2;
   SDMI_CHECK(p.K == p.ksize * p.ksize * Cin, "K != ksize^2 * (c0 + c1 + c2)");
   SDMI_CHECK(p.c0 % BKH == 0 && p.c1 % BKH == 0 && p.c2 % BKH == 0 && p.c0 > 0, "channel counts of every A source must be multiples of 32");
@@ -636,7 +675,7 @@
   SDMI_CHECK(p.c1 == 0 || p.a1 != nullptr, "second A source missing");
   SDMI_CHECK(p.c2 == 0 || (p.a2 != nullptr && p.lda2 % 8 == 0), "third A source missing");
   SDMI_CHECK((p.c1 == 0 || p.lda1 == p.lda0) && (p.c2 == 0 || p.lda2 == p.lda0), "all A sources must share one row pitch");
-  SDMI_CHECK(!p.up || (p.ksize == 3 && p.stride == 1), "upsample folding needs a 3x3 stride-1 conv");
+  SDMI_CHECK(!p.up || ((p.ksize == 3 || phase) && p.stride == 1), "upsample folding needs a 3x3 stride-1 conv");
   if (p.mode == EPI_GEGLU) SDMI_CHECK(p.N % 64 == 0 && p.out_f16 != nullptr, "GEGLU needs N % 64 == 0 and an fp16 output");
   if (p.ln_out)
     SDMI_CHECK(p.mode == EPI_PLAIN && p.out_f32 && p.ldo == p.N && p.N % 4 == 0 && p.N <= 2560 && p.ln_gamma && p.ln_beta,
@@ -673,7 +712,7 @@
                                (p.residual == nullptr || p.ldr % 4 == 0);
   const bool can_split_heads = p.mode == EPI_HEADS && p.splitk_ws && p.dh % 4 == 0 && p.segC % 4 == 0;
   const bool can_split = can_split_plain || can_split_heads;
-  if (env_split >= 0 && splitk == 0) splitk = env_split;
+  if (env_split >= 0 && splitk == 0 && !phase) splitk = env_split;
 
   hipEvent_t ev0 = nullptr, ev1 = nullptr;
   TuneKey tkey{p.M, p.N, nkt * BK, p.split16 ? 11 : p.ksize, p.stride, p.up, p.mode, splitk, p.tail_kt};
@@ -700,7 +739,7 @@
                                           : (sk == 1 || (ws_ok && nkt / sk >= 4 && (halo || (sk != 5 && sk != 10)) &&
                                                          (!halo || (nkt / 9) % sk == 0)));
         if (split_ok && (p.mode != EPI_GEGLU || tile_tn_even(tt)) && (!halo || halo_supported(p, kTiles[tt].bm)) &&
-            (!p.split16 || split16_tile_supported(tt))) {
+            (!p.split16 || split16_tile_supported(tt)) && (!phase || sk == 1)) {
           tile = tt; splitk = sk;
         }
       }
@@ -720,6 +759,10 @@
   if (p.lnp_out) {
     const int hw = p.Hout * p.Wout;
     if (p.M % kTiles[tile].bm || p.N % kTiles[tile].bn || hw % kTiles[tile].bm || (p.split16 && !split16_tile_supported(tile))) tile = 5;
+  }
+  if (phase) {
+    SDMI_CHECK(!tile_is_halo(tile) && splitk <= 1, "upsample phase convs run unsplit on the generic tiles");
+    splitk = 1;
   }
   if (splitk <= 0) {
     splitk = 1;
@@ -787,7 +830,7 @@
       for (int sg = 0; sg < p.N / p.segC; ++sg)
         if (range_scan(what, p.seg_dst[sg], p.seg_kind[sg] == 0 ? (int64_t)p.M * p.segC : (int64_t)p.B * p.segC * p.ntok_pad, stream)) return -1;
     } else if (p.out_f16) {
-      if (range_scan(what, p.out_f16, (int64_t)(p.M - 1) * p.ldo + (p.mode == EPI_GEGLU ? p.N / 2 : p.N), stream)) return -1;
+      if (range_scan(what, p.out_f16, (int64_t)((phase ? 4 : 1) * (int64_t)p.M - 1) * p.ldo + (p.mode == EPI_GEGLU ? p.N / 2 : p.N), stream)) return -1;
     }
     if (p.ln_out && range_scan("LayerNorm output", p.ln_out, (int64_t)p.M * p.N, stream)) return -1;
   }
diff --git a/stable-diffusion_amd/csrc/igemm_dev.h b/stable-diffusion_amd/csrc/igemm_dev.h
--- a/stable-diffusion_amd/csrc/igemm_dev.h
+++ b/stable-diffusion_amd/csrc/igemm_dev.h
@@ -67,7 +67,7 @@
   wait_vmcnt_n(N);
 }
 
-enum : int { KIND_1X1 = 0, KIND_3X3 = 1, KIND_3X3_UP = 2 };
+enum : int { KIND_1X1 = 0, KIND_3X3 = 1, KIND_3X3_UP = 2, KIND_2X2 = 3 };
 
 __device__ __forceinline__ int fast_div(int m, unsigned long long magic) {
   return (int)(((unsigned long long)(unsigned)m * magic) >> 40);
@@ -137,11 +137,11 @@
   return v;
 }
 
-template <int BM, int BN, int WARPS_M, int WARPS_N, int LDS_BYTES>
+template <int BM, int BN, int WARPS_M, int WARPS_N, int LDS_BYTES, bool PHASE = false>
 __device__ __forceinline__ void igemm_epilogue(const IGemmParams& p_arg, f32x16 (&acc)[BM / WARPS_M / 32][BN / WARPS_N / 32],
                                                const int m0, const int n0, const int split, const int tile_m,
                                                const int tile_n, unsigned char* smem, const float lnf_mean = 0.f,
-                                               const float lnf_rstd = 1.f) {
+                                               const float lnf_rstd = 1.f, const int phase = 0) {
 #ifdef SDMI_IGEMM_TIMING
   IGemmParams p = p_arg;
   if (p.dbg_abl & 1) p.residual = nullptr;
@@ -159,6 +159,16 @@
   const int wm = wave / WARPS_N, wn = wave - wm * WARPS_N;
   const int l31 = lane & 31, lg = lane >> 5;
   const int HWout = p.Hout * p.Wout;
+  auto orow = [&](int m) -> size_t {
+    if constexpr (PHASE) {
+      const int b = fast_div_hw(m, p.magic_hw);
+      const int rem = m - b * HWout;
+      const int i = fast_div(rem, p.magic_w), j = rem - i * p.Wout;
+      return ((size_t)(b * 2 * p.Hout + 2 * i + (phase >> 1)) * (size_t)(2 * p.Wout) + (size_t)(2 * j + (phase & 1)));
+    } else {
+      return (size_t)m;
+    }
+  };
   const int mw = m0 + wm * WTM, nw = n0 + wn * WTN;
   const bool full = (m0 + BM <= p.M) && (n0 + BN <= p.N);
   if (p.splitk > 1 && p.splitk_fused) {
@@ -285,7 +295,7 @@
           const int row = q * RPI + rl;
           float* const lp = wl + row * LSTR + c4;
           const f32x4 v = *(const f32x4*)lp + colv + resv[q];
-          const size_t ro = (size_t)(mw + i * 32 + row) * p.ldo + nw + c4;
+          const size_t ro = orow(mw + i * 32 + row) * p.ldo + nw + c4;
           if (p.out_f32) SDMI_ST_F32X4(p.out_f32, ro, v);
           const f32x4 vs = v * g4;
           const f16x4 h = {(f16)vs[0], (f16)vs[1], (f16)vs[2], (f16)vs[3]};
@@ -341,7 +351,7 @@
           }
 #pragma unroll
           for (int r = 0; r < 16; ++r) {
-            const size_t ro = (size_t)(mw + i * 32 + (r & 3) + 8 * (r >> 2) + 4 * lg) * p.ldo + nw + l31;
+            const size_t ro = orow(mw + i * 32 + (r & 3) + 8 * (r >> 2) + 4 * lg) * p.ldo + nw + l31;
 #pragma unroll
             for (int j = 0; j < TN; ++j) {
               const float v = acc[i][j][r] + colv[j] + resv[r][j];
@@ -367,6 +377,7 @@
           const int m = mw + i * 32 + (r & 3) + 8 * (r >> 2) + 4 * lg;
           if (m >= p.M) continue;
           const float* rv = (!atomic && p.rowvec) ? (p.rowvec + (size_t)(m / HWout) * p.ld_rowvec) : nullptr;
+          const size_t om = orow(m) * p.ldo;
 #pragma unroll
           for (int j = 0; j < TN; ++j) {
             const int n = nw + j * 32 + l31;
@@ -379,9 +390,9 @@
               if (rv) v += rv[n];
               if (p.residual) v += p.residual[(size_t)m * p.ldr + n];
               acc[i][j][r] = v;
-              if (p.out_f32) p.out_f32[(size_t)m * p.ldo + n] = v;
-              if (p.out_f16) p.out_f16[(size_t)m * p.ldo + n] = (f16)v;
-              if (p.out_lo) p.out_lo[(size_t)m * p.ldo + n] = (f16)(v - (float)(f16)v);
+              if (p.out_f32) p.out_f32[om + n] = v;
+              if (p.out_f16) p.out_f16[om + n] = (f16)v;
+              if (p.out_lo) p.out_lo[om + n] = (f16)(v - (float)(f16)v);
             }
           }
         }
diff --git a/stable-diffusion_amd/csrc/igemm_kernel.h b/stable-diffusion_amd/csrc/igemm_kernel.h
--- a/stable-diffusion_amd/csrc/igemm_kernel.h
+++ b/stable-diffusion_amd/csrc/igemm_kernel.h
@@ -13,7 +13,10 @@
   static_assert(DMA || NS == 2, "the register-staged path is double buffered");
 #if defined(__HIP_DEVICE_COMPILE__)
   constexpr bool UP = KIND == KIND_3X3_UP;
+  constexpr bool K2 = KIND == KIND_2X2;
   constexpr bool K3 = KIND != KIND_1X1;
+  constexpr int TW = K2 ? 2 : 3;
+  static_assert(!K2 || (DMA && !HALF), "the 2x2 phase kind: LDS-DMA, whole 64-channel chunks");
   constexpr int NT = WARPS_M * WARPS_N * 64;
   constexpr int RPP = NT / 8;
   constexpr int A_PASSES = BM / RPP;
@@ -38,7 +41,7 @@
   else { tile_n = tmn / tiles_m; tile_m = tmn - tile_n * tiles_m; }
   const int m0 = tile_m * BM, n0 = tile_n * BN;
   const int nkt = HALF ? p.nkt : p.K / BK;
-  const int kt_begin = split * kt_per_split;
+  const int kt_begin = K2 ? 0 : split * kt_per_split;
   const int kt_end = min(nkt, kt_begin + kt_per_split);
   if (kt_begin >= kt_end) return;
 
@@ -57,7 +60,8 @@
 
   const int HWout = p.Hout * p.Wout;
   const int pad = K3 ? p.pad : 0;
-  constexpr int ntap = K3 ? 9 : 1;
+  const int pad_y = K2 ? 1 - (split >> 1) : pad, pad_x = K2 ? 1 - (split & 1) : pad;
+  constexpr int ntap = K3 ? TW * TW : 1;
   const int ld = p.lda0;
   int a_off[A_PASSES];
   unsigned a_mask[K3 ? A_PASSES : 1];
@@ -91,8 +95,8 @@
       if constexpr (K3) {
         unsigned mk = 0;
 #pragma unroll
-        for (int t = 0; t < 9; ++t) {
-          const int iy = cy + t / 3 - pad, ix = cx + t % 3 - pad;
+        for (int t = 0; t < ntap; ++t) {
+          const int iy = cy + t / TW - pad_y, ix = cx + t % TW - pad_x;
           if (iy >= 0 && iy < p.Hin && ix >= 0 && ix < p.Win) mk |= 1u << t;
         }
         a_mask[i] = mk | ((HALF && gch < 4) ? mk << 9 : 0u);
@@ -112,7 +116,7 @@
   int ld_kt = kt_begin;
   int ld_tap = K3 ? kt_begin % ntap : 0;
   int ld_cin0 = (kt_begin / ntap) * BK;
-  int ld_ky = K3 ? ld_tap / 3 : 0, ld_kx = K3 ? ld_tap - 3 * (ld_tap / 3) : 0;
+  int ld_ky = K3 ? ld_tap / TW : 0, ld_kx = K3 ? ld_tap - TW * (ld_tap / TW) : 0;
   const int pc0 = p.c0, pc1 = p.c1, pc2 = p.c2;
   const int pp0 = (pc0 + BK - 1) & ~(BK - 1), pp01 = pp0 + ((pc1 + BK - 1) & ~(BK - 1));
   int ld_boff = 0;
@@ -123,10 +127,11 @@
   }
 
   constexpr int OOB = (int)0x80000000;
-  const long long a_shift = (K3 && !UP) ? (long long)(pad * p.Win + pad) * ld * 2 : 0;
+  const long long a_shift = (K3 && !UP) ? (long long)(pad_y * p.Win + pad_x) * ld * 2 : 0;
   const char* const srcA0 = (const char*)p.a0 - a_shift; const char* const srcA1 = (const char*)p.a1 - a_shift;
   const char* const srcA2 = (const char*)p.a2 - a_shift;
-  const __amdgpu_buffer_rsrc_t rsrc_w = __builtin_amdgcn_make_buffer_rsrc((void*)p.w, 0, OOB, 0x00020000);
+  const f16* const w_base = K2 ? p.w + (size_t)split * (size_t)p.N * (size_t)p.K : p.w;
+  const __amdgpu_buffer_rsrc_t rsrc_w = __builtin_amdgcn_make_buffer_rsrc((void*)w_base, 0, OOB, 0x00020000);
   const int pWin = p.Win;
 
   struct TileCursor { __amdgpu_buffer_rsrc_t rsrc_a; int a_soff, b_soff; unsigned tapbit; int ky, kx; unsigned lds; int half; };
@@ -148,7 +153,7 @@
       if constexpr (HALF) ld_boff += half ? BKH * 2 : BK * 2;
       if constexpr (K3) {
         ++ld_tap;
-        if (++ld_kx == 3) { ld_kx = 0; ++ld_ky; }
+        if (++ld_kx == TW) { ld_kx = 0; ++ld_ky; }
         if (ld_tap == ntap) { ld_tap = 0; ld_ky = 0; ld_kx = 0; ld_cin0 += BK; }
       } else {
         ld_cin0 += BK;
@@ -290,7 +295,8 @@
   }
 
   SDMI_STAMP(dbg_t2);
-  igemm_epilogue<BM, BN, WARPS_M, WARPS_N, NS * STAGE_BYTES>(p, acc, m0, n0, split, tile_m, tile_n, smem, lnf_mean, lnf_rstd);
+  igemm_epilogue<BM, BN, WARPS_M, WARPS_N, NS * STAGE_BYTES, K2>(p, acc, m0, n0, K2 ? 0 : split, tile_m, tile_n, smem, lnf_mean, lnf_rstd,
+                                                                 K2 ? split : 0);
 #ifdef SDMI_IGEMM_TIMING
   if (p.dbg_times && tid == 0) {
     long long* d = p.dbg_times + 6 * (size_t)blockIdx.x;
@@ -319,10 +325,12 @@
   q.magic_hw = div_magic_hw(p.Hout * p.Wout);
   q.magic_w = div_magic(p.Wout);
   for (int t = 0; t < p.gn_n; ++t) q.gn_magic[t] = div_magic(p.gn_cpg[t]);
-  dim3 grid(tiles_m * tiles_n * nsplit), block(WARPS_M * WARPS_N * 64);
+  const bool phase = p.ksize == 2;
+  if (phase) SDMI_CHECK(!HALF && dma && nsplit == 1, "the 2x2 phase convs run unsplit on the LDS-DMA kernels, whole 64-channel chunks only");
+  dim3 grid(tiles_m * tiles_n * (phase ? 4 : nsplit)), block(WARPS_M * WARPS_N * 64);
   static const int by_shape = env_int("SDMI_PROF_SHAPES", 0);
   std::string pname = std::string("igemm_") + std::to_string(BM) + "x" + std::to_string(BN) + "w" +
-                      std::to_string(WARPS_M * WARPS_N) + "s" + std::to_string(NS) + (HALF ? "h" : "");
+                      std::to_string(WARPS_M * WARPS_N) + "s" + std::to_string(NS) + (HALF ? "h" : "") + (phase ? "_up2x2" : "");
   if (by_shape && prof_enabled())
     pname += "_M" + std::to_string(p.M) + "_N" + std::to_string(p.N) + "_K" + std::to_string(p.K) + "_k" +
              std::to_string(p.ksize) + "_m" + std::to_string(p.mode) + "_s" + std::to_string(nsplit);
@@ -331,11 +339,13 @@
   const double n_out = p.mode == EPI_GEGLU ? p.N / 2.0 : (double)p.N;
   const int k_alg = p.k_alg > 0 ? p.k_alg : p.K;
   const double cin_alg = p.k_alg > 0 ? (double)p.k_alg : (double)(p.c0 + p.c1 + p.c2);
-  ProfScope ps(pname.c_str(), 2.0 * p.M * (double)p.N * k_alg,
-               src_pix * cin_alg * 2.0 + (double)p.N * k_alg * 2.0 + (double)p.M * n_out * out_b +
+  const double m_out = phase ? 4.0 * p.M : (double)p.M;
+  const double k_ref = phase ? 9.0 * cin_alg : (double)k_alg;
+  ProfScope ps(pname.c_str(), 2.0 * m_out * (double)p.N * k_ref,
+               src_pix * cin_alg * 2.0 + (double)p.N * k_ref * 2.0 + m_out * n_out * out_b +
                    (p.residual ? (double)p.M * p.N * 4.0 : 0.0),
-               stream, 2.0 * p.M * (double)p.N * p.K);
-  const int kind = p.ksize == 1 ? KIND_1X1 : (p.up ? KIND_3X3_UP : KIND_3X3);
+               stream, 2.0 * m_out * (double)p.N * p.K);
+  const int kind = p.ksize == 1 ? KIND_1X1 : (phase ? KIND_2X2 : (p.up ? KIND_3X3_UP : KIND_3X3));
 #define SDMI_LAUNCH_KIND(K_)                                                                                        \
   do {                                                                                                              \
     if (dma) SDMI_LAUNCH((igemm_kernel<BM, BN, WARPS_M, WARPS_N, true, NS, K_, HALF>), grid, block, 0, stream, q,   \
@@ -345,7 +355,9 @@
   } while (0)
   if (kind == KIND_1X1) SDMI_LAUNCH_KIND(KIND_1X1);
   else if (kind == KIND_3X3) SDMI_LAUNCH_KIND(KIND_3X3);
-  else SDMI_LAUNCH_KIND(KIND_3X3_UP);
+  else if (kind == KIND_3X3_UP) SDMI_LAUNCH_KIND(KIND_3X3_UP);
+  else if constexpr (!HALF) SDMI_LAUNCH((igemm_kernel<BM, BN, WARPS_M, WARPS_N, true, NS, KIND_2X2, false>), grid, block, 0, stream, q, tiles_m, tiles_n,
+                                        kt_per_split);
 #undef SDMI_LAUNCH_KIND
   SDMI_HIP_OK(hipGetLastError());
   ps.end();
diff --git a/stable-diffusion_amd/csrc/small.hip b/stable-diffusion_amd/csrc/small.hip
--- a/stable-diffusion_amd/csrc/small.hip
+++ b/stable-diffusion_amd/csrc/small.hip
@@ -652,6 +652,35 @@
   SDMI_HIP_OK(hipGetLastError());
   return 0;
 }
+__global__ void up_phase_weights_kernel(const f16* wp, f16* dst, int N, int Cin) {
+  const int64_t idx = (int64_t)blockIdx.x * blockDim.x + threadIdx.x;
+  const int K4 = 4 * Cin;
+  if (idx >= (int64_t)4 * N * K4) return;
+  const int phase = (int)(idx / ((int64_t)N * K4));
+  const int64_t rem = idx - (int64_t)phase * N * K4;
+  const int n = (int)(rem / K4), k = (int)(rem - (int64_t)n * K4);
+  const int chunk = k / 256, tap = (k % 256) / 64, ch = k % 64;
+  const int a = phase >> 1, c = phase & 1, dy = tap >> 1, dx = tap & 1;
+  const int ky0 = dy ? 1 + a : 0, ky1 = dy ? 2 : a, kx0 = dx ? 1 + c : 0, kx1 = dx ? 2 : c;
+  const f16* src = wp + (size_t)n * 9 * Cin + (size_t)chunk * 9 * 64 + ch;
+  float s = 0.f;
+  bool first = true;
+  for (int ky = ky0; ky <= ky1; ++ky)
+    for (int kx = kx0; kx <= kx1; ++kx) {
+      const float v = (float)src[(ky * 3 + kx) * 64];
+      s = first ? v : s + v;
+      first = false;
+    }
+  dst[idx] = (f16)s;
+}
+int launch_up_phase_weights(const f16* wp, f16* dst, int N, int Cin, hipStream_t s) {
+  SDMI_CHECK(wp && dst && N > 0 && Cin > 0 && Cin % 64 == 0, "upsample phase weights: whole 64-channel chunks of packed 3x3 weights");
+  const int64_t total = (int64_t)16 * N * Cin;
+  SDMI_CHECK(total < ((int64_t)1 << 31), "upsample phase weights: too large");
+  SDMI_LAUNCH(up_phase_weights_kernel, dim3((unsigned)((total + 255) / 256)), dim3(256), 0, s, wp, dst, N, Cin);
+  SDMI_HIP_OK(hipGetLastError());
+  return 0;
+}
 __global__ void __launch_bounds__(256) prefetch_lines_kernel(const unsigned* p, long long nlines) {
   const long long i = (long long)blockIdx.x * 256 + threadIdx.x;
   if (i >= nlines) return;
diff --git a/stable-diffusion_amd/csrc/unet.cpp b/stable-diffusion_amd/csrc/unet.cpp
--- a/stable-diffusion_amd/csrc/unet.cpp
+++ b/stable-diffusion_amd/csrc/unet.cpp
@@ -305,6 +305,11 @@
       }
       return 0;
     })) return -1;
+    if (for_each_layer([&](Layer& L) -> int {
+      if (L.kind != L_UP || full() || L.cin % 64 != 0) return 0;
+      if (store_.alloc((void**)&L.w_up_phase, (size_t)16 * L.cout * L.cin * sizeof(f16))) return -1;
+      return launch_up_phase_weights(L.w16[0], L.w_up_phase, L.cout, L.cin, nullptr);
+    })) return -1;
     SDMI_HIP_OK(hipDeviceSynchronize());
     if (for_each_layer([&](Layer& L) -> int {
       if (L.kind != L_RES || L.updown || L.cin == L.cout || !L.f32[5] || !L.f32[6]) return 0;
@@ -793,6 +798,7 @@
     IGemmParams p = conv3(x16, C, Hin, Win, Hout, Wout, up ? 1 : 2, up ? 1 : 0, L.w16[0], L.cout);
     p.bias = L.f32[0]; p.out_f32 = out.p; p.ldo = L.cout;
     attach_gn_targets(p, out);
+    if (up && L.w_up_phase && (p.gn_n == 0 || (Hin * Win) % 32 == 0) && igemm_plans_up_phase(p)) p = up_phase_of(p, L.w_up_phase);
     gemm(p);
     scratch.off = mark;
     return out;
diff --git a/stable-diffusion_amd/csrc/unet.h b/stable-diffusion_amd/csrc/unet.h
--- a/stable-diffusion_amd/csrc/unet.h
+++ b/stable-diffusion_amd/csrc/unet.h
@@ -198,6 +198,7 @@
   float* w32[1] = {nullptr};
   float* f32[7] = {nullptr, nullptr, nullptr, nullptr, nullptr, nullptr, nullptr};
   float* bias_fold = nullptr;
+  f16* w_up_phase = nullptr;
   std::vector<TBlock> tb;
 };
 
diff --git a/stable-diffusion_amd/csrc/vae.cpp b/stable-diffusion_amd/csrc/vae.cpp
--- a/stable-diffusion_amd/csrc/vae.cpp
+++ b/stable-diffusion_amd/csrc/vae.cpp
@@ -140,6 +140,15 @@
     if (launch_vq_norms(cb_, cb_norm_, ext_.n_embed, cfg_.embed_dim, nullptr)) return -1;
     SDMI_HIP_OK(hipDeviceSynchronize());
   }
+  if (!full()) {
+    SDMI_HIP_OK(hipDeviceSynchronize());
+    for (auto& L : dec_) {
+      if (L.kind != V_UP || L.cin % 64 != 0) continue;
+      if (store_.alloc((void**)&L.w_up_phase, (size_t)16 * L.cout * L.cin * sizeof(f16))) return -1;
+      if (launch_up_phase_weights(L.w16[0], L.w_up_phase, L.cout, L.cin, nullptr)) return -1;
+    }
+    SDMI_HIP_OK(hipDeviceSynchronize());
+  }
   finalized_ = true;
   return 0;
 }
@@ -286,6 +295,7 @@
     if (full) split3(p, x16, x16_lo, C);
     if (!up) p.pad = 0;
     p.bias = L.f32[0]; p.out_f32 = out.p; p.ldo = C;
+    if (up && !full && L.w_up_phase && igemm_plans_up_phase(p)) p = up_phase_of(p, L.w_up_phase);
     gemm(p);
     scratch.off = mark;
     return out;
diff --git a/stable-diffusion_amd/csrc/vae.h b/stable-diffusion_amd/csrc/vae.h
--- a/stable-diffusion_amd/csrc/vae.h
+++ b/stable-diffusion_amd/csrc/vae.h
@@ -16,6 +16,7 @@
   int cin = 0, cout = 0;
   f16* w16[4] = {nullptr, nullptr, nullptr, nullptr};
   float* f32[7] = {nullptr, nullptr, nullptr, nullptr, nullptr, nullptr, nullptr};
+  f16* w_up_phase = nullptr;
 };
 
 class Vae {
```

Result: faster. 3.902 (median of 6 runs) (+1.2%).
